# DengZhuangSouthRd/simple_tensorflow

Measured on AMD Instinct MI355X. Metric: images/sec, higher is better.
Workload: dtype bf16; 1 GPU; model=resnet50_v1, global_batch=256, parallelism=dp1

## Files before the change

simple_tensorflow_amd/csrc/framework/ops_defs.cc:

```cpp
#include "framework/op.h"

namespace stf {

#define NUMTYPES "{float, double, int32, int64, bfloat16, half, uint8, int8, complex64}"
#define REALTYPES "{float, double, int32, int64, bfloat16, half}"
#define FLOATTYPES "{float, double, bfloat16, half}"

REGISTER_OP("Const").Output("output: dtype").Attr("dtype: type").Attr("value: tensor");
REGISTER_OP("Placeholder").Output("output: dtype").Attr("dtype: type").Attr("shape: shape = []");
REGISTER_OP("DepthwiseConv2dNative").Input("input: T").Input("filter: T").Output("output: T").Attr("T: {float, bfloat16}").Attr("strides: list(int)").Attr("padding: string").Attr("data_format: string = 'NHWC'");
REGISTER_OP("DepthwiseConv2dNativeBackpropInput").Input("input_sizes: int32").Input("filter: T").Input("out_backprop: T").Output("output: T").Attr("T: {float, bfloat16}").Attr("strides: list(int)").Attr("padding: string").Attr("data_format: string = 'NHWC'");
REGISTER_OP("DepthwiseConv2dNativeBackpropFilter").Input("input: T").Input("filter_sizes: int32").Input("out_backprop: T").Output("output: T").Attr("T: {float, bfloat16}").Attr("strides: list(int)").Attr("padding: string").Attr("data_format: string = 'NHWC'");
REGISTER_OP("PlaceholderWithDefault").Input("input: dtype").Output("output: dtype").Attr("dtype: type").Attr("shape: shape");
REGISTER_OP("Identity").Input("input: T").Output("output: T").Attr("T: type");
REGISTER_OP("StopGradient").Input("input: T").Output("output: T").Attr("T: type");
REGISTER_OP("PreventGradient").Input("input: T").Output("output: T").Attr("T: type").Attr("message: string = ''");
REGISTER_OP("Shape").Input("input: T").Output("output: out_type").Attr("T: type").Attr("out_type: {int32, int64} = int32");
REGISTER_OP("ShapeN").Input("input: N * T").Output("output: N * out_type").Attr("N: int >= 1").Attr("T: type").Attr("out_type: {int32, int64} = int32");
REGISTER_OP("Rank").Input("input: T").Output("output: int32").Attr("T: type");
REGISTER_OP("Size").Input("input: T").Output("output: out_type").Attr("T: type").Attr("out_type: {int32, int64} = int32");
REGISTER_OP("Reshape").Input("tensor: T").Input("shape: Tshape").Output("output: T").Attr("T: type").Attr("Tshape: {int32, int64} = int32");
REGISTER_OP("ExpandDims").Input("input: T").Input("dim: Tdim").Output("output: T").Attr("T: type").Attr("Tdim: {int32, int64} = int32");
REGISTER_OP("Squeeze").Input("input: T").Output("output: T").Attr("T: type").Attr("squeeze_dims: list(int) = []");
REGISTER_OP("Fill").Input("dims: int32").Input("value: T").Output("output: T").Attr("T: type");
REGISTER_OP("ZerosLike").Input("x: T").Output("y: T").Attr("T: type");
REGISTER_OP("OnesLike").Input("x: T").Output("y: T").Attr("T: type");
REGISTER_OP("Cast").Input("x: SrcT").Output("y: DstT").Attr("SrcT: type").Attr("DstT: type");
REGISTER_OP("Pack").Input("values: N * T").Output("output: T").Attr("N: int >= 1").Attr("T: type").Attr("axis: int = 0");
REGISTER_OP("Unpack").Input("value: T").Output("output: num * T").Attr("num: int >= 0").Attr("T: type").Attr("axis: int = 0");
REGISTER_OP("ConcatV2").Input("values: N * T").Input("axis: Tidx").Output("output: T").Attr("N: int >= 2").Attr("T: type").Attr("Tidx: {int32, int64} = int32");
REGISTER_OP("Concat").Input("concat_dim: int32").Input("values: N * T").Output("output: T").Attr("N: int >= 2").Attr("T: type");
REGISTER_OP("ConcatOffset").Input("concat_dim: int32").Input("shape: N * int32").Output("offset: N * int32").Attr("N: int >= 2");
REGISTER_OP("Split").Input("split_dim: int32").Input("value: T").Output("output: num_split * T").Attr("num_split: int >= 1").Attr("T: type");
REGISTER_OP("SplitV").Input("value: T").Input("size_splits: Tlen").Input("split_dim: int32").Output("output: num_split * T").Attr("num_split: int >= 1").Attr("T: type").Attr("Tlen: {int32, int64} = int64");
REGISTER_OP("Slice").Input("input: T").Input("begin: Index").Input("size: Index").Output("output: T").Attr("T: type").Attr("Index: {int32, int64}");
REGISTER_OP("StridedSlice").Input("input: T").Input("begin: Index").Input("end: Index").Input("strides: Index").Output("output: T").Attr("T: type").Attr("Index: {int32, int64}").Attr("begin_mask: int = 0").Attr("end_mask: int = 0").Attr("ellipsis_mask: int = 0").Attr("new_axis_mask: int = 0").Attr("shrink_axis_mask: int = 0");
REGISTER_OP("StridedSliceGrad").Input("shape: Index").Input("begin: Index").Input("end: Index").Input("strides: Index").Input("dy: T").Output("output: T").Attr("T: type").Attr("Index: {int32, int64}").Attr("begin_mask: int = 0").Attr("end_mask: int = 0").Attr("ellipsis_mask: int = 0").Attr("new_axis_mask: int = 0").Attr("shrink_axis_mask: int = 0");
REGISTER_OP("Pad").Input("input: T").Input("paddings: Tpaddings").Output("output: T").Attr("T: type").Attr("Tpaddings: {int32, int64} = int32");
REGISTER_OP("Transpose").Input("x: T").Input("perm: Tperm").Output("y: T").Attr("T: type").Attr("Tperm: {int32, int64} = int32");
REGISTER_OP("Gather").Input("params: Tparams").Input("indices: Tindices").Output("output: Tparams").Attr("validate_indices: bool = true").Attr("Tparams: type").Attr("Tindices: {int32, int64}");
REGISTER_OP("GatherV2").Input("params: Tparams").Input("indices: Tindices").Input("axis: Taxis").Output("output: Tparams").Attr("Tparams: type").Attr("Tindices: {int32, int64}").Attr("Taxis: {int32, int64} = int32");
REGISTER_OP("Tile").Input("input: T").Input("multiples: Tmultiples").Output("output: T").Attr("T: type").Attr("Tmultiples: {int32, int64} = int32");
REGISTER_OP("InvertPermutation").Input("x: T").Output("y: T").Attr("T: {int32, int64} = int32");
REGISTER_OP("Reverse").Input("tensor: T").Input("dims: bool").Output("output: T").Attr("T: type");
REGISTER_OP("BroadcastGradientArgs").Input("s0: T").Input("s1: T").Output("r0: T").Output("r1: T").Attr("T: {int32, int64} = int32");
REGISTER_OP("OneHot").Input("indices: TI").Input("depth: int32").Input("on_value: T").Input("off_value: T").Output("output: T").Attr("axis: int = -1").Attr("T: type").Attr("TI: {uint8, int32, int64} = int64");
REGISTER_OP("Range").Input("start: Tidx").Input("limit: Tidx").Input("delta: Tidx").Output("output: Tidx").Attr("Tidx: {float, double, int32, int64} = int32");
REGISTER_OP("LinSpace").Input("start: T").Input("stop: T").Input("num: Tidx").Output("output: T").Attr("T: {float, double}").Attr("Tidx: {int32, int64} = int32");
REGISTER_OP("CheckNumerics").Input("tensor: T").Output("output: T").Attr("T: " FLOATTYPES).Attr("message: string");
REGISTER_OP("UnsortedSegmentSum").Input("data: T").Input("segment_ids: Tindices").Input("num_segments: int32").Output("output: T").Attr("T: " NUMTYPES).Attr("Tindices: {int32, int64}");
REGISTER_OP("DynamicStitch").Input("indices: N * int32").Input("data: N * T").Output("merged: T").Attr("N: int >= 1").Attr("T: type");

#define BINARY_OP(NAME) REGISTER_OP(NAME).Input("x: T").Input("y: T").Output("z: T")
BINARY_OP("Add").Attr("T: " NUMTYPES);
BINARY_OP("Sub").Attr("T: " NUMTYPES);
BINARY_OP("Mul").Attr("T: " NUMTYPES);
BINARY_OP("Div").Attr("T: " NUMTYPES);
BINARY_OP("RealDiv").Attr("T: " NUMTYPES);
BINARY_OP("FloorDiv").Attr("T: " NUMTYPES);
BINARY_OP("FloorMod").Attr("T: " NUMTYPES);
BINARY_OP("Pow").Attr("T: " NUMTYPES);
BINARY_OP("Maximum").Attr("T: " REALTYPES);
BINARY_OP("Minimum").Attr("T: " REALTYPES);
BINARY_OP("SquaredDifference").Attr("T: " NUMTYPES);
#undef BINARY_OP
#define CMP_OP(NAME) REGISTER_OP(NAME).Input("x: T").Input("y: T").Output("z: bool")
CMP_OP("Less").Attr("T: " REALTYPES);
CMP_OP("LessEqual").Attr("T: " REALTYPES);
CMP_OP("Greater").Attr("T: " REALTYPES);
CMP_OP("GreaterEqual").Attr("T: " REALTYPES);
CMP_OP("Equal").Attr("T: " NUMTYPES);
CMP_OP("NotEqual").Attr("T: " NUMTYPES);
#undef CMP_OP
REGISTER_OP("LogicalAnd").Input("x: bool").Input("y: bool").Output("z: bool");
REGISTER_OP("LogicalOr").Input("x: bool").Input("y: bool").Output("z: bool");
REGISTER_OP("LogicalNot").Input("x: bool").Output("y: bool");
#define UNARY_OP(NAME) REGISTER_OP(NAME).Input("x: T").Output("y: T")
UNARY_OP("Neg").Attr("T: " NUMTYPES);
UNARY_OP("Abs").Attr("T: " REALTYPES);
UNARY_OP("Sign").Attr("T: " REALTYPES);
UNARY_OP("Square").Attr("T: " NUMTYPES);
UNARY_OP("Sqrt").Attr("T: " FLOATTYPES);
UNARY_OP("Rsqrt").Attr("T: " FLOATTYPES);
UNARY_OP("Exp").Attr("T: " FLOATTYPES);
UNARY_OP("Log").Attr("T: " FLOATTYPES);
UNARY_OP("Log1p").Attr("T: " FLOATTYPES);
UNARY_OP("Tanh").Attr("T: " FLOATTYPES);
UNARY_OP("Sigmoid").Attr("T: " FLOATTYPES);
UNARY_OP("Sin").Attr("T: " FLOATTYPES);
UNARY_OP("Cos").Attr("T: " FLOATTYPES);
UNARY_OP("Floor").Attr("T: " FLOATTYPES);
UNARY_OP("Ceil").Attr("T: " FLOATTYPES);
UNARY_OP("Round").Attr("T: " FLOATTYPES);
UNARY_OP("Reciprocal").Attr("T: " NUMTYPES);
#undef UNARY_OP
REGISTER_OP("IsNan").Input("x: T").Output("y: bool").Attr("T: " FLOATTYPES);
REGISTER_OP("IsInf").Input("x: T").Output("y: bool").Attr("T: " FLOATTYPES);
REGISTER_OP("IsFinite").Input("x: T").Output("y: bool").Attr("T: " FLOATTYPES);
#define GRAD2_OP(NAME) REGISTER_OP(NAME).Input("y: T").Input("dy: T").Output("z: T").Attr("T: " FLOATTYPES)
GRAD2_OP("SigmoidGrad");
GRAD2_OP("TanhGrad");
GRAD2_OP("RsqrtGrad");
GRAD2_OP("SqrtGrad");
GRAD2_OP("ReciprocalGrad");
#undef GRAD2_OP
REGISTER_OP("AddN").Input("inputs: N * T").Output("sum: T").Attr("N: int >= 1").Attr("T: " NUMTYPES);
REGISTER_OP("MatMul").Input("a: T").Input("b: T").Output("product: T").Attr("transpose_a: bool = false").Attr("transpose_b: bool = false").Attr("T: " FLOATTYPES);
REGISTER_OP("BatchMatMul").Input("x: T").Input("y: T").Output("output: T").Attr("T: " FLOATTYPES).Attr("adj_x: bool = false").Attr("adj_y: bool = false");
#define REDUCE_OP(NAME) REGISTER_OP(NAME).Input("input: T").Input("reduction_indices: Tidx").Output("output: T").Attr("keep_dims: bool = false").Attr("T: " NUMTYPES).Attr("Tidx: {int32, int64} = int32")
REDUCE_OP("Sum");
REDUCE_OP("Mean");
REDUCE_OP("Prod");
REDUCE_OP("Max");
REDUCE_OP("Min");
#undef REDUCE_OP
REGISTER_OP("All").Input("input: bool").Input("reduction_indices: Tidx").Output("output: bool").Attr("keep_dims: bool = false").Attr("Tidx: {int32, int64} = int32");
REGISTER_OP("Any").Input("input: bool").Input("reduction_indices: Tidx").Output("output: bool").Attr("keep_dims: bool = false").Attr("Tidx: {int32, int64} = int32");
REGISTER_OP("ArgMax").Input("input: T").Input("dimension: Tidx").Output("output: output_type").Attr("T: " NUMTYPES).Attr("Tidx: {int32, int64} = int32").Attr("output_type: {int32, int64} = int64");
REGISTER_OP("ArgMin").Input("input: T").Input("dimension: Tidx").Output("output: output_type").Attr("T: " NUMTYPES).Attr("Tidx: {int32, int64} = int32").Attr("output_type: {int32, int64} = int64");
REGISTER_OP("Select").Input("condition: bool").Input("t: T").Input("e: T").Output("output: T").Attr("T: type");
REGISTER_OP("Cumsum").Input("x: T").Input("axis: Tidx").Output("out: T").Attr("exclusive: bool = false").Attr("reverse: bool = false").Attr("T: " NUMTYPES).Attr("Tidx: {int32, int64} = int32");

REGISTER_OP("Conv2D").Input("input: T").Input("filter: T").Output("output: T").Attr("T: " FLOATTYPES).Attr("strides: list(int)").Attr("use_cudnn_on_gpu: bool = true").Attr("padding: string").Attr("data_format: string = 'NHWC'");
REGISTER_OP("Conv2DBackpropInput").Input("input_sizes: int32").Input("filter: T").Input("out_backprop: T").Output("output: T").Attr("T: " FLOATTYPES).Attr("strides: list(int)").Attr("use_cudnn_on_gpu: bool = true").Attr("padding: string").Attr("data_format: string = 'NHWC'");
REGISTER_OP("Conv2DBackpropInputAdd").Input("input_sizes: int32").Input("filter: T").Input("out_backprop: T").Input("side: T").Output("output: T").Attr("T: " FLOATTYPES).Attr("strides: list(int)").Attr("padding: string").Attr("data_format: string = 'NHWC'");
REGISTER_OP("Conv2DBackpropFilter").Input("input: T").Input("filter_sizes: int32").Input("out_backprop: T").Output("output: T").Attr("T: " FLOATTYPES).Attr("strides: list(int)").Attr("use_cudnn_on_gpu: bool = true").Attr("padding: string").Attr("data_format: string = 'NHWC'");
REGISTER_OP("BiasAdd").Input("value: T").Input("bias: T").Output("output: T").Attr("T: " NUMTYPES).Attr("data_format: string = 'NHWC'");
REGISTER_OP("BiasAddGrad").Input("out_backprop: T").Output("output: T").Attr("T: " NUMTYPES).Attr("data_format: string = 'NHWC'");
REGISTER_OP("Relu").Input("features: T").Output("activations: T").Attr("T: " REALTYPES);
REGISTER_OP("ReluGrad").Input("gradients: T").Input("features: T").Output("backprops: T").Attr("T: " REALTYPES);
REGISTER_OP("Relu6").Input("features: T").Output("activations: T").Attr("T: " REALTYPES);
REGISTER_OP("Relu6Grad").Input("gradients: T").Input("features: T").Output("backprops: T").Attr("T: " REALTYPES);
REGISTER_OP("Elu").Input("features: T").Output("activations: T").Attr("T: " FLOATTYPES);
REGISTER_OP("EluGrad").Input("gradients: T").Input("outputs: T").Output("backprops: T").Attr("T: " FLOATTYPES);
REGISTER_OP("Softplus").Input("features: T").Output("activations: T").Attr("T: " FLOATTYPES);
REGISTER_OP("SoftplusGrad").Input("gradients: T").Input("features: T").Output("backprops: T").Attr("T: " FLOATTYPES);
REGISTER_OP("Softmax").Input("logits: T").Output("softmax: T").Attr("T: " FLOATTYPES);
REGISTER_OP("LogSoftmax").Input("logits: T").Output("logsoftmax: T").Attr("T: " FLOATTYPES);
REGISTER_OP("SoftmaxCrossEntropyWithLogits").Input("features: T").Input("labels: T").Output("loss: T").Output("backprop: T").Attr("T: " FLOATTYPES);
REGISTER_OP("SparseSoftmaxCrossEntropyWithLogits").Input("features: T").Input("labels: Tlabels").Output("loss: T").Output("backprop: T").Attr("T: " FLOATTYPES).Attr("Tlabels: {int32, int64} = int64");
REGISTER_OP("MaxPool").Input("input: T").Output("output: T").Attr("T: " FLOATTYPES).Attr("ksize: list(int)").Attr("strides: list(int)").Attr("padding: string").Attr("data_format: string = 'NHWC'");
REGISTER_OP("MaxPoolGrad").Input("orig_input: T").Input("orig_output: T").Input("grad: T").Output("output: T").Attr("T: " FLOATTYPES).Attr("ksize: list(int)").Attr("strides: list(int)").Attr("padding: string").Attr("data_format: string = 'NHWC'");
REGISTER_OP("AvgPool").Input("value: T").Output("output: T").Attr("T: " FLOATTYPES).Attr("ksize: list(int)").Attr("strides: list(int)").Attr("padding: string").Attr("data_format: string = 'NHWC'");
REGISTER_OP("AvgPoolGrad").Input("orig_input_shape: int32").Input("grad: T").Output("output: T").Attr("T: " FLOATTYPES).Attr("ksize: list(int)").Attr("strides: list(int)").Attr("padding: string").Attr("data_format: string = 'NHWC'");
REGISTER_OP("FusedBatchNorm").Input("x: T").Input("scale: T").Input("offset: T").Input("mean: T").Input("variance: T").Output("y: T").Output("batch_mean: T").Output("batch_variance: T").Output("reserve_space_1: T").Output("reserve_space_2: T").Attr("T: {float}").Attr("epsilon: float = 0.0001").Attr("data_format: string = 'NHWC'").Attr("is_training: bool = true");
REGISTER_OP("FusedBatchNormGrad").Input("y_backprop: T").Input("x: T").Input("scale: T").Input("reserve_space_1: T").Input("reserve_space_2: T").Output("x_backprop: T").Output("scale_backprop: T").Output("offset_backprop: T").Output("reserve_space_3: T").Output("reserve_space_4: T").Attr("T: {float}").Attr("epsilon: float = 0.0001").Attr("data_format: string = 'NHWC'").Attr("is_training: bool = true");
REGISTER_OP("BatchNormMi").Input("x: T").Input("scale: float").Input("offset: float").Output("y: T").Output("batch_mean: float").Output("batch_variance: float").Output("reserve_inv_std: float").Attr("T: {float, bfloat16}").Attr("epsilon: float = 0.0001").Attr("fuse_relu: bool = false");
REGISTER_OP("BatchNormAddReluMi").Input("x: T").Input("scale: float").Input("offset: float").Input("side: T").Output("y: T").Output("batch_mean: float").Output("batch_variance: float").Output("reserve_inv_std: float").Attr("T: {float, bfloat16}").Attr("epsilon: float = 0.0001");
REGISTER_OP("BatchNormAddReluMiGrad").Input("y_backprop: T").Input("x: T").Input("scale: float").Input("saved_mean: float").Input("saved_inv_std: float").Input("y_relu: T").Output("x_backprop: T").Output("scale_backprop: float").Output("offset_backprop: float").Output("side_backprop: T").Attr("T: {float, bfloat16}").Attr("epsilon: float = 0.0001");
REGISTER_OP("BatchNormMiGrad").Input("y_backprop: T").Input("x: T").Input("scale: float").Input("saved_mean: float").Input("saved_inv_std: float").Input("y_relu: T").Output("x_backprop: T").Output("scale_backprop: float").Output("offset_backprop: float").Attr("T: {float, bfloat16}").Attr("epsilon: float = 0.0001").Attr("fuse_relu: bool = false");
REGISTER_OP("_FusedElementwise").Input("inputs: N * T").Output("output: T").Attr("N: int >= 1").Attr("T: {float, bfloat16}").Attr("program: list(int)");
REGISTER_OP("L2Loss").Input("t: T").Output("output: T").Attr("T: " FLOATTYPES);
REGISTER_OP("LSTMGates").Input("gates: T").Input("c_prev: T").Output("i: T").Output("f: T").Output("o: T").Output("ci: T").Output("cs: T").Output("co: T").Output("h: T").Attr("T: {float, bfloat16}").Attr("forget_bias: float = 1.0");
REGISTER_OP("LSTMGatesGrad").Input("c_prev: T").Input("i: T").Input("f: T").Input("o: T").Input("ci: T").Input("co: T").Input("dh: T").Input("dcs: T").Output("dgates: T").Output("dc_prev: T").Attr("T: {float, bfloat16}");
REGISTER_OP("RGBToHSV").Input("images: T").Output("output: T").Attr("T: {float, double} = float");
REGISTER_OP("HSVToRGB").Input("images: T").Output("output: T").Attr("T: {float, double} = float");
REGISTER_OP("AdjustContrastv2").Input("images: T").Input("contrast_factor: float").Output("output: T").Attr("T: {float} = float");
REGISTER_OP("NonMaxSuppression").Input("boxes: float").Input("scores: float").Input("max_output_size: int32").Output("selected_indices: int32").Attr("iou_threshold: float = 0.5");
REGISTER_OP("NonMaxSuppressionV2").Input("boxes: float").Input("scores: float").Input("max_output_size: int32").Input("iou_threshold: float").Output("selected_indices: int32");
REGISTER_OP("SampleDistortedBoundingBox").Input("image_size: T").Input("bounding_boxes: float").Output("begin: T").Output("size: T").Output("bboxes: float").Attr("T: {int32, int64} = int32").Attr("seed: int = 0").Attr("seed2: int = 0").Attr("min_object_covered: float = 0.1").Attr("aspect_ratio_range: list(float) = [0.75, 1.33]").Attr("area_range: list(float) = [0.05, 1.0]").Attr("max_attempts: int = 100").Attr("use_image_if_no_bounding_boxes: bool = false").SetIsStateful();
REGISTER_OP("LRN").Input("input: T").Output("output: T").Attr("depth_radius: int = 5").Attr("bias: float = 1.0").Attr("alpha: float = 1.0").Attr("beta: float = 0.5").Attr("T: {float}");
REGISTER_OP("InTopK").Input("predictions: float").Input("targets: T").Output("precision: bool").Attr("k: int").Attr("T: {int32, int64} = int32");

#define SAMPLER_OP(NAME) REGISTER_OP(NAME).Input("true_classes: int64").Output("sampled_candidates: int64").Output("true_expected_count: float").Output("sampled_expected_count: float").Attr("num_true: int >= 1").Attr("num_sampled: int >= 1").Attr("unique: bool").Attr("range_max: int >= 1").Attr("seed: int = 0").Attr("seed2: int = 0").SetIsStateful()
SAMPLER_OP("UniformCandidateSampler");
SAMPLER_OP("LogUniformCandidateSampler");
SAMPLER_OP("LearnedUnigramCandidateSampler");
#undef SAMPLER_OP
REGISTER_OP("ComputeAccidentalHits").Input("true_classes: int64").Input("sampled_candidates: int64").Output("indices: int32").Output("ids: int64").Output("weights: float").Attr("num_true: int").Attr("seed: int = 0").Attr("seed2: int = 0");

REGISTER_OP("CTCLoss").Input("inputs: float").Input("labels_indices: int64").Input("labels_values: int32").Input("sequence_length: int32").Output("loss: float").Output("gradient: float").Attr("preprocess_collapse_repeated: bool = false").Attr("ctc_merge_repeated: bool = true");
REGISTER_OP("CTCGreedyDecoder").Input("inputs: float").Input("sequence_length: int32").Output("decoded_indices: int64").Output("decoded_values: int64").Output("decoded_shape: int64").Output("log_probability: float").Attr("merge_repeated: bool = false");

REGISTER_OP("FFT").Input("input: complex64").Output("output: complex64");
REGISTER_OP("IFFT").Input("input: complex64").Output("output: complex64");
REGISTER_OP("FFT2D").Input("input: complex64").Output("output: complex64");
REGISTER_OP("IFFT2D").Input("input: complex64").Output("output: complex64");
REGISTER_OP("FFT3D").Input("input: complex64").Output("output: complex64");
REGISTER_OP("IFFT3D").Input("input: complex64").Output("output: complex64");
REGISTER_OP("RFFT").Input("input: float").Input("fft_length: int32").Output("output: complex64");
REGISTER_OP("IRFFT").Input("input: complex64").Input("fft_length: int32").Output("output: float");
REGISTER_OP("RFFT2D").Input("input: float").Input("fft_length: int32").Output("output: complex64");
REGISTER_OP("IRFFT2D").Input("input: complex64").Input("fft_length: int32").Output("output: float");
REGISTER_OP("Complex").Input("real: T").Input("imag: T").Output("out: Tout").Attr("T: {float, double} = float").Attr("Tout: {complex64, complex128} = complex64");
REGISTER_OP("Real").Input("input: T").Output("output: Tout").Attr("T: {complex64, complex128} = complex64").Attr("Tout: {float, double} = float");
REGISTER_OP("Imag").Input("input: T").Output("output: Tout").Attr("T: {complex64, complex128} = complex64").Attr("Tout: {float, double} = float");
REGISTER_OP("Conj").Input("input: T").Output("output: T").Attr("T: {complex64, complex128} = complex64");
REGISTER_OP("ComplexAbs").Input("x: T").Output("y: Tout").Attr("T: {complex64, complex128} = complex64").Attr("Tout: {float, double} = float");

REGISTER_OP("DenseToDenseSetOperation").Input("set1: T").Input("set2: T").Output("result_indices: int64").Output("result_values: T").Output("result_shape: int64").Attr("set_operation: string").Attr("validate_indices: bool = true").Attr("T: {int32, int64}");
REGISTER_OP("SetSize").Input("set_indices: int64").Input("set_values: T").Input("set_shape: int64").Output("size: int32").Attr("validate_indices: bool = true").Attr("T: {int32, int64}");

REGISTER_OP("QuantizeV2").Input("input: float").Input("min_range: float").Input("max_range: float").Output("output: T").Output("output_min: float").Output("output_max: float").Attr("T: {uint8} = uint8").Attr("mode: string = 'MIN_COMBINED'");
REGISTER_OP("Dequantize").Input("input: T").Input("min_range: float").Input("max_range: float").Output("output: float").Attr("T: {uint8, int32} = uint8").Attr("mode: string = 'MIN_COMBINED'");
REGISTER_OP("QuantizedMatMul").Input("a: T1").Input("b: T2").Input("min_a: float").Input("max_a: float").Input("min_b: float").Input("max_b: float").Output("out: Toutput").Output("min_out: float").Output("max_out: float").Attr("T1: {uint8} = uint8").Attr("T2: {uint8} = uint8").Attr("Toutput: {int32} = int32").Attr("transpose_a: bool = false").Attr("transpose_b: bool = false");
REGISTER_OP("QuantizedRelu").Input("features: T").Input("min_features: float").Input("max_features: float").Output("activations: T").Output("min_activations: float").Output("max_activations: float").Attr("T: {uint8} = uint8");
REGISTER_OP("QuantizeDownAndShrinkRange").Input("input: Tinput").Input("input_min: float").Input("input_max: float").Output("output: out_type").Output("output_min: float").Output("output_max: float").Attr("Tinput: {int32} = int32").Attr("out_type: {uint8} = uint8");
REGISTER_OP("RequantizationRange").Input("input: Tinput").Input("input_min: float").Input("input_max: float").Output("output_min: float").Output("output_max: float").Attr("Tinput: {int32} = int32");

REGISTER_OP("Cholesky").Input("input: T").Output("output: T").Attr("T: {float, double}");
REGISTER_OP("CholeskyGrad").Input("l: T").Input("grad: T").Output("output: T").Attr("T: {float, double}");
REGISTER_OP("MatrixDeterminant").Input("input: T").Output("output: T").Attr("T: {float, double}");
REGISTER_OP("MatrixInverse").Input("input: T").Output("output: T").Attr("adjoint: bool = false").Attr("T: {float, double}");
REGISTER_OP("MatrixSolve").Input("matrix: T").Input("rhs: T").Output("output: T").Attr("adjoint: bool = false").Attr("T: {float, double}");
REGISTER_OP("MatrixTriangularSolve").Input("matrix: T").Input("rhs: T").Output("output: T").Attr("lower: bool = true").Attr("adjoint: bool = false").Attr("T: {float, double}");
REGISTER_OP("MatrixSolveLs").Input("matrix: T").Input("rhs: T").Input("l2_regularizer: double").Output("output: T").Attr("T: {float, double}").Attr("fast: bool = true");
REGISTER_OP("Qr").Input("input: T").Output("q: T").Output("r: T").Attr("full_matrices: bool = false").Attr("T: {float, double}");
REGISTER_OP("Svd").Input("input: T").Output("s: T").Output("u: T").Output("v: T").Attr("compute_uv: bool = true").Attr("full_matrices: bool = false").Attr("T: {float, double}");
REGISTER_OP("SelfAdjointEigV2").Input("input: T").Output("e: T").Output("v: T").Attr("compute_v: bool = true").Attr("T: {float, double}");

REGISTER_OP("VariableV2").Output("ref: Ref(dtype)").Attr("shape: shape").Attr("dtype: type").Attr("container: string = ''").Attr("shared_name: string = ''").SetIsStateful();
REGISTER_OP("Variable").Output("ref: Ref(dtype)").Attr("shape: shape").Attr("dtype: type").Attr("container: string = ''").Attr("shared_name: string = ''").SetIsStateful();
REGISTER_OP("IsVariableInitialized").Input("ref: Ref(dtype)").Output("is_initialized: bool").Attr("dtype: type").SetAllowsUninitializedInput();
REGISTER_OP("Assign").Input("ref: Ref(T)").Input("value: T").Output("output_ref: Ref(T)").Attr("T: type").Attr("validate_shape: bool = true").Attr("use_locking: bool = true").SetAllowsUninitializedInput();
REGISTER_OP("AssignAdd").Input("ref: Ref(T)").Input("value: T").Output("output_ref: Ref(T)").Attr("T: " NUMTYPES).Attr("use_locking: bool = false");
REGISTER_OP("AssignSub").Input("ref: Ref(T)").Input("value: T").Output("output_ref: Ref(T)").Attr("T: " NUMTYPES).Attr("use_locking: bool = false");
REGISTER_OP("ScatterSub").Input("ref: Ref(T)").Input("indices: Tindices").Input("updates: T").Output("output_ref: Ref(T)").Attr("T: " NUMTYPES).Attr("Tindices: {int32, int64}").Attr("use_locking: bool = false");
REGISTER_OP("ScatterAdd").Input("ref: Ref(T)").Input("indices: Tindices").Input("updates: T").Output("output_ref: Ref(T)").Attr("T: " NUMTYPES).Attr("Tindices: {int32, int64}").Attr("use_locking: bool = false");
REGISTER_OP("ApplyGradientDescent").Input("var: Ref(T)").Input("alpha: T").Input("delta: T").Output("out: Ref(T)").Attr("T: " FLOATTYPES).Attr("use_locking: bool = false");
REGISTER_OP("ApplyMomentum").Input("var: Ref(T)").Input("accum: Ref(T)").Input("lr: T").Input("grad: T").Input("momentum: T").Output("out: Ref(T)").Attr("T: " FLOATTYPES).Attr("use_locking: bool = false").Attr("use_nesterov: bool = false");
REGISTER_OP("ApplyAdam").Input("var: Ref(T)").Input("m: Ref(T)").Input("v: Ref(T)").Input("beta1_power: T").Input("beta2_power: T").Input("lr: T").Input("beta1: T").Input("beta2: T").Input("epsilon: T").Input("grad: T").Output("out: Ref(T)").Attr("T: " FLOATTYPES).Attr("use_locking: bool = false");
REGISTER_OP("ApplyRMSProp").Input("var: Ref(T)").Input("ms: Ref(T)").Input("mom: Ref(T)").Input("lr: T").Input("rho: T").Input("momentum: T").Input("epsilon: T").Input("grad: T").Output("out: Ref(T)").Attr("T: " FLOATTYPES).Attr("use_locking: bool = false");
REGISTER_OP("ApplyAdagrad").Input("var: Ref(T)").Input("accum: Ref(T)").Input("lr: T").Input("grad: T").Output("out: Ref(T)").Attr("T: " FLOATTYPES).Attr("use_locking: bool = false");
REGISTER_OP("ApplyAdadelta").Input("var: Ref(T)").Input("accum: Ref(T)").Input("accum_update: Ref(T)").Input("lr: T").Input("rho: T").Input("epsilon: T").Input("grad: T").Output("out: Ref(T)").Attr("T: " FLOATTYPES).Attr("use_locking: bool = false");
REGISTER_OP("ApplyFtrl").Input("var: Ref(T)").Input("accum: Ref(T)").Input("linear: Ref(T)").Input("grad: T").Input("lr: T").Input("l1: T").Input("l2: T").Input("lr_power: T").Output("out: Ref(T)").Attr("T: " FLOATTYPES).Attr("use_locking: bool = false");
REGISTER_OP("ApplyProximalGradientDescent").Input("var: Ref(T)").Input("alpha: T").Input("l1: T").Input("l2: T").Input("delta: T").Output("out: Ref(T)").Attr("T: " FLOATTYPES).Attr("use_locking: bool = false");
REGISTER_OP("CountUpTo").Input("ref: Ref(T)").Output("output: T").Attr("limit: int").Attr("T: {int32, int64}");
REGISTER_OP("DestroyTemporaryVariable").Input("ref: Ref(T)").Output("value: T").Attr("T: type").Attr("var_name: string");

REGISTER_OP("RandomUniform").Input("shape: T").Output("output: dtype").Attr("seed: int = 0").Attr("seed2: int = 0").Attr("dtype: " FLOATTYPES).Attr("T: {int32, int64}").SetIsStateful();
REGISTER_OP("RandomStandardNormal").Input("shape: T").Output("output: dtype").Attr("seed: int = 0").Attr("seed2: int = 0").Attr("dtype: " FLOATTYPES).Attr("T: {int32, int64}").SetIsStateful();
REGISTER_OP("TruncatedNormal").Input("shape: T").Output("output: dtype").Attr("seed: int = 0").Attr("seed2: int = 0").Attr("dtype: " FLOATTYPES).Attr("T: {int32, int64}").SetIsStateful();
REGISTER_OP("RandomUniformInt").Input("shape: T").Input("minval: Tout").Input("maxval: Tout").Output("output: Tout").Attr("seed: int = 0").Attr("seed2: int = 0").Attr("T: {int32, int64}").Attr("Tout: {int32, int64}").SetIsStateful();
REGISTER_OP("RandomShuffle").Input("value: T").Output("output: T").Attr("seed: int = 0").Attr("seed2: int = 0").Attr("T: type").SetIsStateful();
REGISTER_OP("Multinomial").Input("logits: T").Input("num_samples: int32").Output("output: int64").Attr("seed: int = 0").Attr("seed2: int = 0").Attr("T: " REALTYPES).SetIsStateful();

REGISTER_OP("Switch").Input("data: T").Input("pred: bool").Output("output_false: T").Output("output_true: T").Attr("T: type");
REGISTER_OP("RefSwitch").Input("data: Ref(T)").Input("pred: bool").Output("output_false: Ref(T)").Output("output_true: Ref(T)").Attr("T: type").SetAllowsUninitializedInput();
REGISTER_OP("Merge").Input("inputs: N * T").Output("output: T").Output("value_index: int32").Attr("N: int >= 1").Attr("T: type");
REGISTER_OP("RefMerge").Input("inputs: N * Ref(T)").Output("output: Ref(T)").Output("value_index: int32").Attr("N: int >= 1").Attr("T: type");
REGISTER_OP("Enter").Input("data: T").Output("output: T").Attr("T: type").Attr("frame_name: string").Attr("is_constant: bool = false").Attr("parallel_iterations: int = 10");
REGISTER_OP("RefEnter").Input("data: Ref(T)").Output("output: Ref(T)").Attr("T: type").Attr("frame_name: string").Attr("is_constant: bool = false").Attr("parallel_iterations: int = 10");
REGISTER_OP("Exit").Input("data: T").Output("output: T").Attr("T: type");
REGISTER_OP("RefExit").Input("data: Ref(T)").Output("output: Ref(T)").Attr("T: type");
REGISTER_OP("NextIteration").Input("data: T").Output("output: T").Attr("T: type");
REGISTER_OP("RefNextIteration").Input("data: Ref(T)").Output("output: Ref(T)").Attr("T: type");
REGISTER_OP("LoopCond").Input("input: bool").Output("output: bool");
REGISTER_OP("ControlTrigger");
REGISTER_OP("NoOp");

REGISTER_OP("_Send").Input("tensor: T").Attr("T: type").Attr("tensor_name: string").Attr("send_device: string").Attr("send_device_incarnation: int = 0").Attr("recv_device: string").Attr("client_terminated: bool = false").SetIsStateful();
REGISTER_OP("_Recv").Output("tensor: tensor_type").Attr("tensor_type: type").Attr("tensor_name: string").Attr("send_device: string").Attr("send_device_incarnation: int = 0").Attr("recv_device: string").Attr("client_terminated: bool = false").SetIsStateful();

REGISTER_OP("Assert").Input("condition: bool").Input("data: T").Attr("T: list(type)").Attr("summarize: int = 3").SetIsStateful();
REGISTER_OP("Print").Input("input: T").Input("data: U").Output("output: T").Attr("T: type").Attr("U: list(type)").Attr("message: string = ''").Attr("first_n: int = -1").Attr("summarize: int = 3").SetIsStateful();
REGISTER_OP("ScalarSummary").Input("tags: string").Input("values: T").Output("summary: string").Attr("T: " REALTYPES);
REGISTER_OP("HistogramSummary").Input("tag: string").Input("values: T").Output("summary: string").Attr("T: " REALTYPES);
REGISTER_OP("MergeSummary").Input("inputs: N * string").Output("summary: string").Attr("N: int >= 1");

REGISTER_OP("SaveV2").Input("prefix: string").Input("tensor_names: string").Input("shape_and_slices: string").Input("tensors: dtypes").Attr("dtypes: list(type)").SetIsStateful();
REGISTER_OP("RestoreV2").Input("prefix: string").Input("tensor_names: string").Input("shape_and_slices: string").Output("tensors: dtypes").Attr("dtypes: list(type)").SetIsStateful();
REGISTER_OP("MergeV2Checkpoints").Input("checkpoint_prefixes: string").Input("destination_prefix: string").Attr("delete_old_dirs: bool = true").SetIsStateful();

REGISTER_OP("PlaceholderWithDefault").Input("input: dtype").Output("output: dtype").Attr("dtype: type").Attr("shape: shape = []");
REGISTER_OP("SparseToDense").Input("sparse_indices: Tindices").Input("output_shape: Tindices").Input("sparse_values: T").Input("default_value: T").Output("dense: T").Attr("validate_indices: bool = true").Attr("T: type").Attr("Tindices: {int32, int64}");

REGISTER_OP("SparseAdd").Input("a_indices: int64").Input("a_values: T").Input("a_shape: int64").Input("b_indices: int64").Input("b_values: T").Input("b_shape: int64").Input("thresh: Treal").Output("sum_indices: int64").Output("sum_values: T").Output("sum_shape: int64").Attr("T: " NUMTYPES).Attr("Treal: {float, double, int32, int64}");
REGISTER_OP("SparseTensorDenseAdd").Input("a_indices: Tindices").Input("a_values: T").Input("a_shape: Tindices").Input("b: T").Output("output: T").Attr("T: " NUMTYPES).Attr("Tindices: {int32, int64}");
REGISTER_OP("SparseReorder").Input("input_indices: int64").Input("input_values: T").Input("input_shape: int64").Output("output_indices: int64").Output("output_values: T").Attr("T: type");
REGISTER_OP("SparseReduceSum").Input("input_indices: int64").Input("input_values: T").Input("input_shape: int64").Input("reduction_axes: int32").Output("output: T").Attr("keep_dims: bool = false").Attr("T: " NUMTYPES);
REGISTER_OP("SparseConcat").Input("indices: N * int64").Input("values: N * T").Input("shapes: N * int64").Output("output_indices: int64").Output("output_values: T").Output("output_shape: int64").Attr("concat_dim: int").Attr("N: int >= 2").Attr("T: type");REGISTER_OP("ResizeBilinear").Input("images: T").Input("size: int32").Output("resized_images: float").Attr("T: {float}").Attr("align_corners: bool = false");
REGISTER_OP("ResizeBilinearGrad").Input("grads: float").Input("original_image: T").Output("output: T").Attr("T: {float}").Attr("align_corners: bool = false");
REGISTER_OP("ResizeNearestNeighbor").Input("images: T").Input("size: int32").Output("resized_images: T").Attr("T: {float}").Attr("align_corners: bool = false");
REGISTER_OP("ConditionalAccumulator").Output("handle: Ref(string)").Attr("dtype: type").Attr("shape: shape").Attr("container: string = ''").Attr("shared_name: string = ''").SetIsStateful();
REGISTER_OP("AccumulatorApplyGradient").Input("handle: Ref(string)").Input("local_step: int64").Input("gradient: dtype").Attr("dtype: type").SetIsStateful();
REGISTER_OP("AccumulatorTakeGradient").Input("handle: Ref(string)").Input("num_required: int32").Output("average: dtype").Attr("dtype: type").SetIsStateful();
REGISTER_OP("AccumulatorSetGlobalStep").Input("handle: Ref(string)").Input("new_global_step: int64").SetIsStateful();
REGISTER_OP("AccumulatorNumAccumulated").Input("handle: Ref(string)").Output("num_accumulated: int32").SetIsStateful();
REGISTER_OP("PyFunc").Input("input: Tin").Output("output: Tout").Attr("token: string").Attr("Tin: list(type) >= 0").Attr("Tout: list(type) >= 0").SetIsStateful();
REGISTER_OP("PyFuncStateless").Input("input: Tin").Output("output: Tout").Attr("token: string").Attr("Tin: list(type) >= 0").Attr("Tout: list(type) >= 0");
REGISTER_OP("TensorArrayV3").Input("size: int32").Output("handle: string").Output("flow: float").Attr("dtype: type").Attr("dynamic_size: bool = false").Attr("clear_after_read: bool = true").Attr("tensor_array_name: string = ''").SetIsStateful();
REGISTER_OP("TensorArrayGradV3").Input("handle: string").Input("flow_in: float").Output("grad_handle: string").Output("flow_out: float").Attr("source: string").SetIsStateful();
REGISTER_OP("TensorArrayWriteV3").Input("handle: string").Input("index: int32").Input("value: T").Input("flow_in: float").Output("flow_out: float").Attr("T: type").SetIsStateful();
REGISTER_OP("TensorArrayReadV3").Input("handle: string").Input("index: int32").Input("flow_in: float").Output("value: dtype").Attr("dtype: type").SetIsStateful();
REGISTER_OP("TensorArraySizeV3").Input("handle: string").Input("flow_in: float").Output("size: int32").SetIsStateful();
REGISTER_OP("TensorArrayGatherV3").Input("handle: string").Input("indices: int32").Input("flow_in: float").Output("value: dtype").Attr("dtype: type").SetIsStateful();
REGISTER_OP("TensorArrayScatterV3").Input("handle: string").Input("indices: int32").Input("value: T").Input("flow_in: float").Output("flow_out: float").Attr("T: type").SetIsStateful();
REGISTER_OP("TensorArrayCloseV3").Input("handle: string").SetIsStateful();

REGISTER_OP("FIFOQueue").Output("handle: Ref(string)").Attr("component_types: list(type)").Attr("shapes: list(shape) = []").Attr("capacity: int = -1").Attr("container: string = ''").Attr("shared_name: string = ''").SetIsStateful();
REGISTER_OP("RandomShuffleQueue").Output("handle: Ref(string)").Attr("component_types: list(type)").Attr("shapes: list(shape) = []").Attr("capacity: int = -1").Attr("min_after_dequeue: int = 0").Attr("seed: int = 0").Attr("seed2: int = 0").Attr("container: string = ''").Attr("shared_name: string = ''").SetIsStateful();
REGISTER_OP("PaddingFIFOQueue").Output("handle: Ref(string)").Attr("component_types: list(type)").Attr("shapes: list(shape) = []").Attr("capacity: int = -1").Attr("container: string = ''").Attr("shared_name: string = ''").SetIsStateful();
REGISTER_OP("QueueEnqueue").Input("handle: Ref(string)").Input("components: Tcomponents").Attr("Tcomponents: list(type)").Attr("timeout_ms: int = -1").SetIsStateful().SetAllowsUninitializedInput();
REGISTER_OP("QueueEnqueueMany").Input("handle: Ref(string)").Input("components: Tcomponents").Attr("Tcomponents: list(type)").Attr("timeout_ms: int = -1").SetIsStateful().SetAllowsUninitializedInput();
REGISTER_OP("QueueDequeue").Input("handle: Ref(string)").Output("components: component_types").Attr("component_types: list(type)").Attr("timeout_ms: int = -1").SetIsStateful().SetAllowsUninitializedInput();
REGISTER_OP("QueueDequeueMany").Input("handle: Ref(string)").Input("n: int32").Output("components: component_types").Attr("component_types: list(type)").Attr("timeout_ms: int = -1").SetIsStateful().SetAllowsUninitializedInput();
REGISTER_OP("QueueClose").Input("handle: Ref(string)").Attr("cancel_pending_enqueues: bool = false").SetIsStateful().SetAllowsUninitializedInput();
REGISTER_OP("QueueSize").Input("handle: Ref(string)").Output("size: int32").SetIsStateful().SetAllowsUninitializedInput();

REGISTER_OP("RcclAllReduce").Input("input: T").Output("output: T").Attr("T: {float, bfloat16, half}").Attr("reduction: string = 'sum'").Attr("num_devices: int = 1").Attr("shared_name: string = ''").SetIsStateful();
REGISTER_OP("RcclBroadcast").Input("input: T").Output("output: T").Attr("T: {float, bfloat16, half}").Attr("root: int = 0").SetIsStateful();
REGISTER_OP("RcclBucketAllReduce").Input("inputs: N * T").Output("outputs: N * T").Attr("N: int >= 1").Attr("T: {float, bfloat16}").Attr("scale: float = 1").SetIsStateful();
REGISTER_OP("RcclCommSync").SetIsStateful();

REGISTER_OP("Where").Input("input: bool").Output("index: int64");
REGISTER_OP("Unique").Input("x: T").Output("y: T").Output("idx: out_idx").Attr("T: type").Attr("out_idx: {int32, int64} = int32");
REGISTER_OP("UniqueWithCounts").Input("x: T").Output("y: T").Output("idx: out_idx").Output("count: out_idx").Attr("T: type").Attr("out_idx: {int32, int64} = int32");
REGISTER_OP("TopKV2").Input("input: T").Input("k: int32").Output("values: T").Output("indices: int32").Attr("sorted: bool = true").Attr("T: " REALTYPES);
REGISTER_OP("TopK").Input("input: T").Output("values: T").Output("indices: int32").Attr("k: int >= 0").Attr("sorted: bool = true").Attr("T: " REALTYPES);
REGISTER_OP("Cumprod").Input("x: T").Input("axis: Tidx").Output("out: T").Attr("exclusive: bool = false").Attr("reverse: bool = false").Attr("T: " NUMTYPES).Attr("Tidx: {int32, int64} = int32");
#define SEGMENT_OP(NAME) REGISTER_OP(NAME).Input("data: T").Input("segment_ids: Tindices").Output("output: T").Attr("T: " NUMTYPES).Attr("Tindices: {int32, int64}")
SEGMENT_OP("SegmentSum");
SEGMENT_OP("SegmentMean");
SEGMENT_OP("SegmentMax");
SEGMENT_OP("SegmentMin");
SEGMENT_OP("SegmentProd");
#undef SEGMENT_OP
REGISTER_OP("ReverseV2").Input("tensor: T").Input("axis: Tidx").Output("output: T").Attr("T: type").Attr("Tidx: {int32, int64} = int32");
REGISTER_OP("ListDiff").Input("x: T").Input("y: T").Output("out: T").Output("idx: out_idx").Attr("T: type").Attr("out_idx: {int32, int64} = int32");
REGISTER_OP("DynamicPartition").Input("data: T").Input("partitions: int32").Output("outputs: num_partitions * T").Attr("num_partitions: int >= 1").Attr("T: type");
REGISTER_OP("GatherNd").Input("params: Tparams").Input("indices: Tindices").Output("output: Tparams").Attr("Tparams: type").Attr("Tindices: {int32, int64}");
REGISTER_OP("ScatterNd").Input("indices: Tindices").Input("updates: T").Input("shape: Tindices").Output("output: T").Attr("T: " NUMTYPES).Attr("Tindices: {int32, int64}");
REGISTER_OP("Diag").Input("diagonal: T").Output("output: T").Attr("T: " NUMTYPES);
REGISTER_OP("DiagPart").Input("input: T").Output("diagonal: T").Attr("T: " NUMTYPES);
REGISTER_OP("MatrixDiag").Input("diagonal: T").Output("output: T").Attr("T: type");
REGISTER_OP("BatchMatrixDiag").Input("diagonal: T").Output("output: T").Attr("T: type");
REGISTER_OP("MatrixDiagPart").Input("input: T").Output("diagonal: T").Attr("T: type");
REGISTER_OP("BatchMatrixDiagPart").Input("input: T").Output("diagonal: T").Attr("T: type");
REGISTER_OP("MatrixSetDiag").Input("input: T").Input("diagonal: T").Output("output: T").Attr("T: type");
REGISTER_OP("BatchMatrixSetDiag").Input("input: T").Input("diagonal: T").Output("output: T").Attr("T: type");
REGISTER_OP("MatrixBandPart").Input("input: T").Input("num_lower: int64").Input("num_upper: int64").Output("band: T").Attr("T: " NUMTYPES);
REGISTER_OP("BatchMatrixBandPart").Input("input: T").Input("num_lower: int64").Input("num_upper: int64").Output("band: T").Attr("T: " NUMTYPES);
REGISTER_OP("SpaceToDepth").Input("input: T").Output("output: T").Attr("T: type").Attr("block_size: int >= 2");
REGISTER_OP("DepthToSpace").Input("input: T").Output("output: T").Attr("T: type").Attr("block_size: int >= 2");
REGISTER_OP("MirrorPad").Input("input: T").Input("paddings: Tpaddings").Output("output: T").Attr("T: type").Attr("Tpaddings: {int32, int64} = int32").Attr("mode: string");
REGISTER_OP("ReverseSequence").Input("input: T").Input("seq_lengths: Tlen").Output("output: T").Attr("seq_dim: int").Attr("batch_dim: int = 0").Attr("T: " NUMTYPES).Attr("Tlen: {int32, int64} = int64");
REGISTER_OP("Bitcast").Input("input: T").Output("output: type").Attr("T: " NUMTYPES).Attr("type: " NUMTYPES);
#define UOP(NAME) REGISTER_OP(NAME).Input("x: T").Output("y: T").Attr("T: " FLOATTYPES)
UOP("Tan");
UOP("Asin");
UOP("Acos");
UOP("Atan");
UOP("Erf");
UOP("Erfc");
UOP("Expm1");
UOP("Lgamma");
UOP("Digamma");
UOP("Rint");
UOP("Softsign");
UOP("Inv");
#undef UOP
REGISTER_OP("SoftsignGrad").Input("gradients: T").Input("features: T").Output("backprops: T").Attr("T: " FLOATTYPES);
REGISTER_OP("InvGrad").Input("y: T").Input("dy: T").Output("z: T").Attr("T: " FLOATTYPES);
REGISTER_OP("Mod").Input("x: T").Input("y: T").Output("z: T").Attr("T: {float, double, int32, int64}");
REGISTER_OP("ApproximateEqual").Input("x: T").Input("y: T").Output("z: bool").Attr("T: " NUMTYPES).Attr("tolerance: float = 1e-05");
REGISTER_OP("AsString").Input("input: T").Output("output: string").Attr("T: {float, double, int32, int64, bool}").Attr("precision: int = -1").Attr("scientific: bool = false").Attr("shortest: bool = false").Attr("width: int = -1").Attr("fill: string = ''");
REGISTER_OP("DecodeRaw").Input("bytes: string").Output("output: out_type").Attr("out_type: {float, double, int32, uint8, int16, int8, int64}").Attr("little_endian: bool = true");
REGISTER_OP("StringJoin").Input("inputs: N * string").Output("output: string").Attr("N: int >= 1").Attr("separator: string = ''");
REGISTER_OP("StringSplit").Input("input: string").Input("delimiter: string").Output("indices: int64").Output("values: string").Output("shape: int64").Attr("skip_empty: bool = true");
REGISTER_OP("Substr").Input("input: string").Input("pos: T").Input("len: T").Output("output: string").Attr("T: {int32, int64}");
REGISTER_OP("StringToHashBucket").Input("string_tensor: string").Output("output: int64").Attr("num_buckets: int >= 1");
REGISTER_OP("StringToHashBucketFast").Input("input: string").Output("output: int64").Attr("num_buckets: int >= 1");
REGISTER_OP("StringToHashBucketStrong").Input("input: string").Output("output: int64").Attr("num_buckets: int >= 1").Attr("key: list(int)");
REGISTER_OP("StringToNumber").Input("string_tensor: string").Output("output: out_type").Attr("out_type: {float, double, int32, int64} = float");
REGISTER_OP("ReduceJoin").Input("inputs: string").Input("reduction_indices: int32").Output("output: string").Attr("keep_dims: bool = false").Attr("separator: string = ''");
REGISTER_OP("EncodeBase64").Input("input: string").Output("output: string").Attr("pad: bool = false");
REGISTER_OP("DecodeBase64").Input("input: string").Output("output: string");
REGISTER_OP("HashTable").Output("table_handle: Ref(string)").Attr("container: string = ''").Attr("shared_name: string = ''").Attr("key_dtype: type").Attr("value_dtype: type").SetIsStateful();
REGISTER_OP("MutableHashTable").Output("table_handle: Ref(string)").Attr("container: string = ''").Attr("shared_name: string = ''").Attr("key_dtype: type").Attr("value_dtype: type").SetIsStateful();
REGISTER_OP("InitializeTable").Input("table_handle: Ref(string)").Input("keys: Tkey").Input("values: Tval").Attr("Tkey: type").Attr("Tval: type").SetIsStateful().SetAllowsUninitializedInput();
REGISTER_OP("LookupTableInsert").Input("table_handle: Ref(string)").Input("keys: Tin").Input("values: Tout").Attr("Tin: type").Attr("Tout: type").SetIsStateful().SetAllowsUninitializedInput();
REGISTER_OP("LookupTableImport").Input("table_handle: Ref(string)").Input("keys: Tin").Input("values: Tout").Attr("Tin: type").Attr("Tout: type").SetIsStateful().SetAllowsUninitializedInput();
REGISTER_OP("LookupTableFind").Input("table_handle: Ref(string)").Input("keys: Tin").Input("default_value: Tout").Output("values: Tout").Attr("Tin: type").Attr("Tout: type").SetIsStateful().SetAllowsUninitializedInput();
REGISTER_OP("LookupTableSize").Input("table_handle: Ref(string)").Output("size: int64").SetIsStateful().SetAllowsUninitializedInput();
REGISTER_OP("LookupTableExport").Input("table_handle: Ref(string)").Output("keys: Tkeys").Output("values: Tvalues").Attr("Tkeys: type").Attr("Tvalues: type").SetIsStateful().SetAllowsUninitializedInput();
REGISTER_OP("Stack").Output("handle: Ref(string)").Attr("elem_type: type").Attr("stack_name: string = ''").SetIsStateful();
REGISTER_OP("StackPush").Input("handle: Ref(string)").Input("elem: T").Output("output: T").Attr("T: type").Attr("swap_memory: bool = false").SetIsStateful().SetAllowsUninitializedInput();
REGISTER_OP("StackPop").Input("handle: Ref(string)").Output("elem: elem_type").Attr("elem_type: type").SetIsStateful().SetAllowsUninitializedInput();
REGISTER_OP("StackClose").Input("handle: Ref(string)").SetIsStateful().SetAllowsUninitializedInput();
REGISTER_OP("Barrier").Output("handle: Ref(string)").Attr("component_types: list(type) >= 1").Attr("shapes: list(shape) = []").Attr("capacity: int = -1").Attr("container: string = ''").Attr("shared_name: string = ''").SetIsStateful();
REGISTER_OP("BarrierInsertMany").Input("handle: Ref(string)").Input("keys: string").Input("values: T").Attr("T: type").Attr("component_index: int").SetIsStateful().SetAllowsUninitializedInput();
REGISTER_OP("BarrierTakeMany").Input("handle: Ref(string)").Input("num_elements: int32").Output("indices: int64").Output("keys: string").Output("values: component_types").Attr("component_types: list(type) >= 1").Attr("allow_small_batch: bool = false").Attr("wait_for_incomplete: bool = false").Attr("timeout_ms: int = -1").SetIsStateful().SetAllowsUninitializedInput();
REGISTER_OP("BarrierClose").Input("handle: Ref(string)").Attr("cancel_pending_enqueues: bool = false").SetIsStateful().SetAllowsUninitializedInput();
REGISTER_OP("BarrierReadySize").Input("handle: Ref(string)").Output("size: int32").SetIsStateful().SetAllowsUninitializedInput();
REGISTER_OP("BarrierIncompleteSize").Input("handle: Ref(string)").Output("size: int32").SetIsStateful().SetAllowsUninitializedInput();
#define SCATTER_VAR_OP(NAME) REGISTER_OP(NAME).Input("ref: Ref(T)").Input("indices: Tindices").Input("updates: T").Output("output_ref: Ref(T)").Attr("T: " NUMTYPES).Attr("Tindices: {int32, int64}").Attr("use_locking: bool = true")
SCATTER_VAR_OP("ScatterUpdate");
SCATTER_VAR_OP("ScatterMul");
SCATTER_VAR_OP("ScatterDiv");
#undef SCATTER_VAR_OP

}
```

simple_tensorflow_amd/csrc/graph/graph.h:

```cpp
#pragma once

#include <map>
#include <memory>
#include <set>
#include <string>
#include <vector>

#include "core/base.h"
#include "core/protos.h"
#include "framework/op.h"

namespace stf {

class Node;

struct Edge {
  Node* src = nullptr;
  int src_output = 0;
  Node* dst = nullptr;
  int dst_input = 0;
  bool IsControl() const { return src_output < 0; }
};

class Node {
 public:
  int id = -1;
  NodeDef def;
  const OpDef* op_def = nullptr;
  std::vector<DataType> in_types;
  std::vector<DataType> out_types;
  std::vector<bool> out_is_ref;
  std::vector<Edge*> in_edges;
  std::vector<Edge*> out_edges;
  std::string assigned_device;

  const std::string& name() const { return def.name; }
  const std::string& op() const { return def.op; }
  int num_inputs() const { return (int)in_types.size(); }
  int num_outputs() const { return (int)out_types.size(); }

  bool IsSwitch() const { return def.op == "Switch" || def.op == "RefSwitch"; }
  bool IsMerge() const { return def.op == "Merge" || def.op == "RefMerge"; }
  bool IsEnter() const { return def.op == "Enter" || def.op == "RefEnter"; }
  bool IsExit() const { return def.op == "Exit" || def.op == "RefExit"; }
  bool IsNextIteration() const {
    return def.op == "NextIteration" || def.op == "RefNextIteration";
  }
  bool IsConstant() const { return def.op == "Const"; }
  bool IsSend() const { return def.op == "_Send" || def.op == "_HostSend"; }
  bool IsRecv() const { return def.op == "_Recv" || def.op == "_HostRecv"; }
  bool IsControlFlow() const {
    return IsSwitch() || IsMerge() || IsEnter() || IsExit() || IsNextIteration();
  }

  const Edge* input_edge(int i) const {
    for (auto* e : in_edges)
      if (!e->IsControl() && e->dst_input == i) return e;
    return nullptr;
  }
};

class Graph {
 public:
  Graph() {}

  Status AddNode(const NodeDef& def, Node** out);
  Edge* AddEdge(Node* src, int src_output, Node* dst, int dst_input);
  Edge* AddControlEdge(Node* src, Node* dst);
  void RemoveNode(Node* n);
  void RemoveEdge(Edge* e);

  Node* FindNode(const std::string& name) const {
    auto it = by_name_.find(name);
    return it == by_name_.end() ? nullptr : it->second;
  }

  const std::vector<Node*>& nodes() const { return alive_; }
  int num_node_ids() const { return (int)nodes_.size(); }
  Node* FindNodeId(int id) const { return nodes_[id].get(); }

  void ToGraphDef(GraphDef* out) const;

 private:
  std::vector<std::unique_ptr<Node>> nodes_;
  std::vector<std::unique_ptr<Edge>> edges_;
  std::vector<Node*> alive_;
  std::map<std::string, Node*> by_name_;
};

Status ConvertGraphDefToGraph(const GraphDef& gdef, Graph* g);

Status TopologicalOrder(const Graph& g, std::vector<Node*>* order);

class Device;

int OptimizeGraph(Graph* g, Device* cpu, const std::set<std::string>& preserve);

}
```

simple_tensorflow_amd/csrc/graph/optimizer.cc:

```cpp
#include <map>
#include <set>
#include <string>
#include <vector>

#include "framework/op_kernel.h"
#include "graph/graph.h"
#include "kernels/fused_ew.h"

namespace stf {

namespace {

bool Blacklisted(const Node* n) {
  const std::string& op = n->op();
  return n->IsControlFlow() || n->IsSend() || n->IsRecv() ||
         op == "Placeholder" ||
         op == "PlaceholderWithDefault" || op == "NoOp" ||
         StrStartsWith(op, "Rccl") || StrStartsWith(op, "Random") ||
         StrStartsWith(op, "TruncatedNormal") || op == "PyFunc";
}

bool IsPure(const Node* n) {
  if (Blacklisted(n)) return false;
  if (n->op_def && n->op_def->is_stateful) return false;
  for (bool r : n->out_is_ref)
    if (r) return false;
  for (DataType t : n->in_types)
    if (t == DT_STRING) return false;
  for (const Edge* e : n->in_edges)
    if (!e->IsControl() && e->src_output < (int)e->src->out_is_ref.size() &&
        e->src->out_is_ref[e->src_output])
      return false;
  return true;
}

std::string AttrFingerprint(const NodeDef& def) {
  pb::Writer w;
  for (const auto& kv : def.attr) {
    pb::Writer av;
    kv.second.Serialize(&av);
    w.PutString(1, kv.first);
    w.PutString(2, av.buf());
  }
  return w.buf();
}

int EliminateCommonSubexpressions(Graph* g,
                                  const std::set<std::string>& preserve) {
  std::vector<Node*> order;
  if (!TopologicalOrder(*g, &order).ok()) return 0;
  std::map<std::string, Node*> canonical;
  int merged = 0;
  for (Node* n : order) {
    if (!IsPure(n) || preserve.count(n->name())) continue;
    std::string sig = n->op() + '\0' + n->def.device + '\0' +
                      AttrFingerprint(n->def);
    std::vector<std::string> ctrl;
    std::map<int, std::string> data;
    bool ok = true;
    for (const Edge* e : n->in_edges) {
      if (e->IsControl()) {
        ctrl.push_back(e->src->name());
      } else {
        data[e->dst_input] = e->src->name() + ':' +
                             std::to_string(e->src_output);
      }
    }
    for (auto& kv : data) sig += '\1' + kv.second;
    std::sort(ctrl.begin(), ctrl.end());
    for (auto& c : ctrl) sig += '\2' + c;
    (void)ok;
    auto it = canonical.find(sig);
    if (it == canonical.end()) {
      canonical.emplace(std::move(sig), n);
      continue;
    }
    Node* rep = it->second;
    std::vector<Edge*> outs(n->out_edges.begin(), n->out_edges.end());
    for (Edge* e : outs) {
      Node* dst = e->dst;
      int di = e->dst_input;
      int so = e->src_output;
      g->RemoveEdge(e);
      if (so < 0)
        g->AddControlEdge(rep, dst);
      else
        g->AddEdge(rep, so, dst, di);
    }
    g->RemoveNode(n);
    ++merged;
  }
  return merged;
}

constexpr int64_t kMaxFoldElements = 1 << 20;

bool AllInputsConst(const Node* n) {
  bool any = false;
  for (const Edge* e : n->in_edges) {
    if (e->IsControl()) return false;
    if (!e->src->IsConstant()) return false;
    any = true;
  }
  return any;
}

int FoldConstants(Graph* g, Device* cpu,
                  const std::set<std::string>& preserve) {
  int folded_total = 0;
  bool changed = true;
  while (changed) {
    changed = false;
    std::vector<Node*> order;
    if (!TopologicalOrder(*g, &order).ok()) return folded_total;
    for (Node* n : order) {
      if (!IsPure(n) || n->num_outputs() != 1 || !AllInputsConst(n) ||
          preserve.count(n->name()))
        continue;
      if (!KernelRegistry::Global()->HasKernel(n->def, "CPU")) continue;
      std::vector<Tensor> inputs(n->num_inputs());
      bool ready = true;
      for (const Edge* e : n->in_edges) {
        auto it = e->src->def.attr.find("value");
        if (it == e->src->def.attr.end() || it->second.kind != 'e') {
          ready = false;
          break;
        }
        Tensor t;
        if (!Tensor::FromProto(it->second.tensor, &t).ok()) {
          ready = false;
          break;
        }
        inputs[e->dst_input] = t;
      }
      if (!ready) continue;
      std::unique_ptr<OpKernel> kernel;
      if (!CreateOpKernel("CPU", cpu, n->def, &kernel).ok()) continue;
      OpKernelContext ctx(kernel.get(), cpu, std::move(inputs));
      kernel->Compute(&ctx);
      if (!ctx.status().ok()) continue;
      const Tensor& result = ctx.output(0);
      if (!result.IsInitialized() ||
          result.NumElements() > kMaxFoldElements ||
          result.dtype() == DT_STRING)
        continue;
      NodeDef cdef;
      cdef.name = n->name() + "/_folded";
      cdef.op = "Const";
      cdef.device = n->def.device;
      AttrValue dt;
      dt.kind = 't';
      dt.type = result.dtype();
      cdef.attr["dtype"] = dt;
      AttrValue val;
      val.kind = 'e';
      result.AsProto(&val.tensor);
      cdef.attr["value"] = val;
      Node* cnode = nullptr;
      if (!g->AddNode(cdef, &cnode).ok()) continue;
      std::vector<Edge*> outs(n->out_edges.begin(), n->out_edges.end());
      for (Edge* e : outs) {
        Node* dst = e->dst;
        int di = e->dst_input;
        int so = e->src_output;
        g->RemoveEdge(e);
        if (so < 0)
          g->AddControlEdge(cnode, dst);
        else
          g->AddEdge(cnode, 0, dst, di);
      }
      g->RemoveNode(n);
      ++folded_total;
      changed = true;
    }
  }
  return folded_total;
}

}


namespace {

int FuseOpcode(const std::string& op) {
  using namespace fused_ew;
  if (op == "Relu") return kRelu;
  if (op == "Relu6") return kRelu6;
  if (op == "Sigmoid") return kSigmoid;
  if (op == "Tanh") return kTanh;
  if (op == "Exp") return kExp;
  if (op == "Log") return kLog;
  if (op == "Log1p") return kLog1p;
  if (op == "Neg") return kNeg;
  if (op == "Sqrt") return kSqrt;
  if (op == "Rsqrt") return kRsqrt;
  if (op == "Square") return kSquare;
  if (op == "Abs") return kAbs;
  if (op == "Softplus") return kSoftplus;
  if (op == "Sign") return kSign;
  if (op == "Floor") return kFloor;
  if (op == "Reciprocal") return kReciprocal;
  if (op == "Add") return kAdd;
  if (op == "Sub") return kSub;
  if (op == "Mul") return kMul;
  if (op == "Div" || op == "RealDiv") return kDiv;
  if (op == "Maximum") return kMaximum;
  if (op == "Minimum") return kMinimum;
  if (op == "SquaredDifference") return kSquaredDifference;
  if (op == "Pow") return kPow;
  return 0;
}

bool IsScalarConst(const Node* n) {
  if (!n->IsConstant()) return false;
  auto it = n->def.attr.find("value");
  if (it == n->def.attr.end() || it->second.kind != 'e') return false;
  const TensorShapeProto& sh = it->second.tensor.tensor_shape;
  int64_t elems = 1;
  for (auto& d : sh.dim) elems *= d.size;
  return elems == 1;
}

bool FusableDtype(const Node* n) {
  if (n->out_types.size() != 1) return false;
  DataType t = n->out_types[0];
  if (t != DT_FLOAT && t != DT_BFLOAT16) return false;
  for (DataType it : n->in_types)
    if (it != t) return false;
  return true;
}

int FuseElementwise(Graph* g, const std::set<std::string>& preserve) {
  std::vector<Node*> order;
  if (!TopologicalOrder(*g, &order).ok()) return 0;
  std::map<Node*, std::pair<Node*, int>> root;
  std::map<Node*, int> opcode;
  for (Node* n : order) {
    if (preserve.count(n->name())) continue;
    int oc = FuseOpcode(n->op());
    if (!oc || !FusableDtype(n)) continue;
    bool has_control = false;
    for (const Edge* e : n->in_edges)
      if (e->IsControl()) has_control = true;
    if (has_control) continue;
    Node* r = nullptr;
    int rp = 0;
    bool ok = true;
    for (const Edge* e : n->in_edges) {
      Node* src = e->src;
      if (IsScalarConst(src)) continue;
      Node* cand;
      int cand_p;
      auto it = root.find(src);
      if (it != root.end()) {
        cand = it->second.first;
        cand_p = it->second.second;
      } else {
        cand = src;
        cand_p = e->src_output;
      }
      if (!r) {
        r = cand;
        rp = cand_p;
      } else if (r != cand || rp != cand_p) {
        ok = false;
        break;
      }
    }
    if (ok && r) {
      root[n] = {r, rp};
      opcode[n] = oc;
    }
  }
  std::map<std::pair<Node*, int>, std::vector<Node*>> groups;
  for (Node* n : order) {
    auto it = root.find(n);
    if (it != root.end()) groups[it->second].push_back(n);
  }
  int fused_total = 0;
  for (auto& kv : groups) {
    const std::vector<Node*>& members = kv.second;
    std::set<Node*> mem(members.begin(), members.end());
    std::vector<Node*> exits;
    for (Node* n : members) {
      bool escapes = n->out_edges.empty();
      for (const Edge* e : n->out_edges)
        if (!mem.count(e->dst)) escapes = true;
      if (escapes) exits.push_back(n);
    }
    for (Node* exit_node : exits) {
    std::vector<Node*> chain;
    std::set<Node*> keep;
    std::vector<Node*> stack = {exit_node};
    while (!stack.empty()) {
      Node* n = stack.back();
      stack.pop_back();
      if (!keep.insert(n).second) continue;
      for (const Edge* e : n->in_edges)
        if (mem.count(e->src)) stack.push_back(e->src);
    }
    for (Node* n : members)
      if (keep.count(n)) chain.push_back(n);
    if ((int)chain.size() < 2 ||
        (int)chain.size() > fused_ew::kMaxInstr)
      continue;
    Node* rnode = kv.first.first;
    int rport = kv.first.second;
    std::vector<std::pair<Node*, int>> inputs = {{rnode, rport}};
    std::map<Node*, int> slot_of_input;
    std::map<Node*, int> slot_of;
    auto input_slot = [&](Node* src, int port) -> int {
      if (src == rnode) return 0;
      auto it = slot_of_input.find(src);
      if (it != slot_of_input.end()) return it->second;
      int s = (int)inputs.size();
      inputs.push_back({src, port});
      slot_of_input[src] = s;
      return s;
    };
    bool ok = true;
    for (Node* n : chain) {
      for (const Edge* e : n->in_edges) {
        if (mem.count(e->src) && keep.count(e->src)) continue;
        if (IsScalarConst(e->src)) {
          input_slot(e->src, e->src_output);
        } else if (!(e->src == rnode && e->src_output == rport)) {
          ok = false;
        }
      }
      if (!ok) break;
    }
    if (!ok || (int)inputs.size() > fused_ew::kMaxInputs) continue;
    int n_in = (int)inputs.size();
    std::vector<int64_t> prog;
    int next_slot = n_in;
    for (Node* n : chain) {
      int srcs[2] = {0, 0};
      int si = 0;
      for (const Edge* e : n->in_edges) {
        if (e->IsControl()) continue;
        int slot;
        if (keep.count(e->src))
          slot = slot_of[e->src];
        else if (e->src == rnode && e->src_output == rport)
          slot = 0;
        else
          slot = input_slot(e->src, e->src_output);
        if (si < 2) srcs[e->dst_input < 2 ? e->dst_input : si] = slot;
        ++si;
      }
      prog.push_back(fused_ew::Pack(opcode[n], srcs[0], srcs[1]));
      slot_of[n] = next_slot++;
    }
    NodeDef fdef;
    fdef.name = exit_node->name() + "/_fused";
    fdef.op = "_FusedElementwise";
    fdef.device = exit_node->def.device;
    AttrValue t;
    t.kind = 't';
    t.type = exit_node->out_types[0];
    fdef.attr["T"] = t;
    AttrValue nattr;
    nattr.kind = 'i';
    nattr.i = n_in;
    fdef.attr["N"] = nattr;
    AttrValue pattr;
    pattr.kind = 'l';
    pattr.list.i = prog;
    fdef.attr["program"] = pattr;
    Node* fnode = nullptr;
    if (!g->AddNode(fdef, &fnode).ok()) continue;
    for (int i = 0; i < n_in; ++i)
      g->AddEdge(inputs[i].first, inputs[i].second, fnode, i);
    std::vector<Edge*> outs(exit_node->out_edges.begin(),
                            exit_node->out_edges.end());
    for (Edge* e : outs) {
      if (mem.count(e->dst)) continue;
      Node* dst = e->dst;
      int di = e->dst_input;
      int so = e->src_output;
      g->RemoveEdge(e);
      if (so < 0)
        g->AddControlEdge(fnode, dst);
      else
        g->AddEdge(fnode, 0, dst, di);
    }
    fused_total += (int)chain.size();
    }
    for (auto it = members.rbegin(); it != members.rend(); ++it)
      if ((*it)->out_edges.empty()) g->RemoveNode(*it);
  }
  return fused_total;
}

}

int OptimizeGraph(Graph* g, Device* cpu,
                  const std::set<std::string>& preserve) {
  static const bool disabled = getenv("STF_NO_GRAPH_OPT") != nullptr;
  if (disabled) return 0;
  int total = 0;
  for (int pass = 0; pass < 3; ++pass) {
    int changed = EliminateCommonSubexpressions(g, preserve);
    changed += FoldConstants(g, cpu, preserve);
    total += changed;
    if (!changed) break;
  }
  static const bool no_fusion = getenv("STF_NO_FUSION") != nullptr;
  if (!no_fusion) total += FuseElementwise(g, preserve);
  return total;
}

}
```

simple_tensorflow_amd/csrc/kernels/gpu_conv.cc:

```cpp
#include "kernels/gpu_common.h"

namespace stf {
namespace {

struct GpuConvGeom {
  int64_t N, H, W, C, R, S, K, sh, sw, ph, pw, P, Q;
  int64_t M() const { return N * P * Q; }
  int64_t RSC() const { return R * S * C; }
  int64_t RSCp() const { return (RSC() + 63) & ~int64_t(63); }
  bool is_1x1_s1() const {
    return R == 1 && S == 1 && sh == 1 && sw == 1 && ph == 0 && pw == 0;
  }
  StfConvGeom abi() const {
    return StfConvGeom{(int)N,  (int)H,  (int)W,  (int)C,  (int)R, (int)S,
                       (int)sh, (int)sw, (int)ph, (int)pw, (int)P, (int)Q, K};
  }
};

static Status GetConvGeom(const TensorShape& x, const TensorShape& f,
                          const std::vector<int64_t>& strides,
                          const std::string& padding, GpuConvGeom* g) {
  g->N = x.dim_size(0);
  g->H = x.dim_size(1);
  g->W = x.dim_size(2);
  g->C = x.dim_size(3);
  g->R = f.dim_size(0);
  g->S = f.dim_size(1);
  g->K = f.dim_size(3);
  if (f.dim_size(2) != g->C)
    return errors::InvalidArgument("conv channel mismatch");
  g->sh = strides[1];
  g->sw = strides[2];
  if (padding == "SAME") {
    g->P = (g->H + g->sh - 1) / g->sh;
    g->Q = (g->W + g->sw - 1) / g->sw;
    g->ph = std::max<int64_t>(0, (g->P - 1) * g->sh + g->R - g->H) / 2;
    g->pw = std::max<int64_t>(0, (g->Q - 1) * g->sw + g->S - g->W) / 2;
  } else {
    g->P = (g->H - g->R) / g->sh + 1;
    g->Q = (g->W - g->S) / g->sw + 1;
    g->ph = g->pw = 0;
  }
  return Status::OK();
}

static bool ImplicitConvEnabled() {
  static const bool enabled = getenv("STF_NO_IMPLICIT_CONV") == nullptr;
  return enabled;
}

static hipError_t PadChannels(OpKernelContext* ctx, const Tensor& x,
                              GpuConvGeom* g, Tensor* xp, hipStream_t s) {
  int64_t c8 = (g->C + 7) & ~7ll;
  *xp = ctx->allocate_temp(DT_BFLOAT16, TensorShape({g->N, g->H, g->W, c8}));
  hipError_t e = stf_block_pad(1, x.raw_data(), xp->raw_data(),
                               g->N * g->H * g->W, g->C, c8, s);
  g->C = c8;
  return e;
}

static hipError_t Im2Col(OpKernelContext* ctx, const Tensor& x,
                         const GpuConvGeom& g, int64_t ld, Tensor* col,
                         hipStream_t s) {
  *col = ctx->allocate_temp(DT_BFLOAT16, TensorShape({g.M(), ld}));
  if (ld != g.RSC()) {
    hipError_t e = hipMemsetAsync(col->raw_data(), 0, g.M() * ld * 2, s);
    if (e != hipSuccess) return e;
  }
  StfConvGeom sg = g.abi();
  return stf_im2col_bf16(x.raw_data(), col->raw_data(), &sg, ld, s);
}

static hipError_t TransposeBf16(OpKernelContext* ctx, const void* src,
                                int64_t rows, int64_t cols, Tensor* dst,
                                hipStream_t s) {
  *dst = ctx->allocate_temp(DT_BFLOAT16, TensorShape({cols, rows}));
  return stf_transpose2d(2, src, dst->raw_data(), rows, cols, s);
}

class GpuConv2DOp : public OpKernel {
 public:
  explicit GpuConv2DOp(OpKernelConstruction* c) : OpKernel(c) {
    c->GetAttr("strides", &strides_);
    c->GetAttr("padding", &padding_);
  }
  void Compute(OpKernelContext* ctx) override {
    hipStream_t s = GPU_STREAM(ctx);
    Tensor x = ctx->input(0);
    Tensor w = ctx->input(1);
    GpuConvGeom g;
    OP_REQUIRES_OK(ctx, GetConvGeom(x.shape(), w.shape(), strides_, padding_,
                                    &g));
    Tensor* y = ctx->allocate_output(0, TensorShape({g.N, g.P, g.Q, g.K}));
    if (!g.is_1x1_s1() && (g.C % 8) != 0 && x.dtype() == DT_BFLOAT16) {
      int64_t c = g.C;
      Tensor xp, wp;
      OP_HIP_OK(ctx, PadChannels(ctx, x, &g, &xp, s));
      wp = ctx->allocate_temp(DT_BFLOAT16, TensorShape({g.RSC(), g.K}));
      OP_HIP_OK(ctx, stf_block_pad(1, w.raw_data(), wp.raw_data(), g.R * g.S,
                                   c * g.K, g.C * g.K, s));
      x = xp;
      w = wp;
    }
    int64_t rsc = g.RSC();
    int64_t rscp = g.is_1x1_s1() ? rsc : g.RSCp();
    if (rscp != rsc) {
      Tensor wz = ctx->allocate_temp(DT_BFLOAT16, TensorShape({rscp, g.K}));
      OP_HIP_OK(ctx, hipMemsetAsync(wz.raw_data(), 0, rscp * g.K * 2, s));
      OP_HIP_OK(ctx, hipMemcpyAsync(wz.raw_data(), w.raw_data(),
                                    rsc * g.K * 2, hipMemcpyDeviceToDevice,
                                    s));
      w = wz;
    }
    StfConvGeom sg = g.abi();

    bool fits_8ph = stf_gemm_bf16_8ph_ok(g.M(), g.K, rscp);
    bool implicit = ImplicitConvEnabled() && !g.is_1x1_s1() && (g.C % 8) == 0;
    enum { kImplicit8Ph, kImplicitNT, kIm2ColGemm } path =
        implicit && fits_8ph && ZeroPage()         ? kImplicit8Ph
        : implicit && (g.K & 7) == 0 && ZeroPage() ? kImplicitNT
                                                   : kIm2ColGemm;

    Tensor wt;
    if (path == kImplicit8Ph) {
      OP_HIP_OK(ctx, TransposeBf16(ctx, w.raw_data(), rscp, g.K, &wt, s));
      OP_HIP_OK(ctx, stf_conv2d_fwd_8ph(x.raw_data(), wt.raw_data(),
                                        y->raw_data(), ZeroPage(), &sg, rscp,
                                        s));
      return;
    }
    if (path == kImplicitNT) {
      OP_HIP_OK(ctx, stf_conv2d_fwd_nt(x.raw_data(), w.raw_data(),
                                       y->raw_data(), ZeroPage(), &sg, rscp,
                                       s));
      return;
    }
    Tensor col = x;
    if (!g.is_1x1_s1()) OP_HIP_OK(ctx, Im2Col(ctx, x, g, rscp, &col, s));
    if (!fits_8ph && (g.K & 7) == 0) {
      OP_HIP_OK(ctx, stf_gemm_bf16(col.raw_data(), w.raw_data(), y->raw_data(),
                                   g.M(), g.K, rscp, rscp, g.K, 0, 1, s));
    } else {
      OP_HIP_OK(ctx, TransposeBf16(ctx, w.raw_data(), rscp, g.K, &wt, s));
      OP_HIP_OK(ctx, stf_gemm_bf16_nt(col.raw_data(), wt.raw_data(),
                                      y->raw_data(), g.M(), g.K, rscp, s));
    }
  }

 private:
  std::vector<int64_t> strides_;
  std::string padding_;
};
REGISTER_KERNEL_BUILDER(Name("Conv2D").Device(DEVICE_GPU).TypeConstraint<bfloat16>("T"), GpuConv2DOp);

class GpuConv2DBackpropInputOp : public OpKernel {
 public:
  explicit GpuConv2DBackpropInputOp(OpKernelConstruction* c, bool side = false)
      : OpKernel(c), side_(side) {
    c->GetAttr("strides", &strides_);
    c->GetAttr("padding", &padding_);
    implicit_dx_ = getenv("STF_NO_IMPLICIT_DX") == nullptr;
  }
  void Compute(OpKernelContext* ctx) override {
    auto in_sizes = IntVector(ctx->input(0));
    const Tensor& w = ctx->input(1);
    const Tensor& dy = ctx->input(2);
    hipStream_t s = GPU_STREAM(ctx);
    TensorShape x_shape(in_sizes);
    GpuConvGeom g;
    OP_REQUIRES_OK(ctx, GetConvGeom(x_shape, w.shape(), strides_, padding_,
                                    &g));
    Tensor* dx = ctx->allocate_output(0, x_shape);
    const void* side = nullptr;
    if (side_) {
      const Tensor& sd = ctx->input(3);
      OP_REQUIRES(ctx, sd.NumElements() == dx->NumElements(),
                  errors::InvalidArgument(
                      "Conv2DBackpropInputAdd: side shape mismatch"));
      side = sd.raw_data();
    }
    if (g.is_1x1_s1() && side && stf_gemm_bf16_8ph_ok(g.M(), g.RSC(), g.K)) {
      OP_HIP_OK(ctx, stf_gemm_bf16_8ph_side(dy.raw_data(), w.raw_data(),
                                            dx->raw_data(), side, g.M(),
                                            g.RSC(), g.K, g.K, g.K, s));
      return;
    }
    StfConvGeom sg = g.abi();
    int64_t nhw = g.N * g.H * g.W;
    int64_t rskp = (g.R * g.S * g.K + 63) & ~int64_t(63);
    bool implicit = implicit_dx_ && g.sh == 1 && g.sw == 1 &&
                    !g.is_1x1_s1() && (g.K % 8) == 0 && ZeroPage();
    if (implicit && stf_gemm_bf16_8ph_ok(nhw, g.C, rskp)) {
      Tensor wt = ctx->allocate_temp(DT_BFLOAT16, TensorShape({g.C, rskp}));
      OP_HIP_OK(ctx, stf_conv_dx_filter(w.raw_data(), wt.raw_data(), (int)g.R,
                                        (int)g.S, (int)g.C, g.K, rskp, s));
      OP_HIP_OK(ctx, stf_conv2d_dx_8ph(dy.raw_data(), wt.raw_data(),
                                       dx->raw_data(), side, ZeroPage(), &sg,
                                       rskp, s));
      return;
    }
    if (g.is_1x1_s1()) {
      OP_HIP_OK(ctx, stf_gemm_bf16_nt(dy.raw_data(), w.raw_data(),
                                      dx->raw_data(), g.M(), g.RSC(), g.K, s));
    } else {
      Tensor dcol = ctx->allocate_temp(DT_BFLOAT16,
                                       TensorShape({g.M(), g.RSC()}));
      OP_HIP_OK(ctx, stf_gemm_bf16_nt(dy.raw_data(), w.raw_data(),
                                      dcol.raw_data(), g.M(), g.RSC(), g.K,
                                      s));
      OP_HIP_OK(ctx, stf_col2im_bf16(dcol.raw_data(), side, dx->raw_data(),
                                     &sg, s));
      return;
    }
    if (side)
      OP_HIP_OK(ctx, stf_binary(B_ADD, DtypeCode(DT_BFLOAT16), dx->raw_data(),
                                side, dx->raw_data(), dx->NumElements(), s));
  }

 private:
  std::vector<int64_t> strides_;
  std::string padding_;
  bool side_;
  bool implicit_dx_;
};
REGISTER_KERNEL_BUILDER(Name("Conv2DBackpropInput").Device(DEVICE_GPU).TypeConstraint<bfloat16>("T").HostMemory("input_sizes"), GpuConv2DBackpropInputOp);

class GpuConv2DBackpropInputAddOp : public GpuConv2DBackpropInputOp {
 public:
  explicit GpuConv2DBackpropInputAddOp(OpKernelConstruction* c)
      : GpuConv2DBackpropInputOp(c, true) {}
};
REGISTER_KERNEL_BUILDER(Name("Conv2DBackpropInputAdd").Device(DEVICE_GPU).TypeConstraint<bfloat16>("T").HostMemory("input_sizes"), GpuConv2DBackpropInputAddOp);

class GpuConv2DBackpropFilterOp : public OpKernel {
 public:
  explicit GpuConv2DBackpropFilterOp(OpKernelConstruction* c) : OpKernel(c) {
    c->GetAttr("strides", &strides_);
    c->GetAttr("padding", &padding_);
  }
  void Compute(OpKernelContext* ctx) override {
    hipStream_t s = GPU_STREAM(ctx);
    const Tensor& x = ctx->input(0);
    auto f_sizes = IntVector(ctx->input(1));
    const Tensor& dy = ctx->input(2);
    TensorShape f_shape(f_sizes);
    GpuConvGeom g;
    OP_REQUIRES_OK(ctx, GetConvGeom(x.shape(), f_shape, strides_, padding_,
                                    &g));
    Tensor* dw = ctx->allocate_output(0, f_shape);
    int64_t rsc = g.RSC();

    bool pad_c = (g.C % 8) != 0 && x.dtype() == DT_BFLOAT16;
    enum { kImplicit, kKMajorGemm, kTransposeGemm } path =
        ImplicitConvEnabled() && !g.is_1x1_s1() &&
                ((g.C % 8) == 0 || pad_c) && (g.K & 7) == 0 &&
                (g.M() & 63) == 0 && ZeroPage()
            ? kImplicit
        : (g.K & 7) == 0 && (!g.is_1x1_s1() || (g.C & 7) == 0)
            ? kKMajorGemm
            : kTransposeGemm;

    if (path == kImplicit) {
      GpuConvGeom gi = g;
      Tensor xp, dwp;
      const void* xdata = x.raw_data();
      void* out = dw->raw_data();
      if (pad_c) {
        OP_HIP_OK(ctx, PadChannels(ctx, x, &gi, &xp, s));
        dwp = ctx->allocate_temp(DT_BFLOAT16, TensorShape({gi.RSC(), g.K}));
        xdata = xp.raw_data();
        out = dwp.raw_data();
      }
      StfConvGeom sg = gi.abi();
      int sk = PickSplitK(gi.RSC(), g.K, g.M());
      OP_HIP_OK(ctx, SplitKInto(ctx, gi.RSC() * g.K, [&](float* acc) {
        return stf_conv2d_dw_splitk(xdata, dy.raw_data(), acc, ZeroPage(),
                                    &sg, sk, s);
      }, out));
      if (pad_c)
        OP_HIP_OK(ctx, stf_block_pad(1, dwp.raw_data(), dw->raw_data(),
                                     g.R * g.S, gi.C * g.K, g.C * g.K, s));
      return;
    }
    if (path == kKMajorGemm) {
      Tensor col = x;
      int64_t lda = g.C;
      if (!g.is_1x1_s1()) {
        lda = g.RSCp();
        OP_HIP_OK(ctx, Im2Col(ctx, x, g, lda, &col, s));
      }
      OP_HIP_OK(ctx, GemmBf16AutoEx(ctx, col.raw_data(), dy.raw_data(),
                                    dw->raw_data(), rsc, g.K, g.M(), lda,
                                    g.K, 1, 1, s));
      return;
    }
    Tensor col = x, colT, dyT;
    if (!g.is_1x1_s1()) OP_HIP_OK(ctx, Im2Col(ctx, x, g, rsc, &col, s));
    OP_HIP_OK(ctx, TransposeBf16(ctx, col.raw_data(), g.M(), rsc, &colT, s));
    OP_HIP_OK(ctx, TransposeBf16(ctx, dy.raw_data(), g.M(), g.K, &dyT, s));
    OP_HIP_OK(ctx, GemmBf16AutoEx(ctx, colT.raw_data(), dyT.raw_data(),
                                  dw->raw_data(), rsc, g.K, g.M(), g.M(),
                                  g.M(), 0, 0, s));
  }

 private:
  std::vector<int64_t> strides_;
  std::string padding_;
};
REGISTER_KERNEL_BUILDER(Name("Conv2DBackpropFilter").Device(DEVICE_GPU).TypeConstraint<bfloat16>("T").HostMemory("filter_sizes"), GpuConv2DBackpropFilterOp);

class GpuDepthwiseConvOp : public OpKernel {
 public:
  explicit GpuDepthwiseConvOp(OpKernelConstruction* c) : OpKernel(c) {
    c->GetAttr("strides", &strides_);
    c->GetAttr("padding", &padding_);
  }
  void Compute(OpKernelContext* ctx) override {
    const Tensor& x = ctx->input(0);
    const Tensor& w = ctx->input(1);
    GpuConvGeom g;
    OP_REQUIRES_OK(ctx, GetConvGeom(x.shape(), w.shape(), strides_, padding_,
                                    &g));
    int mult = (int)w.dim_size(3);
    Tensor* y = ctx->allocate_output(
        0, TensorShape({g.N, g.P, g.Q, g.C * mult}));
    StfConvGeom sg = g.abi();
    OP_HIP_OK(ctx, stf_depthwise_fwd(x.raw_data(), w.raw_data(), y->raw_data(),
                                     &sg, mult, GPU_STREAM(ctx)));
  }

 private:
  std::vector<int64_t> strides_;
  std::string padding_;
};
REGISTER_KERNEL_BUILDER(Name("DepthwiseConv2dNative").Device(DEVICE_GPU).TypeConstraint<bfloat16>("T"), GpuDepthwiseConvOp);

class GpuDepthwiseConvBackpropInputOp : public OpKernel {
 public:
  explicit GpuDepthwiseConvBackpropInputOp(OpKernelConstruction* c)
      : OpKernel(c) {
    c->GetAttr("strides", &strides_);
    c->GetAttr("padding", &padding_);
  }
  void Compute(OpKernelContext* ctx) override {
    auto in_sizes = IntVector(ctx->input(0));
    const Tensor& w = ctx->input(1);
    const Tensor& dy = ctx->input(2);
    TensorShape x_shape(in_sizes);
    GpuConvGeom g;
    OP_REQUIRES_OK(ctx, GetConvGeom(x_shape, w.shape(), strides_, padding_,
                                    &g));
    int mult = (int)w.dim_size(3);
    Tensor* dx = ctx->allocate_output(0, x_shape);
    StfConvGeom sg = g.abi();
    OP_HIP_OK(ctx, stf_depthwise_bwd_input(dy.raw_data(), w.raw_data(),
                                           dx->raw_data(), &sg, mult,
                                           GPU_STREAM(ctx)));
  }

 private:
  std::vector<int64_t> strides_;
  std::string padding_;
};
REGISTER_KERNEL_BUILDER(Name("DepthwiseConv2dNativeBackpropInput").Device(DEVICE_GPU).TypeConstraint<bfloat16>("T").HostMemory("input_sizes"), GpuDepthwiseConvBackpropInputOp);

class GpuDepthwiseConvBackpropFilterOp : public OpKernel {
 public:
  explicit GpuDepthwiseConvBackpropFilterOp(OpKernelConstruction* c)
      : OpKernel(c) {
    c->GetAttr("strides", &strides_);
    c->GetAttr("padding", &padding_);
  }
  void Compute(OpKernelContext* ctx) override {
    const Tensor& x = ctx->input(0);
    auto f_sizes = IntVector(ctx->input(1));
    const Tensor& dy = ctx->input(2);
    TensorShape f_shape(f_sizes);
    GpuConvGeom g;
    OP_REQUIRES_OK(ctx, GetConvGeom(x.shape(), f_shape, strides_, padding_,
                                    &g));
    int mult = (int)f_shape.dim_size(3);
    hipStream_t s = GPU_STREAM(ctx);
    Tensor* dw = ctx->allocate_output(0, f_shape);
    Tensor scratch = ctx->allocate_temp(
        DT_FLOAT, TensorShape({f_shape.num_elements()}));
    OP_HIP_OK(ctx, ZeroF32(scratch.raw_data(), f_shape.num_elements(), s));
    StfConvGeom sg = g.abi();
    OP_HIP_OK(ctx, stf_depthwise_bwd_filter(x.raw_data(), dy.raw_data(),
                                            scratch.flat<float>(), &sg, mult,
                                            s));
    OP_HIP_OK(ctx, stf_cast(0, CastCode(dw->dtype()), scratch.raw_data(),
                            dw->raw_data(), f_shape.num_elements(), s));
  }

 private:
  std::vector<int64_t> strides_;
  std::string padding_;
};
REGISTER_KERNEL_BUILDER(Name("DepthwiseConv2dNativeBackpropFilter").Device(DEVICE_GPU).TypeConstraint<bfloat16>("T").HostMemory("filter_sizes"), GpuDepthwiseConvBackpropFilterOp);

}
}
```

simple_tensorflow_amd/csrc/kernels/gpu_nn.cc:

```cpp
#include "kernels/gpu_common.h"

namespace stf {
namespace {

class GpuBiasAddOp : public OpKernel {
 public:
  using OpKernel::OpKernel;
  void Compute(OpKernelContext* ctx) override {
    const Tensor& x = ctx->input(0);
    const Tensor& b = ctx->input(1);
    Tensor* y = ctx->allocate_output(0, x.shape());
    OP_HIP_OK(ctx, stf_bias_add(DtypeCode(x.dtype()), x.raw_data(),
                                b.raw_data(), y->raw_data(), x.NumElements(),
                                (int)b.NumElements(), GPU_STREAM(ctx)));
  }
};
REGISTER_KERNEL_BUILDER(Name("BiasAdd").Device(DEVICE_GPU).TypeConstraint<float>("T"), GpuBiasAddOp);
REGISTER_KERNEL_BUILDER(Name("BiasAdd").Device(DEVICE_GPU).TypeConstraint<bfloat16>("T"), GpuBiasAddOp);

class GpuBiasAddGradOp : public OpKernel {
 public:
  using OpKernel::OpKernel;
  void Compute(OpKernelContext* ctx) override {
    const Tensor& dy = ctx->input(0);
    int c = (int)dy.dim_size(dy.dims() - 1);
    int64_t rows = dy.NumElements() / c;
    Tensor* db = ctx->allocate_output(0, TensorShape({c}));
    hipStream_t s = GPU_STREAM(ctx);
    Tensor scratch = ctx->allocate_temp(DT_FLOAT, TensorShape({c}));
    OP_HIP_OK(ctx, ZeroF32(scratch.raw_data(), c, s));
    OP_HIP_OK(ctx, stf_bias_grad(DtypeCode(dy.dtype()), dy.raw_data(),
                                 scratch.raw_data(), rows, c, s));
    OP_HIP_OK(ctx, stf_cast(0, CastCode(db->dtype()), scratch.raw_data(),
                            db->raw_data(), c, s));
  }
};
REGISTER_KERNEL_BUILDER(Name("BiasAddGrad").Device(DEVICE_GPU).TypeConstraint<float>("T"), GpuBiasAddGradOp);
REGISTER_KERNEL_BUILDER(Name("BiasAddGrad").Device(DEVICE_GPU).TypeConstraint<bfloat16>("T"), GpuBiasAddGradOp);

class GpuSoftmaxOp : public OpKernel {
 public:
  GpuSoftmaxOp(OpKernelConstruction* c, bool log_sm)
      : OpKernel(c), log_(log_sm) {}
  void Compute(OpKernelContext* ctx) override {
    const Tensor& x = ctx->input(0);
    Tensor* y = ctx->allocate_output(0, x.shape());
    int cols = (int)x.dim_size(x.dims() - 1);
    int64_t rows = x.NumElements() / cols;
    OP_HIP_OK(ctx, stf_softmax(DtypeCode(x.dtype()), log_, x.raw_data(),
                               y->raw_data(), rows, cols, GPU_STREAM(ctx)));
  }

 private:
  bool log_;
};
class SoftmaxGpu : public GpuSoftmaxOp {
 public:
  explicit SoftmaxGpu(OpKernelConstruction* c) : GpuSoftmaxOp(c, false) {}
};
class LogSoftmaxGpu : public GpuSoftmaxOp {
 public:
  explicit LogSoftmaxGpu(OpKernelConstruction* c) : GpuSoftmaxOp(c, true) {}
};
REGISTER_KERNEL_BUILDER(Name("Softmax").Device(DEVICE_GPU).TypeConstraint<float>("T"), SoftmaxGpu);
REGISTER_KERNEL_BUILDER(Name("Softmax").Device(DEVICE_GPU).TypeConstraint<bfloat16>("T"), SoftmaxGpu);
REGISTER_KERNEL_BUILDER(Name("LogSoftmax").Device(DEVICE_GPU).TypeConstraint<float>("T"), LogSoftmaxGpu);

class GpuSparseXentOp : public OpKernel {
 public:
  using OpKernel::OpKernel;
  void Compute(OpKernelContext* ctx) override {
    const Tensor& logits = ctx->input(0);
    const Tensor& labels = ctx->input(1);
    int64_t rows = logits.dim_size(0);
    int cols = (int)logits.dim_size(1);
    Tensor* loss = ctx->allocate_output(0, TensorShape({rows}));
    Tensor* bp = ctx->allocate_output(1, logits.shape());
    hipStream_t s = GPU_STREAM(ctx);
    Tensor loss_f32 = ctx->allocate_temp(DT_FLOAT, TensorShape({rows}));
    OP_HIP_OK(ctx,
              stf_sparse_xent(DtypeCode(logits.dtype()), logits.raw_data(),
                              labels.raw_data(), labels.dtype() == DT_INT32,
                              loss_f32.raw_data(), bp->raw_data(), rows, cols,
                              s));
    OP_HIP_OK(ctx, stf_cast(0, CastCode(loss->dtype()), loss_f32.raw_data(),
                            loss->raw_data(), rows, s));
  }
};
REGISTER_KERNEL_BUILDER(Name("SparseSoftmaxCrossEntropyWithLogits").Device(DEVICE_GPU).TypeConstraint<float>("T"), GpuSparseXentOp);
REGISTER_KERNEL_BUILDER(Name("SparseSoftmaxCrossEntropyWithLogits").Device(DEVICE_GPU).TypeConstraint<bfloat16>("T"), GpuSparseXentOp);

class GpuXentOp : public OpKernel {
 public:
  using OpKernel::OpKernel;
  void Compute(OpKernelContext* ctx) override {
    const Tensor& logits = ctx->input(0);
    const Tensor& labels = ctx->input(1);
    int64_t rows = logits.dim_size(0);
    int cols = (int)logits.dim_size(1);
    Tensor* loss = ctx->allocate_output(0, TensorShape({rows}));
    Tensor* bp = ctx->allocate_output(1, logits.shape());
    hipStream_t s = GPU_STREAM(ctx);
    Tensor loss_f32 = ctx->allocate_temp(DT_FLOAT, TensorShape({rows}));
    OP_HIP_OK(ctx, stf_xent(DtypeCode(logits.dtype()), logits.raw_data(),
                            labels.raw_data(), loss_f32.raw_data(),
                            bp->raw_data(), rows, cols, s));
    OP_HIP_OK(ctx, stf_cast(0, CastCode(loss->dtype()), loss_f32.raw_data(),
                            loss->raw_data(), rows, s));
  }
};
REGISTER_KERNEL_BUILDER(Name("SoftmaxCrossEntropyWithLogits").Device(DEVICE_GPU).TypeConstraint<float>("T"), GpuXentOp);
REGISTER_KERNEL_BUILDER(Name("SoftmaxCrossEntropyWithLogits").Device(DEVICE_GPU).TypeConstraint<bfloat16>("T"), GpuXentOp);

class GpuBatchNormMiOp : public OpKernel {
 public:
  explicit GpuBatchNormMiOp(OpKernelConstruction* c) : OpKernel(c) {
    c->GetAttr("epsilon", &eps_);
    c->GetAttr("fuse_relu", &fuse_relu_);
  }
  void Compute(OpKernelContext* ctx) override {
    const Tensor& x = ctx->input(0);
    const Tensor& scale = ctx->input(1);
    const Tensor& offset = ctx->input(2);
    int c = (int)x.dim_size(x.dims() - 1);
    int64_t rows = x.NumElements() / c;
    Tensor* y = ctx->allocate_output(0, x.shape());
    Tensor* mean = ctx->allocate_output(1, TensorShape({c}));
    Tensor* var = ctx->allocate_output(2, TensorShape({c}));
    Tensor* inv_std = ctx->allocate_output(3, TensorShape({c}));
    hipStream_t s = GPU_STREAM(ctx);
    Tensor acc = ctx->allocate_temp(DT_FLOAT, TensorShape({2 * c}));
    OP_HIP_OK(ctx, ZeroF32(acc.raw_data(), 2 * c, s));
    OP_HIP_OK(ctx, stf_bn_fwd(DtypeCode(x.dtype()), x.raw_data(),
                              scale.raw_data(), offset.raw_data(),
                              acc.flat<float>(), mean->flat<float>(),
                              var->flat<float>(), inv_std->flat<float>(),
                              y->raw_data(), rows, c, eps_,
                              fuse_relu_ ? 1 : 0, s));
  }

 private:
  float eps_ = 1e-4f;
  bool fuse_relu_ = false;
};
REGISTER_KERNEL_BUILDER(Name("BatchNormMi").Device(DEVICE_GPU).TypeConstraint<float>("T"), GpuBatchNormMiOp);
REGISTER_KERNEL_BUILDER(Name("BatchNormMi").Device(DEVICE_GPU).TypeConstraint<bfloat16>("T"), GpuBatchNormMiOp);

class GpuBatchNormAddReluMiOp : public OpKernel {
 public:
  explicit GpuBatchNormAddReluMiOp(OpKernelConstruction* c) : OpKernel(c) {
    c->GetAttr("epsilon", &eps_);
  }
  void Compute(OpKernelContext* ctx) override {
    const Tensor& x = ctx->input(0);
    const Tensor& scale = ctx->input(1);
    const Tensor& offset = ctx->input(2);
    const Tensor& side = ctx->input(3);
    int c = (int)x.dim_size(x.dims() - 1);
    int64_t rows = x.NumElements() / c;
    Tensor* y = ctx->allocate_output(0, x.shape());
    Tensor* mean = ctx->allocate_output(1, TensorShape({c}));
    Tensor* var = ctx->allocate_output(2, TensorShape({c}));
    Tensor* inv_std = ctx->allocate_output(3, TensorShape({c}));
    hipStream_t s = GPU_STREAM(ctx);
    Tensor acc = ctx->allocate_temp(DT_FLOAT, TensorShape({2 * c}));
    OP_HIP_OK(ctx, ZeroF32(acc.raw_data(), 2 * c, s));
    OP_HIP_OK(ctx, stf_bn_stats_only(DtypeCode(x.dtype()), x.raw_data(),
                                     acc.flat<float>(), mean->flat<float>(),
                                     var->flat<float>(),
                                     inv_std->flat<float>(), rows, c, eps_,
                                     s));
    OP_HIP_OK(ctx, stf_bn_add_relu(x.raw_data(), side.raw_data(),
                                   mean->flat<float>(),
                                   inv_std->flat<float>(), scale.raw_data(),
                                   offset.raw_data(), y->raw_data(), rows, c,
                                   s));
  }

 private:
  float eps_ = 1e-4f;
};
REGISTER_KERNEL_BUILDER(Name("BatchNormAddReluMi").Device(DEVICE_GPU).TypeConstraint<bfloat16>("T"), GpuBatchNormAddReluMiOp);

class GpuBatchNormMiGradOp : public OpKernel {
 public:
  explicit GpuBatchNormMiGradOp(OpKernelConstruction* c) : OpKernel(c) {
    c->GetAttr("fuse_relu", &fuse_relu_);
  }
  void Compute(OpKernelContext* ctx) override {
    const Tensor& dy = ctx->input(0);
    const Tensor& x = ctx->input(1);
    const Tensor& scale = ctx->input(2);
    const Tensor& mean = ctx->input(3);
    const Tensor& inv_std = ctx->input(4);
    const Tensor& y_relu = ctx->input(5);
    int c = (int)x.dim_size(x.dims() - 1);
    int64_t rows = x.NumElements() / c;
    Tensor* dx = ctx->allocate_output(0, x.shape());
    Tensor* dscale = ctx->allocate_output(1, TensorShape({c}));
    Tensor* doffset = ctx->allocate_output(2, TensorShape({c}));
    hipStream_t s = GPU_STREAM(ctx);
    OP_HIP_OK(ctx, ZeroF32(doffset->raw_data(), c, s));
    OP_HIP_OK(ctx, ZeroF32(dscale->raw_data(), c, s));
    OP_HIP_OK(ctx, stf_bn_bwd(DtypeCode(x.dtype()), dy.raw_data(),
                              x.raw_data(), y_relu.raw_data(),
                              mean.flat<float>(), inv_std.flat<float>(),
                              scale.raw_data(), doffset->flat<float>(),
                              dscale->flat<float>(), dx->raw_data(), nullptr,
                              rows, c, fuse_relu_ ? 1 : 0, s));
  }

 private:
  bool fuse_relu_ = false;
};
class GpuBatchNormAddReluMiGradOp : public OpKernel {
 public:
  using OpKernel::OpKernel;
  void Compute(OpKernelContext* ctx) override {
    const Tensor& dy = ctx->input(0);
    const Tensor& x = ctx->input(1);
    const Tensor& scale = ctx->input(2);
    const Tensor& mean = ctx->input(3);
    const Tensor& inv_std = ctx->input(4);
    const Tensor& y_relu = ctx->input(5);
    int c = (int)x.dim_size(x.dims() - 1);
    int64_t rows = x.NumElements() / c;
    Tensor* dx = ctx->allocate_output(0, x.shape());
    Tensor* dscale = ctx->allocate_output(1, TensorShape({c}));
    Tensor* doffset = ctx->allocate_output(2, TensorShape({c}));
    Tensor* dside = ctx->allocate_output(3, x.shape());
    hipStream_t s = GPU_STREAM(ctx);
    OP_HIP_OK(ctx, ZeroF32(doffset->raw_data(), c, s));
    OP_HIP_OK(ctx, ZeroF32(dscale->raw_data(), c, s));
    OP_HIP_OK(ctx, stf_bn_bwd(DtypeCode(x.dtype()), dy.raw_data(),
                              x.raw_data(), y_relu.raw_data(),
                              mean.flat<float>(), inv_std.flat<float>(),
                              scale.raw_data(), doffset->flat<float>(),
                              dscale->flat<float>(), dx->raw_data(),
                              dside->raw_data(), rows, c, 1, s));
  }
};
REGISTER_KERNEL_BUILDER(Name("BatchNormAddReluMiGrad").Device(DEVICE_GPU).TypeConstraint<bfloat16>("T"), GpuBatchNormAddReluMiGradOp);

REGISTER_KERNEL_BUILDER(Name("BatchNormMiGrad").Device(DEVICE_GPU).TypeConstraint<float>("T"), GpuBatchNormMiGradOp);
REGISTER_KERNEL_BUILDER(Name("BatchNormMiGrad").Device(DEVICE_GPU).TypeConstraint<bfloat16>("T"), GpuBatchNormMiGradOp);

struct PoolAttrs {
  std::vector<int64_t> ksize, strides;
  std::string padding;
};
static void GetPool(OpKernelConstruction* c, PoolAttrs* p) {
  c->GetAttr("ksize", &p->ksize);
  c->GetAttr("strides", &p->strides);
  c->GetAttr("padding", &p->padding);
}
static StfPoolGeom PoolGeomFor(const TensorShape& x, const PoolAttrs& p) {
  StfPoolGeom g;
  g.N = (int)x.dim_size(0);
  g.H = (int)x.dim_size(1);
  g.W = (int)x.dim_size(2);
  g.C = (int)x.dim_size(3);
  g.kh = (int)p.ksize[1];
  g.kw = (int)p.ksize[2];
  g.sh = (int)p.strides[1];
  g.sw = (int)p.strides[2];
  if (p.padding == "SAME") {
    g.P = (g.H + g.sh - 1) / g.sh;
    g.Q = (g.W + g.sw - 1) / g.sw;
    g.ph = std::max(0, (g.P - 1) * g.sh + g.kh - g.H) / 2;
    g.pw = std::max(0, (g.Q - 1) * g.sw + g.kw - g.W) / 2;
  } else {
    g.P = (g.H - g.kh) / g.sh + 1;
    g.Q = (g.W - g.kw) / g.sw + 1;
    g.ph = g.pw = 0;
  }
  return g;
}

class GpuPoolOp : public OpKernel {
 public:
  GpuPoolOp(OpKernelConstruction* c, bool is_max)
      : OpKernel(c), is_max_(is_max) {
    GetPool(c, &p_);
  }
  void Compute(OpKernelContext* ctx) override {
    const Tensor& x = ctx->input(0);
    StfPoolGeom g = PoolGeomFor(x.shape(), p_);
    Tensor* y = ctx->allocate_output(0, TensorShape({g.N, g.P, g.Q, g.C}));
    OP_HIP_OK(ctx, stf_pool_fwd(DtypeCode(x.dtype()), is_max_, x.raw_data(),
                                y->raw_data(), &g, GPU_STREAM(ctx)));
  }

 private:
  bool is_max_;
  PoolAttrs p_;
};
class MaxPoolGpu : public GpuPoolOp {
 public:
  explicit MaxPoolGpu(OpKernelConstruction* c) : GpuPoolOp(c, true) {}
};
class AvgPoolGpu : public GpuPoolOp {
 public:
  explicit AvgPoolGpu(OpKernelConstruction* c) : GpuPoolOp(c, false) {}
};
REGISTER_KERNEL_BUILDER(Name("MaxPool").Device(DEVICE_GPU).TypeConstraint<float>("T"), MaxPoolGpu);
REGISTER_KERNEL_BUILDER(Name("MaxPool").Device(DEVICE_GPU).TypeConstraint<bfloat16>("T"), MaxPoolGpu);
REGISTER_KERNEL_BUILDER(Name("AvgPool").Device(DEVICE_GPU).TypeConstraint<float>("T"), AvgPoolGpu);
REGISTER_KERNEL_BUILDER(Name("AvgPool").Device(DEVICE_GPU).TypeConstraint<bfloat16>("T"), AvgPoolGpu);

class GpuMaxPoolGradOp : public OpKernel {
 public:
  explicit GpuMaxPoolGradOp(OpKernelConstruction* c) : OpKernel(c) {
    GetPool(c, &p_);
  }
  void Compute(OpKernelContext* ctx) override {
    const Tensor& x = ctx->input(0);
    const Tensor& dy = ctx->input(2);
    StfPoolGeom g = PoolGeomFor(x.shape(), p_);
    Tensor* dx = ctx->allocate_output(0, x.shape());
    hipStream_t s = GPU_STREAM(ctx);
    if (x.dtype() == DT_BFLOAT16 && g.C % 8 == 0) {
      OP_HIP_OK(ctx, stf_max_pool_bwd_v8(x.raw_data(), dy.raw_data(),
                                         dx->raw_data(), &g, s));
      return;
    }
    Tensor scratch = ctx->allocate_temp(DT_FLOAT, x.shape());
    OP_HIP_OK(ctx, ZeroF32(scratch.raw_data(), x.NumElements(), s));
    OP_HIP_OK(ctx, stf_max_pool_bwd(DtypeCode(x.dtype()), x.raw_data(),
                                    dy.raw_data(), scratch.flat<float>(), &g,
                                    s));
    OP_HIP_OK(ctx, stf_cast(0, CastCode(dx->dtype()), scratch.raw_data(),
                            dx->raw_data(), x.NumElements(), s));
  }

 private:
  PoolAttrs p_;
};
REGISTER_KERNEL_BUILDER(Name("MaxPoolGrad").Device(DEVICE_GPU).TypeConstraint<float>("T"), GpuMaxPoolGradOp);
REGISTER_KERNEL_BUILDER(Name("MaxPoolGrad").Device(DEVICE_GPU).TypeConstraint<bfloat16>("T"), GpuMaxPoolGradOp);

class GpuAvgPoolGradOp : public OpKernel {
 public:
  explicit GpuAvgPoolGradOp(OpKernelConstruction* c) : OpKernel(c) {
    GetPool(c, &p_);
  }
  void Compute(OpKernelContext* ctx) override {
    auto in_sizes = IntVector(ctx->input(0));
    const Tensor& dy = ctx->input(1);
    TensorShape x_shape(in_sizes);
    StfPoolGeom g = PoolGeomFor(x_shape, p_);
    Tensor* dx = ctx->allocate_output(0, x_shape);
    OP_HIP_OK(ctx, stf_avg_pool_bwd(DtypeCode(dy.dtype()), dy.raw_data(),
                                    dx->raw_data(), &g, GPU_STREAM(ctx)));
  }

 private:
  PoolAttrs p_;
};
REGISTER_KERNEL_BUILDER(Name("AvgPoolGrad").Device(DEVICE_GPU).TypeConstraint<float>("T").HostMemory("orig_input_shape"), GpuAvgPoolGradOp);
REGISTER_KERNEL_BUILDER(Name("AvgPoolGrad").Device(DEVICE_GPU).TypeConstraint<bfloat16>("T").HostMemory("orig_input_shape"), GpuAvgPoolGradOp);

class GpuLRNOp : public OpKernel {
 public:
  explicit GpuLRNOp(OpKernelConstruction* c) : OpKernel(c) {
    c->GetAttr("depth_radius", &radius_);
    c->GetAttr("bias", &bias_);
    c->GetAttr("alpha", &alpha_);
    c->GetAttr("beta", &beta_);
  }
  void Compute(OpKernelContext* ctx) override {
    const Tensor& x = ctx->input(0);
    Tensor* y = ctx->allocate_output(0, x.shape());
    int64_t c = x.dim_size(x.dims() - 1);
    OP_HIP_OK(ctx, stf_lrn_fwd(x.raw_data(), y->raw_data(),
                               x.NumElements() / c, (int)c, (int)radius_,
                               bias_, alpha_, beta_, GPU_STREAM(ctx)));
  }

 private:
  int64_t radius_ = 5;
  float bias_ = 1.f, alpha_ = 1.f, beta_ = 0.5f;
};
REGISTER_KERNEL_BUILDER(Name("LRN").Device(DEVICE_GPU).TypeConstraint<float>("T"), GpuLRNOp);

class GpuL2LossOp : public OpKernel {
 public:
  using OpKernel::OpKernel;
  void Compute(OpKernelContext* ctx) override {
    const Tensor& x = ctx->input(0);
    hipStream_t s = GPU_STREAM(ctx);
    int dt = DtypeCode(x.dtype());
    int64_t n = x.NumElements();
    Tensor* out = ctx->allocate_output(0, TensorShape({}));
    if (x.dtype() == DT_FLOAT) {
      OP_HIP_OK(ctx, ZeroF32(out->raw_data(), 1, s));
      OP_HIP_OK(ctx, stf_l2loss(dt, x.raw_data(), out->flat<float>(), n, s));
    } else {
      Tensor acc = ctx->allocate_temp(DT_FLOAT, TensorShape({}));
      OP_HIP_OK(ctx, ZeroF32(acc.raw_data(), 1, s));
      OP_HIP_OK(ctx, stf_l2loss(dt, x.raw_data(), acc.flat<float>(), n, s));
      OP_HIP_OK(ctx, stf_cast(0, CastCode(x.dtype()), acc.raw_data(),
                              out->raw_data(), 1, s));
    }
  }
};
REGISTER_KERNEL_BUILDER(Name("L2Loss").Device(DEVICE_GPU).TypeConstraint<float>("T"), GpuL2LossOp);
REGISTER_KERNEL_BUILDER(Name("L2Loss").Device(DEVICE_GPU).TypeConstraint<bfloat16>("T"), GpuL2LossOp);

class GpuLSTMGatesOp : public OpKernel {
 public:
  explicit GpuLSTMGatesOp(OpKernelConstruction* c) : OpKernel(c) {
    c->GetAttr("forget_bias", &forget_bias_);
  }
  void Compute(OpKernelContext* ctx) override {
    const Tensor& gates = ctx->input(0);
    const Tensor& c_prev = ctx->input(1);
    int64_t B = c_prev.shape().dim_size(0);
    int64_t H = c_prev.shape().dim_size(1);
    void* outs[7];
    for (int k = 0; k < 7; ++k)
      outs[k] = ctx->allocate_output(k, c_prev.shape())->raw_data();
    OP_HIP_OK(ctx, stf_lstm_gates(DtypeCode(gates.dtype()), gates.raw_data(),
                                  c_prev.raw_data(), forget_bias_, outs[0],
                                  outs[1], outs[2], outs[3], outs[4], outs[5],
                                  outs[6], B, (int)H, GPU_STREAM(ctx)));
  }

 private:
  float forget_bias_ = 1.f;
};
REGISTER_KERNEL_BUILDER(Name("LSTMGates").Device(DEVICE_GPU).TypeConstraint<float>("T"), GpuLSTMGatesOp);
REGISTER_KERNEL_BUILDER(Name("LSTMGates").Device(DEVICE_GPU).TypeConstraint<bfloat16>("T"), GpuLSTMGatesOp);

class GpuLSTMGatesGradOp : public OpKernel {
 public:
  using OpKernel::OpKernel;
  void Compute(OpKernelContext* ctx) override {
    const Tensor& c_prev = ctx->input(0);
    int64_t B = c_prev.shape().dim_size(0);
    int64_t H = c_prev.shape().dim_size(1);
    Tensor* dgates = ctx->allocate_output(0, TensorShape({B, 4 * H}));
    Tensor* dc_prev = ctx->allocate_output(1, c_prev.shape());
    OP_HIP_OK(ctx, stf_lstm_gates_grad(
                       DtypeCode(c_prev.dtype()), c_prev.raw_data(),
                       ctx->input(1).raw_data(), ctx->input(2).raw_data(),
                       ctx->input(3).raw_data(), ctx->input(4).raw_data(),
                       ctx->input(5).raw_data(), ctx->input(6).raw_data(),
                       ctx->input(7).raw_data(), dgates->raw_data(),
                       dc_prev->raw_data(), B, (int)H, GPU_STREAM(ctx)));
  }
};
REGISTER_KERNEL_BUILDER(Name("LSTMGatesGrad").Device(DEVICE_GPU).TypeConstraint<float>("T"), GpuLSTMGatesGradOp);
REGISTER_KERNEL_BUILDER(Name("LSTMGatesGrad").Device(DEVICE_GPU).TypeConstraint<bfloat16>("T"), GpuLSTMGatesGradOp);

}
}
```

simple_tensorflow_amd/csrc/kernels/hip/bn.hip:

```cpp
#include "hip_common.h"
#include "stf_kernels.h"

namespace {

template <typename T>
__global__ void BnStatsKernel(const T* __restrict__ x, float* __restrict__ acc,
                              int64_t rows, int c) {
  extern __shared__ __attribute__((aligned(16))) char smem[];
  float* s1 = (float*)smem;
  float* s2 = s1 + c;
  for (int i = threadIdx.x; i < c; i += blockDim.x) {
    s1[i] = 0.f;
    s2[i] = 0.f;
  }
  __syncthreads();
  int64_t n = rows * c;
  int64_t gstride = (int64_t)gridDim.x * blockDim.x;
  for (int64_t i = (int64_t)blockIdx.x * blockDim.x + threadIdx.x; i < n;
       i += gstride) {
    float f = (float)x[i];
    int ch = (int)(i % c);
    atomicAdd(&s1[ch], f);
    atomicAdd(&s2[ch], f * f);
  }
  __syncthreads();
  for (int i = threadIdx.x; i < c; i += blockDim.x) {
    atomicAdd(&acc[i], s1[i]);
    atomicAdd(&acc[c + i], s2[i]);
  }
}

__global__ void BnFinalizeKernel(const float* __restrict__ acc,
                                 float* __restrict__ mean,
                                 float* __restrict__ var,
                                 float* __restrict__ inv_std, int64_t rows,
                                 int c, float eps) {
  int i = blockIdx.x * blockDim.x + threadIdx.x;
  if (i >= c) return;
  float m = acc[i] / rows;
  float v = acc[c + i] / rows - m * m;
  v = v > 0.f ? v : 0.f;
  mean[i] = m;
  var[i] = v;
  inv_std[i] = rsqrtf(v + eps);
}

template <typename T, bool RELU>
__global__ void BnNormKernel(const T* __restrict__ x,
                             const float* __restrict__ mean,
                             const float* __restrict__ inv_std,
                             const float* __restrict__ scale,
                             const float* __restrict__ offset,
                             T* __restrict__ y, int64_t n, int c) {
  int64_t stride = (int64_t)gridDim.x * blockDim.x;
  for (int64_t i = blockIdx.x * blockDim.x + threadIdx.x; i < n; i += stride) {
    int ch = (int)(i % c);
    float v = ((float)x[i] - mean[ch]) * inv_std[ch] * scale[ch] + offset[ch];
    if (RELU) v = v > 0.f ? v : 0.f;
    y[i] = (T)v;
  }
}

template <typename T, bool RELU>
__global__ void BnGradStatsKernel(const T* __restrict__ dy,
                                  const T* __restrict__ x,
                                  const T* __restrict__ yr,
                                  const float* __restrict__ mean,
                                  const float* __restrict__ inv_std,
                                  float* __restrict__ sum_dy,
                                  float* __restrict__ sum_dy_xhat,
                                  int64_t rows, int c) {
  extern __shared__ __attribute__((aligned(16))) char smem[];
  float* s1 = (float*)smem;
  float* s2 = s1 + c;
  for (int i = threadIdx.x; i < c; i += blockDim.x) {
    s1[i] = 0.f;
    s2[i] = 0.f;
  }
  __syncthreads();
  int64_t n = rows * c;
  int64_t gstride = (int64_t)gridDim.x * blockDim.x;
  for (int64_t i = (int64_t)blockIdx.x * blockDim.x + threadIdx.x; i < n;
       i += gstride) {
    int ch = (int)(i % c);
    float gf = (float)dy[i];
    if (RELU && (float)yr[i] <= 0.f) gf = 0.f;
    float xhat = ((float)x[i] - mean[ch]) * inv_std[ch];
    atomicAdd(&s1[ch], gf);
    atomicAdd(&s2[ch], gf * xhat);
  }
  __syncthreads();
  for (int i = threadIdx.x; i < c; i += blockDim.x) {
    atomicAdd(&sum_dy[i], s1[i]);
    atomicAdd(&sum_dy_xhat[i], s2[i]);
  }
}

template <typename T, bool RELU, bool DSIDE>
__global__ void BnGradKernel(const T* __restrict__ dy, const T* __restrict__ x,
                             const T* __restrict__ yr,
                             const float* __restrict__ mean,
                             const float* __restrict__ inv_std,
                             const float* __restrict__ scale,
                             const float* __restrict__ sum_dy,
                             const float* __restrict__ sum_dy_xhat,
                             T* __restrict__ dx, T* __restrict__ dside,
                             int64_t n, int64_t rows, int c) {
  int64_t stride = (int64_t)gridDim.x * blockDim.x;
  float inv_rows = 1.f / (float)rows;
  for (int64_t i = blockIdx.x * blockDim.x + threadIdx.x; i < n; i += stride) {
    int ch = (int)(i % c);
    float xhat = ((float)x[i] - mean[ch]) * inv_std[ch];
    float g = (float)dy[i];
    if (RELU && (float)yr[i] <= 0.f) g = 0.f;
    dx[i] = (T)(scale[ch] * inv_std[ch] *
                (g - sum_dy[ch] * inv_rows -
                 xhat * sum_dy_xhat[ch] * inv_rows));
    if (DSIDE) dside[i] = (T)((float)yr[i] > 0.f ? (float)dy[i] : 0.f);
  }
}

struct BnIdx {
  int nw;
  int w;
  int64_t chunk;
  int64_t chunks;
  bool active;
};

__device__ __forceinline__ BnIdx BnThreadIndex(int c, int64_t rows) {
  BnIdx ix;
  ix.nw = c >> 3;
  int64_t tid = (int64_t)blockIdx.x * blockDim.x + threadIdx.x;
  int64_t nthreads = (int64_t)gridDim.x * blockDim.x;
  ix.chunks = nthreads / ix.nw;
  if (ix.chunks > rows) ix.chunks = rows;
  if (ix.chunks < 1) ix.chunks = 1;
  ix.w = (int)(tid % ix.nw);
  ix.chunk = tid / ix.nw;
  ix.active = ix.chunk < ix.chunks;
  return ix;
}

inline int BnGridV9(int c, int64_t rows) {
  int nw = c >> 3;
  int64_t chunks = (131072 + nw - 1) / nw;
  if (chunks > rows) chunks = rows;
  if (chunks < 1) chunks = 1;
  return (int)((nw * chunks + 255) / 256) + 1;
}

__device__ __forceinline__ void Load8(__bf16 (&v)[8], const __bf16* p) {
  *(ulong2*)v = *(const ulong2*)p;
}
__device__ __forceinline__ void Store8(__bf16* p, __bf16 (&v)[8]) {
  *(ulong2*)p = *(ulong2*)v;
}

__global__ void BnStatsKernelV9(const __bf16* __restrict__ x,
                                float* __restrict__ acc, int64_t rows,
                                int c) {
  extern __shared__ __attribute__((aligned(16))) char smem[];
  float* s1 = (float*)smem;
  float* s2 = s1 + c;
  for (int i = threadIdx.x; i < c; i += blockDim.x) {
    s1[i] = 0.f;
    s2[i] = 0.f;
  }
  __syncthreads();
  BnIdx ix = BnThreadIndex(c, rows);
  float p1[8] = {0, 0, 0, 0, 0, 0, 0, 0};
  float p2[8] = {0, 0, 0, 0, 0, 0, 0, 0};
  if (ix.active) {
    const __bf16* base = x + (int64_t)ix.w * 8;
    for (int64_t r = ix.chunk; r < rows; r += ix.chunks) {
      __bf16 v[8];
      Load8(v, base + r * c);
#pragma unroll
      for (int e = 0; e < 8; ++e) {
        float f = (float)v[e];
        p1[e] += f;
        p2[e] += f * f;
      }
    }
#pragma unroll
    for (int e = 0; e < 8; ++e) {
      atomicAdd(&s1[ix.w * 8 + e], p1[e]);
      atomicAdd(&s2[ix.w * 8 + e], p2[e]);
    }
  }
  __syncthreads();
  for (int i = threadIdx.x; i < c; i += blockDim.x)
    if (s1[i] != 0.f || s2[i] != 0.f) {
      atomicAdd(&acc[i], s1[i]);
      atomicAdd(&acc[c + i], s2[i]);
    }
}

template <bool RELU>
__global__ void BnNormKernelV9(const __bf16* __restrict__ x,
                               const float* __restrict__ mean,
                               const float* __restrict__ inv_std,
                               const float* __restrict__ scale,
                               const float* __restrict__ offset,
                               __bf16* __restrict__ y, int64_t rows, int c) {
  BnIdx ix = BnThreadIndex(c, rows);
  if (!ix.active) return;
  int cb = ix.w * 8;
  float m[8], is[8], sc[8], of[8];
#pragma unroll
  for (int e = 0; e < 8; ++e) {
    m[e] = mean[cb + e];
    is[e] = inv_std[cb + e] * scale[cb + e];
    sc[e] = is[e];
    of[e] = offset[cb + e] - m[e] * is[e];
  }
  for (int64_t r = ix.chunk; r < rows; r += ix.chunks) {
    __bf16 v[8], o[8];
    Load8(v, x + r * c + cb);
#pragma unroll
    for (int e = 0; e < 8; ++e) {
      float f = (float)v[e] * sc[e] + of[e];
      if (RELU) f = f > 0.f ? f : 0.f;
      o[e] = (__bf16)f;
    }
    Store8(y + r * c + cb, o);
  }
}

__global__ void BnNormAddReluKernelV9(const __bf16* __restrict__ x,
                                      const __bf16* __restrict__ side,
                                      const float* __restrict__ mean,
                                      const float* __restrict__ inv_std,
                                      const float* __restrict__ scale,
                                      const float* __restrict__ offset,
                                      __bf16* __restrict__ y, int64_t rows,
                                      int c) {
  BnIdx ix = BnThreadIndex(c, rows);
  if (!ix.active) return;
  int cb = ix.w * 8;
  float sc[8], of[8];
#pragma unroll
  for (int e = 0; e < 8; ++e) {
    sc[e] = inv_std[cb + e] * scale[cb + e];
    of[e] = offset[cb + e] - mean[cb + e] * sc[e];
  }
  for (int64_t r = ix.chunk; r < rows; r += ix.chunks) {
    __bf16 v[8], sd[8], o[8];
    Load8(v, x + r * c + cb);
    Load8(sd, side + r * c + cb);
#pragma unroll
    for (int e = 0; e < 8; ++e) {
      float f = (float)v[e] * sc[e] + of[e] + (float)sd[e];
      o[e] = (__bf16)(f > 0.f ? f : 0.f);
    }
    Store8(y + r * c + cb, o);
  }
}

template <bool RELU>
__global__ void BnGradStatsKernelV9(const __bf16* __restrict__ dy,
                                    const __bf16* __restrict__ x,
                                    const __bf16* __restrict__ yr,
                                    const float* __restrict__ mean,
                                    const float* __restrict__ inv_std,
                                    float* __restrict__ sum_dy,
                                    float* __restrict__ sum_dy_xhat,
                                    int64_t rows, int c) {
  extern __shared__ __attribute__((aligned(16))) char smem[];
  float* s1 = (float*)smem;
  float* s2 = s1 + c;
  for (int i = threadIdx.x; i < c; i += blockDim.x) {
    s1[i] = 0.f;
    s2[i] = 0.f;
  }
  __syncthreads();
  BnIdx ix = BnThreadIndex(c, rows);
  float p1[8] = {0, 0, 0, 0, 0, 0, 0, 0};
  float p2[8] = {0, 0, 0, 0, 0, 0, 0, 0};
  if (ix.active) {
    int cb = ix.w * 8;
    float mloc[8], iloc[8];
#pragma unroll
    for (int e = 0; e < 8; ++e) {
      mloc[e] = mean[cb + e];
      iloc[e] = inv_std[cb + e];
    }
    int64_t off = (int64_t)cb;
    for (int64_t r = ix.chunk; r < rows; r += ix.chunks) {
      __bf16 g[8], xv[8], yv[8];
      Load8(g, dy + r * c + off);
      Load8(xv, x + r * c + off);
      if (RELU) Load8(yv, yr + r * c + off);
#pragma unroll
      for (int e = 0; e < 8; ++e) {
        float gf = (float)g[e];
        if (RELU && (float)yv[e] <= 0.f) gf = 0.f;
        float xhat = ((float)xv[e] - mloc[e]) * iloc[e];
        p1[e] += gf;
        p2[e] += gf * xhat;
      }
    }
#pragma unroll
    for (int e = 0; e < 8; ++e) {
      atomicAdd(&s1[cb + e], p1[e]);
      atomicAdd(&s2[cb + e], p2[e]);
    }
  }
  __syncthreads();
  for (int i = threadIdx.x; i < c; i += blockDim.x)
    if (s1[i] != 0.f || s2[i] != 0.f) {
      atomicAdd(&sum_dy[i], s1[i]);
      atomicAdd(&sum_dy_xhat[i], s2[i]);
    }
}

template <bool RELU, bool DSIDE>
__global__ void BnGradKernelV9(const __bf16* __restrict__ dy,
                               const __bf16* __restrict__ x,
                               const __bf16* __restrict__ yr,
                               const float* __restrict__ mean,
                               const float* __restrict__ inv_std,
                               const float* __restrict__ scale,
                               const float* __restrict__ sum_dy,
                               const float* __restrict__ sum_dy_xhat,
                               __bf16* __restrict__ dx,
                               __bf16* __restrict__ dside, int64_t rows,
                               int c) {
  BnIdx ix = BnThreadIndex(c, rows);
  if (!ix.active) return;
  int cb = ix.w * 8;
  float inv_rows = 1.f / (float)rows;
  float m[8], is[8], k[8], a[8], b[8];
#pragma unroll
  for (int e = 0; e < 8; ++e) {
    m[e] = mean[cb + e];
    is[e] = inv_std[cb + e];
    k[e] = scale[cb + e] * is[e];
    a[e] = sum_dy[cb + e] * inv_rows;
    b[e] = sum_dy_xhat[cb + e] * inv_rows;
  }
  for (int64_t r = ix.chunk; r < rows; r += ix.chunks) {
    __bf16 g8[8], x8[8], y8[8], o[8], ds[8];
    Load8(g8, dy + r * c + cb);
    Load8(x8, x + r * c + cb);
    if (RELU) Load8(y8, yr + r * c + cb);
#pragma unroll
    for (int e = 0; e < 8; ++e) {
      float xhat = ((float)x8[e] - m[e]) * is[e];
      float g = (float)g8[e];
      if (RELU && (float)y8[e] <= 0.f) g = 0.f;
      o[e] = (__bf16)(k[e] * (g - a[e] - xhat * b[e]));
      if (DSIDE) ds[e] = (__bf16)((float)y8[e] > 0.f ? (float)g8[e] : 0.f);
    }
    Store8(dx + r * c + cb, o);
    if (DSIDE) Store8(dside + r * c + cb, ds);
  }
}

inline bool UseV9(int dtype, int c) { return dtype != 0 && c % 8 == 0; }

inline size_t BnLdsBytes(int c) { return (size_t)c * 2 * sizeof(float); }

void LaunchBnStats(int dtype, const void* x, float* acc, float* mean,
                   float* var, float* inv_std, int64_t rows, int c, float eps,
                   hipStream_t stream) {
  if (UseV9(dtype, c)) {
    hipLaunchKernelGGL(BnStatsKernelV9, dim3(BnGridV9(c, rows)), dim3(256),
                       BnLdsBytes(c), stream, (const __bf16*)x, acc, rows, c);
  } else {
    DispatchDtype(dtype, [&](auto t) {
      using T = typename decltype(t)::type;
      hipLaunchKernelGGL((BnStatsKernel<T>), dim3(512), dim3(256),
                         BnLdsBytes(c), stream, (const T*)x, acc, rows, c);
    });
  }
  hipLaunchKernelGGL(BnFinalizeKernel, dim3((c + 255) / 256), dim3(256), 0,
                     stream, acc, mean, var, inv_std, rows, c, eps);
}

}

extern "C" {

hipError_t stf_bn_stats_only(int dtype, const void* x, float* acc, float* mean,
                             float* var, float* inv_std, int64_t rows, int c,
                             float eps, hipStream_t stream) {
  LaunchBnStats(dtype, x, acc, mean, var, inv_std, rows, c, eps, stream);
  return hipGetLastError();
}

hipError_t stf_bn_fwd(int dtype, const void* x, const void* scale,
                      const void* offset, float* acc, float* mean, float* var,
                      float* inv_std, void* y, int64_t rows, int c, float eps,
                      int fuse_relu, hipStream_t stream) {
  LaunchBnStats(dtype, x, acc, mean, var, inv_std, rows, c, eps, stream);
  DispatchBool(fuse_relu, [&](auto relu) {
    constexpr bool RELU = decltype(relu)::value;
    if (UseV9(dtype, c)) {
      hipLaunchKernelGGL((BnNormKernelV9<RELU>), dim3(BnGridV9(c, rows)),
                         dim3(256), 0, stream, (const __bf16*)x, mean,
                         inv_std, (const float*)scale, (const float*)offset,
                         (__bf16*)y, rows, c);
      return;
    }
    DispatchDtype(dtype, [&](auto t) {
      using T = typename decltype(t)::type;
      int64_t n = rows * c;
      hipLaunchKernelGGL((BnNormKernel<T, RELU>), ElemwiseGrid(n, 256, 4),
                         dim3(256), 0, stream, (const T*)x, mean, inv_std,
                         (const float*)scale, (const float*)offset, (T*)y, n,
                         c);
    });
  });
  return hipGetLastError();
}

hipError_t stf_bn_add_relu(const void* x, const void* side, const float* mean,
                           const float* inv_std, const void* scale,
                           const void* offset, void* y, int64_t rows, int c,
                           hipStream_t stream) {
  if (c % 8 != 0) return hipErrorInvalidValue;
  hipLaunchKernelGGL(BnNormAddReluKernelV9, dim3(BnGridV9(c, rows)),
                     dim3(256), 0, stream, (const __bf16*)x,
                     (const __bf16*)side, mean, inv_std, (const float*)scale,
                     (const float*)offset, (__bf16*)y, rows, c);
  return hipGetLastError();
}

hipError_t stf_bn_bwd(int dtype, const void* dy, const void* x,
                      const void* y_relu, const float* mean,
                      const float* inv_std, const void* scale,
                      float* sum_dy, float* sum_dy_xhat, void* dx,
                      void* dside, int64_t rows, int c, int fuse_relu,
                      hipStream_t stream) {
  if (dside && !fuse_relu) return hipErrorInvalidValue;
  DispatchBool(fuse_relu, [&](auto relu) {
    constexpr bool RELU = decltype(relu)::value;
    if (UseV9(dtype, c)) {
      dim3 g9(BnGridV9(c, rows));
      hipLaunchKernelGGL((BnGradStatsKernelV9<RELU>), g9, dim3(256),
                         BnLdsBytes(c), stream, (const __bf16*)dy,
                         (const __bf16*)x, (const __bf16*)y_relu, mean,
                         inv_std, sum_dy, sum_dy_xhat, rows, c);
      DispatchBool(RELU && dside, [&](auto ds) {
        constexpr bool DSIDE = RELU && decltype(ds)::value;
        hipLaunchKernelGGL((BnGradKernelV9<RELU, DSIDE>), g9, dim3(256), 0,
                           stream, (const __bf16*)dy, (const __bf16*)x,
                           (const __bf16*)y_relu, mean, inv_std,
                           (const float*)scale, sum_dy, sum_dy_xhat,
                           (__bf16*)dx, (__bf16*)dside, rows, c);
      });
      return;
    }
    DispatchDtype(dtype, [&](auto t) {
      using T = typename decltype(t)::type;
      int64_t n = rows * c;
      hipLaunchKernelGGL((BnGradStatsKernel<T, RELU>), dim3(512), dim3(256),
                         BnLdsBytes(c), stream, (const T*)dy, (const T*)x,
                         (const T*)y_relu, mean, inv_std, sum_dy, sum_dy_xhat,
                         rows, c);
      DispatchBool(RELU && dside, [&](auto ds) {
        constexpr bool DSIDE = RELU && decltype(ds)::value;
        hipLaunchKernelGGL((BnGradKernel<T, RELU, DSIDE>),
                           ElemwiseGrid(n, 256, 4), dim3(256), 0, stream,
                           (const T*)dy, (const T*)x, (const T*)y_relu, mean,
                           inv_std, (const float*)scale, sum_dy, sum_dy_xhat,
                           (T*)dx, (T*)dside, n, rows, c);
      });
    });
  });
  return hipGetLastError();
}

}
```

simple_tensorflow_amd/csrc/kernels/hip/gemm_bf16_8ph.hip:

```cpp
#include "hip_common.h"
#include "stf_kernels.h"

#include <type_traits>

namespace {

__device__ __forceinline__ f32x4 mfma_bf16_8(bf16x8 a, bf16x8 b, f32x4 c) {
  return __builtin_amdgcn_mfma_f32_16x16x32_bf16(a, b, c, 0, 0, 0);
}

__device__ __forceinline__ int Swz8(int r) { return (r ^ (r >> 3)) & 7; }

constexpr int kBM = 256, kBK = 64;
constexpr int kThreads = 512;

template <int ROWS, class AG>
__device__ __forceinline__ void Stage8(const AG& ag, int64_t row0, int64_t k0,
                                       uint16_t* lds_base, int tid) {
#pragma unroll
  for (int p = 0; p < ROWS / 64; ++p) {
    int s = p * kThreads + tid;
    int r = s >> 3;
    int c8 = (s & 7) ^ Swz8(r);
    const uint16_t* g = ag.at(row0 + r, k0 + c8 * 8);
    __builtin_amdgcn_global_load_lds(
        (const __attribute__((address_space(1))) uint32_t*)g,
        (__attribute__((address_space(3))) uint32_t*)(lds_base + s * 8), 16,
        0, 0);
  }
}

template <int NR, bool OUT_BF16, bool FUSE_RELU, class AG>
__launch_bounds__(512) __global__ void Gemm256x8Ph(
    AG ag, const uint16_t* __restrict__ B, void* __restrict__ C,
    const float* __restrict__ bias, const uint16_t* __restrict__ side,
    int64_t M, int64_t N, int64_t K, int64_t ldb) {
  constexpr int kBN = 64 * NR;
  constexpr int kABytes = kBM * kBK * 2;
  constexpr int kBBytes = kBN * kBK * 2;
  extern __shared__ __attribute__((aligned(16))) uint16_t lds[];
  auto a_slot = [&](int slot) { return lds + (size_t)slot * (kABytes / 2); };
  auto b_slot = [&](int slot) {
    return lds + kABytes + (size_t)slot * (kBBytes / 2);
  };

  int nbm = (int)(M / kBM), nbn = (int)(N / kBN);
  int bid = XcdSwizzle(blockIdx.x, nbm * nbn);
  int64_t m0 = (int64_t)(bid / nbn) * kBM;
  int64_t n0 = (int64_t)(bid % nbn) * kBN;

  int tid = threadIdx.x;
  int lane = tid & 63;
  int wid = tid >> 6;
  int wr = wid >> 2;
  int wc = wid & 3;

  int nkt = (int)(K / kBK);

  Stage8<128>(ag, m0, 0, a_slot(0), tid);
  Stage8<128>(ag, m0 + 128, 0, a_slot(0) + 128 * kBK, tid);
  Stage8<kBN>(LinearAG{B, ldb}, n0, 0, b_slot(0), tid);
  if (nkt > 1) {
    Stage8<kBN>(LinearAG{B, ldb}, n0, kBK, b_slot(1), tid);
    if (NR == 4) asm volatile("s_waitcnt vmcnt(4)" ::: "memory");
    else if (NR == 2) asm volatile("s_waitcnt vmcnt(2)" ::: "memory");
    else asm volatile("s_waitcnt vmcnt(1)" ::: "memory");
  } else {
    asm volatile("s_waitcnt vmcnt(0)" ::: "memory");
  }
  __builtin_amdgcn_s_barrier();

  f32x4 acc[8][NR];
#pragma unroll
  for (int i = 0; i < 8; ++i)
#pragma unroll
    for (int j = 0; j < NR; ++j) acc[i][j] = {0.f, 0.f, 0.f, 0.f};

  int a_row_base = wr * 128 + (lane & 15);
  int b_row_base = wc * 16 * NR + (lane & 15);
  int kq = lane >> 4;

  for (int u = 0; u < nkt; ++u) {
    int slot = u & 1;
    const uint16_t* at = a_slot(slot);
    const uint16_t* bt = b_slot(slot);

    bf16x8 bfr[NR][2];
    bf16x8 afr[2][2];

#pragma unroll
    for (int j = 0; j < NR; ++j) {
      int r = b_row_base + j * 16;
#pragma unroll
      for (int kk = 0; kk < 2; ++kk)
        bfr[j][kk] =
            *(const bf16x8*)(bt + (r * 8 + ((kk * 4 + kq) ^ Swz8(r))) * 8);
    }
#pragma unroll
    for (int i = 0; i < 2; ++i) {
      int r = a_row_base + i * 16;
#pragma unroll
      for (int kk = 0; kk < 2; ++kk)
        afr[i][kk] =
            *(const bf16x8*)(at + (r * 8 + ((kk * 4 + kq) ^ Swz8(r))) * 8);
    }
    if (u + 1 < nkt)
      Stage8<128>(ag, m0, (int64_t)(u + 1) * kBK, a_slot(slot ^ 1), tid);
    __builtin_amdgcn_s_barrier();
    asm volatile("s_waitcnt lgkmcnt(0)" ::: "memory");
    __builtin_amdgcn_s_setprio(1);
#pragma unroll
    for (int i = 0; i < 2; ++i)
#pragma unroll
      for (int j = 0; j < NR; ++j)
#pragma unroll
        for (int kk = 0; kk < 2; ++kk)
          acc[i][j] = mfma_bf16_8(afr[i][kk], bfr[j][kk], acc[i][j]);
    __builtin_amdgcn_s_setprio(0);
    __builtin_amdgcn_s_barrier();

#pragma unroll
    for (int q = 1; q < 4; ++q) {
#pragma unroll
      for (int i = 0; i < 2; ++i) {
        int r = a_row_base + (q * 2 + i) * 16;
#pragma unroll
        for (int kk = 0; kk < 2; ++kk)
          afr[i][kk] =
              *(const bf16x8*)(at + (r * 8 + ((kk * 4 + kq) ^ Swz8(r))) * 8);
      }
      if (q == 1) {
        if (u + 1 < nkt)
          Stage8<128>(ag, m0 + 128, (int64_t)(u + 1) * kBK,
                      a_slot(slot ^ 1) + 128 * kBK, tid);
      } else if (q == 2) {
        if (NR == 4) {
          if (u + 2 < nkt)
            Stage8<128>(LinearAG{B, ldb}, n0, (int64_t)(u + 2) * kBK,
                        b_slot(slot), tid);
        }
      } else {
        if (u + 2 < nkt) {
          if (NR == 4) {
            Stage8<128>(LinearAG{B, ldb}, n0 + 128, (int64_t)(u + 2) * kBK,
                        b_slot(slot) + 128 * kBK, tid);
            asm volatile("s_waitcnt vmcnt(4)" ::: "memory");
          } else if (NR == 2) {
            Stage8<kBN>(LinearAG{B, ldb}, n0, (int64_t)(u + 2) * kBK,
                        b_slot(slot), tid);
            asm volatile("s_waitcnt vmcnt(2)" ::: "memory");
          } else {
            Stage8<kBN>(LinearAG{B, ldb}, n0, (int64_t)(u + 2) * kBK,
                        b_slot(slot), tid);
            asm volatile("s_waitcnt vmcnt(1)" ::: "memory");
          }
        } else {
          asm volatile("s_waitcnt vmcnt(0)" ::: "memory");
        }
      }
      __builtin_amdgcn_s_barrier();
      asm volatile("s_waitcnt lgkmcnt(0)" ::: "memory");
      __builtin_amdgcn_s_setprio(1);
#pragma unroll
      for (int i = 0; i < 2; ++i)
#pragma unroll
        for (int j = 0; j < NR; ++j)
#pragma unroll
          for (int kk = 0; kk < 2; ++kk)
            acc[q * 2 + i][j] =
                mfma_bf16_8(afr[i][kk], bfr[j][kk], acc[q * 2 + i][j]);
      __builtin_amdgcn_s_setprio(0);
      __builtin_amdgcn_s_barrier();
    }
  }

  if (OUT_BF16) {
    uint16_t* cbuf = lds;
#pragma unroll
    for (int i = 0; i < 8; ++i) {
#pragma unroll
      for (int j = 0; j < NR; ++j) {
        int col = wc * 16 * NR + j * 16 + (lane & 15);
        float bv = bias ? bias[n0 + col] : 0.f;
#pragma unroll
        for (int rgi = 0; rgi < 4; ++rgi) {
          int row = wr * 128 + i * 16 + (lane >> 4) * 4 + rgi;
          float v = acc[i][j][rgi] + bv;
          if (FUSE_RELU) v = v > 0.f ? v : 0.f;
          cbuf[row * kBN + col] = f32_to_bf16(v);
        }
      }
    }
    __builtin_amdgcn_s_barrier();
    asm volatile("s_waitcnt lgkmcnt(0)" ::: "memory");
#pragma unroll
    for (int p = 0; p < kBM * kBN / 8 / kThreads; ++p) {
      int sidx = (p * kThreads + tid) * 8;
      int r = sidx / kBN;
      int c = sidx % kBN;
      int64_t off = (m0 + r) * N + n0 + c;
      if (side) {
        __bf16 v[8], sv[8];
        *(ulong2*)v = *(ulong2*)(cbuf + sidx);
        *(ulong2*)sv = *(const ulong2*)(side + off);
#pragma unroll
        for (int e = 0; e < 8; ++e) v[e] = (__bf16)((float)v[e] + (float)sv[e]);
        *(ulong2*)((uint16_t*)C + off) = *(ulong2*)v;
      } else {
        *(ulong2*)((uint16_t*)C + off) = *(ulong2*)(cbuf + sidx);
      }
    }
    return;
  }
#pragma unroll
  for (int i = 0; i < 8; ++i) {
#pragma unroll
    for (int j = 0; j < NR; ++j) {
      int64_t col = n0 + wc * 16 * NR + j * 16 + (lane & 15);
      float bv = bias ? bias[col] : 0.f;
#pragma unroll
      for (int rgi = 0; rgi < 4; ++rgi) {
        int64_t row = m0 + wr * 128 + i * 16 + (lane >> 4) * 4 + rgi;
        float v = acc[i][j][rgi] + bv;
        if (side) v += (float)((const __bf16*)side)[row * N + col];
        if (FUSE_RELU) v = v > 0.f ? v : 0.f;
        ((float*)C)[row * N + col] = v;
      }
    }
  }
}

template <class AG>
hipError_t Launch8Ph(const AG& ag, const void* B, void* C, const void* side,
                     int64_t M, int64_t N, int64_t K, int64_t ldb,
                     hipStream_t stream) {
  auto launch = [&](auto nr_c) {
    constexpr int NR = decltype(nr_c)::value;
    int64_t blocks = (M / kBM) * (N / (64 * NR));
    size_t shmem = 64 * 1024 + 2 * (size_t)(64 * NR) * kBK * 2;
    hipLaunchKernelGGL((Gemm256x8Ph<NR, true, false, AG>),
                       dim3((uint32_t)blocks), dim3(kThreads), shmem, stream,
                       ag, (const uint16_t*)B, C, (const float*)nullptr,
                       (const uint16_t*)side, M, N, K, ldb);
  };
  if (N % 256 == 0) launch(std::integral_constant<int, 4>{});
  else if (N % 128 == 0) launch(std::integral_constant<int, 2>{});
  else launch(std::integral_constant<int, 1>{});
  return hipGetLastError();
}

}

extern "C" {

int stf_gemm_bf16_8ph_ok(int64_t M, int64_t N, int64_t K) {
  return (M % 256 == 0) && (N % 64 == 0) && (K % 64 == 0) && K > 0;
}

hipError_t stf_gemm_bf16_8ph_side(const void* A, const void* B, void* C,
                                  const void* side_bf16, int64_t M, int64_t N,
                                  int64_t K, int64_t lda, int64_t ldb,
                                  hipStream_t stream) {
  if (!stf_gemm_bf16_8ph_ok(M, N, K)) return hipErrorInvalidValue;
  LinearAG ag{(const uint16_t*)A, lda};
  return Launch8Ph(ag, B, C, side_bf16, M, N, K, ldb, stream);
}

hipError_t stf_conv2d_fwd_8ph(const void* x, const void* wt, void* y,
                              const void* zero16, const StfConvGeom* g,
                              int64_t rscp, hipStream_t stream) {
  int64_t M = (int64_t)g->n * g->p * g->q;
  if (!stf_gemm_bf16_8ph_ok(M, g->cout, rscp) || (g->c % 8) != 0)
    return hipErrorInvalidValue;
  return Launch8Ph(MakeConvAG(*g, x, zero16), wt, y, nullptr, M, g->cout,
                   rscp, rscp, stream);
}

hipError_t stf_conv2d_dx_8ph(const void* dy, const void* wt, void* dx,
                             const void* side, const void* zero16,
                             const StfConvGeom* g, int64_t rscp,
                             hipStream_t stream) {
  int64_t M = (int64_t)g->n * g->h * g->w;
  if (g->sh != 1 || g->sw != 1 || (g->cout % 8) != 0 ||
      !stf_gemm_bf16_8ph_ok(M, g->c, rscp) ||
      rscp < (int64_t)g->r * g->s * g->cout)
    return hipErrorInvalidValue;
  return Launch8Ph(MakeConvAG(ConvDxGeom(*g), dy, zero16), wt, dx, side, M,
                   g->c, rscp, rscp, stream);
}

}
```

simple_tensorflow_amd/csrc/kernels/hip/stf_kernels.h:

```cpp
#pragma once

#include <hip/hip_runtime_api.h>

#include <cstdint>

struct StfConvGeom {
  int n, h, w, c;
  int r, s;
  int sh, sw, ph, pw;
  int p, q;
  int64_t cout;
};

struct StfPoolGeom {
  int N, H, W, C, kh, kw, sh, sw, ph, pw, P, Q;
};

constexpr int kStfMaxPermuteRank = 6;

enum StfReduce { STF_REDUCE_SUM = 0, STF_REDUCE_MAX = 1, STF_REDUCE_MIN = 2 };
constexpr float StfReduceIdentity(StfReduce kind) {
  return kind == STF_REDUCE_SUM ? 0.f
         : kind == STF_REDUCE_MAX ? -3.4e38f : 3.4e38f;
}

extern "C" {

hipError_t stf_gemm_bf16(const void* A, const void* B, void* C, int64_t M,
                         int64_t N, int64_t K, int64_t lda, int64_t ldb,
                         int a_km, int b_km, hipStream_t stream);
hipError_t stf_gemm_bf16_nt(const void* A, const void* B, void* C, int64_t M,
                            int64_t N, int64_t K, hipStream_t stream);
hipError_t stf_gemm_bf16_splitk(const void* A, const void* B, void* C_f32,
                                int64_t M, int64_t N, int64_t K, int64_t lda,
                                int64_t ldb, int a_km, int b_km, int splitk,
                                hipStream_t stream);
int stf_gemm_bf16_8ph_ok(int64_t M, int64_t N, int64_t K);
hipError_t stf_gemm_bf16_8ph_side(const void* A, const void* B, void* C,
                                  const void* side_bf16, int64_t M, int64_t N,
                                  int64_t K, int64_t lda, int64_t ldb,
                                  hipStream_t stream);
hipError_t stf_gemm_f32_nt(const void* A, const void* B, void* C, int64_t M,
                           int64_t N, int64_t K, hipStream_t stream);

hipError_t stf_conv2d_fwd_8ph(const void* x, const void* wt, void* y,
                              const void* zero16, const StfConvGeom* g,
                              int64_t rscp, hipStream_t stream);
hipError_t stf_conv2d_fwd_nt(const void* x, const void* w, void* y,
                             const void* zero16, const StfConvGeom* g,
                             int64_t rscp, hipStream_t stream);
hipError_t stf_conv2d_dw_splitk(const void* x, const void* dy, void* dw_f32,
                                const void* zero16, const StfConvGeom* g,
                                int splitk, hipStream_t stream);
hipError_t stf_im2col_bf16(const void* x, void* col, const StfConvGeom* g,
                           int64_t ld, hipStream_t stream);
hipError_t stf_col2im_bf16(const void* dcol, const void* side, void* dx,
                           const StfConvGeom* g, hipStream_t stream);
hipError_t stf_conv_dx_filter(const void* w, void* wt, int r, int s, int c,
                              int64_t k, int64_t rscp, hipStream_t stream);
hipError_t stf_conv2d_dx_8ph(const void* dy, const void* wt, void* dx,
                             const void* side, const void* zero16,
                             const StfConvGeom* g, int64_t rscp,
                             hipStream_t stream);

hipError_t stf_depthwise_fwd(const void* x, const void* w, void* y,
                             const StfConvGeom* g, int mult,
                             hipStream_t stream);
hipError_t stf_depthwise_bwd_input(const void* dy, const void* w, void* dx,
                                   const StfConvGeom* g, int mult,
                                   hipStream_t stream);
hipError_t stf_depthwise_bwd_filter(const void* x, const void* dy,
                                    float* dw_f32, const StfConvGeom* g,
                                    int mult, hipStream_t stream);

hipError_t stf_unary(int op, int dtype, const void* x, void* y, int64_t n,
                     hipStream_t stream);
hipError_t stf_binary(int op, int dtype, const void* a, const void* b,
                      void* y, int64_t n, hipStream_t stream);
hipError_t stf_binary_scalar(int op, int dtype, const void* a,
                             const void* scalar, void* y, int64_t n,
                             int scalar_left, hipStream_t stream);
hipError_t stf_binary_bcast(int op, int dtype, const void* a, const void* b,
                            void* y, int64_t n, int rank,
                            const int64_t* out_dims, const int64_t* sa,
                            const int64_t* sb, hipStream_t stream);
hipError_t stf_cast(int sdt, int ddt, const void* x, void* y, int64_t n,
                    hipStream_t stream);
hipError_t stf_cast_f32_bf16_zero(void* src_f32, void* dst_bf16, int64_t n,
                                  hipStream_t stream);
hipError_t stf_fill_f32(void* y, float v, int64_t n, int as_bf16,
                        hipStream_t stream);
hipError_t stf_scale(int dtype, const void* x, void* y, int64_t n,
                     float factor, hipStream_t stream);
hipError_t stf_fused_elementwise(int dtype, const void** inputs,
                                 const uint8_t* scalar_flags, int n_in,
                                 const int64_t* prog, int n_prog, void* out,
                                 int64_t n, hipStream_t stream);

hipError_t stf_lrn_fwd(const void* x, void* y, int64_t rows, int c,
                       int radius, float bias, float alpha, float beta,
                       hipStream_t stream);

hipError_t stf_bias_add(int dtype, const void* x, const void* bias, void* y,
                        int64_t n, int c, hipStream_t stream);
hipError_t stf_bias_grad(int dtype, const void* dy, void* db_f32,
                         int64_t rows, int c, hipStream_t stream);
hipError_t stf_softmax(int dtype, int log_sm, const void* x, void* y,
                       int64_t rows, int cols, hipStream_t stream);
hipError_t stf_sparse_xent(int dtype, const void* logits, const void* labels,
                           int labels_i32, void* loss_f32, void* backprop,
                           int64_t rows, int cols, hipStream_t stream);
hipError_t stf_xent(int dtype, const void* logits, const void* labels,
                    void* loss_f32, void* backprop, int64_t rows, int cols,
                    hipStream_t stream);

hipError_t stf_bn_fwd(int dtype, const void* x, const void* scale,
                      const void* offset, float* acc, float* mean, float* var,
                      float* inv_std, void* y, int64_t rows, int c, float eps,
                      int fuse_relu, hipStream_t stream);
hipError_t stf_bn_stats_only(int dtype, const void* x, float* acc,
                             float* mean, float* var, float* inv_std,
                             int64_t rows, int c, float eps,
                             hipStream_t stream);
hipError_t stf_bn_add_relu(const void* x, const void* side, const float* mean,
                           const float* inv_std, const void* scale,
                           const void* offset, void* y, int64_t rows, int c,
                           hipStream_t stream);
hipError_t stf_bn_bwd(int dtype, const void* dy, const void* x,
                      const void* y_relu, const float* mean,
                      const float* inv_std, const void* scale, float* sum_dy,
                      float* sum_dy_xhat, void* dx, void* dside, int64_t rows,
                      int c, int fuse_relu, hipStream_t stream);

hipError_t stf_pool_fwd(int dtype, int is_max, const void* x, void* y,
                        const StfPoolGeom* g, hipStream_t stream);
hipError_t stf_max_pool_bwd(int dtype, const void* x, const void* dy,
                            float* dx_f32, const StfPoolGeom* g,
                            hipStream_t stream);
hipError_t stf_max_pool_bwd_v8(const void* x, const void* dy, void* dx_bf16,
                               const StfPoolGeom* g, hipStream_t stream);
hipError_t stf_avg_pool_bwd(int dtype, const void* dy, void* dx,
                            const StfPoolGeom* g, hipStream_t stream);

hipError_t stf_lstm_gates(int dtype, const void* gates, const void* c_prev,
                          float forget_bias, void* i_out, void* f_out,
                          void* o_out, void* ci_out, void* cs_out,
                          void* co_out, void* h_out, int64_t batch, int H,
                          hipStream_t stream);
hipError_t stf_lstm_gates_grad(int dtype, const void* c_prev, const void* i_,
                               const void* f_, const void* o_,
                               const void* ci_, const void* co_,
                               const void* dh, const void* dcs_next,
                               void* dgates, void* dc_prev, int64_t batch,
                               int H, hipStream_t stream);

hipError_t stf_transpose2d(int elem_size, const void* in, void* out,
                           int64_t rows, int64_t cols, hipStream_t stream);
hipError_t stf_permute(int elem_size, const void* in, void* out, int64_t n,
                       int rank, const int64_t* out_dims,
                       const int64_t* src_strides, hipStream_t stream);
hipError_t stf_block_pad(int dtype, const void* src, void* dst,
                         int64_t nblocks, int64_t in_block, int64_t out_block,
                         hipStream_t stream);
hipError_t stf_strided_copy(int elem_size, int scatter, const void* src,
                            void* dst, int64_t outer, int64_t rows,
                            int64_t inner, int64_t big_stride,
                            int64_t row_off, hipStream_t stream);

hipError_t stf_l2loss(int dtype, const void* x, float* out_f32, int64_t n,
                      hipStream_t stream);
hipError_t stf_full_reduce(int dtype, StfReduce red, const void* x,
                           float* out_f32, int64_t n, hipStream_t stream);
hipError_t stf_row_reduce(int dtype, StfReduce red, const void* x, float* y,
                          int64_t rows, int64_t inner, hipStream_t stream);
hipError_t stf_col_reduce(int dtype, StfReduce red, const void* x, float* y,
                          int64_t outer, int64_t inner, hipStream_t stream);

hipError_t stf_apply_sgd(int grad_bf16, void* var, const void* lr,
                         const void* grad, int64_t n, hipStream_t stream);
hipError_t stf_apply_momentum(int grad_bf16, void* var, void* accum,
                              const void* lr, const void* grad,
                              const void* momentum, int nesterov, int64_t n,
                              hipStream_t stream);
hipError_t stf_apply_adam(int grad_bf16, void* var, void* m, void* v,
                          const void* b1p, const void* b2p, const void* lr,
                          const void* b1, const void* b2, const void* eps,
                          const void* grad, int64_t n, hipStream_t stream);

hipError_t stf_random_uniform(uint64_t seed, void* ctr_dev, void* out,
                              int64_t n, int as_bf16, hipStream_t stream);
hipError_t stf_random_normal(uint64_t seed, void* ctr_dev, void* out,
                             int64_t n, int as_bf16, int truncated,
                             hipStream_t stream);

hipError_t stf_gather_rows(int dtype, int idx_i32, const void* params,
                           const void* indices, void* out, int64_t nidx,
                           int64_t row, int64_t nrows, hipStream_t stream);
hipError_t stf_segment_sum(int dtype, int idx_i32, const void* data,
                           const void* ids, float* out_f32, int64_t nidx,
                           int64_t row, int64_t nseg, hipStream_t stream);

int stf_comm_max_segments();
hipError_t stf_comm_pack(int nseg, const void* const* ptrs,
                         const int64_t* ends, const unsigned char* is_bf16,
                         float* dst, int64_t total, hipStream_t stream);
hipError_t stf_comm_unpack(int nseg, void* const* ptrs, const int64_t* ends,
                           const unsigned char* is_bf16, const float* src,
                           float scale, int64_t total, hipStream_t stream);

}
```

simple_tensorflow_amd/csrc/runtime/session.cc:

```cpp
#include "runtime/session.h"

#include "gpu/gpu_tracer.h"

#include <algorithm>
#include <atomic>
#include <chrono>
#include <condition_variable>
#include <set>
#include <thread>

#include "graph/graph.h"

namespace stf {

void AddGpuDevices(DeviceMgr* mgr);
void* NewResourceMgr();
void DeleteResourceMgr(void*);

namespace {

std::pair<std::string, int> ParseTensorName(const std::string& s) {
  auto colon = s.rfind(':');
  if (colon != std::string::npos &&
      s.find_first_not_of("0123456789", colon + 1) == std::string::npos &&
      colon + 1 < s.size())
    return {s.substr(0, colon), atoi(s.c_str() + colon + 1)};
  return {s, 0};
}

NodeDef MakeSendRecv(const std::string& op, const std::string& name,
                     DataType dtype, const std::string& tensor_name,
                     const std::string& send_dev, const std::string& recv_dev) {
  NodeDef d;
  d.name = name;
  d.op = op;
  d.attr[op == "_Recv" ? "tensor_type" : "T"] = AttrValue::Type(dtype);
  d.attr["tensor_name"] = AttrValue::S(tensor_name);
  d.attr["send_device"] = AttrValue::S(send_dev);
  d.attr["recv_device"] = AttrValue::S(recv_dev);
  return d;
}

}

DirectSession::DirectSession(bool force_cpu_only, int num_threads) {
  devices_.AddDevice(std::make_unique<ThreadPoolDevice>("/cpu:0"));
  if (!force_cpu_only) AddGpuDevices(&devices_);
  int n = num_threads > 0 ? num_threads
                          : std::max(4u, std::thread::hardware_concurrency());
  pool_ = std::make_unique<ThreadPool>(n);
  resource_mgr_ = NewResourceMgr();
}

Status DirectSession::Create(const GraphDef& def) {
  std::lock_guard<std::mutex> l(mu_);
  graph_def_ = def;
  executors_.clear();
  return Status::OK();
}

Status DirectSession::Extend(const GraphDef& def) {
  std::lock_guard<std::mutex> l(mu_);
  for (auto& n : def.node) graph_def_.node.push_back(n);
  executors_.clear();
  return Status::OK();
}

Status DirectSession::GetOrCreateExecutors(
    const std::vector<std::string>& feeds,
    const std::vector<std::string>& fetches,
    const std::vector<std::string>& targets, ExecutorsAndKeys** out) {
  std::string key;
  for (auto& f : feeds) key += f + ",";
  key += "|";
  for (auto& f : fetches) key += f + ",";
  key += "|";
  for (auto& t : targets) key += t + ",";
  {
    std::lock_guard<std::mutex> l(mu_);
    auto it = executors_.find(key);
    if (it != executors_.end()) {
      *out = it->second.get();
      return Status::OK();
    }
  }
  std::unique_ptr<ExecutorsAndKeys> ek;
  STF_RETURN_IF_ERROR(BuildExecutors(feeds, fetches, targets, &ek));
  std::lock_guard<std::mutex> l(mu_);
  auto& slot = executors_[key];
  if (!slot) slot = std::move(ek);
  *out = slot.get();
  return Status::OK();
}

Status DirectSession::BuildExecutors(const std::vector<std::string>& feeds,
                                     const std::vector<std::string>& fetches,
                                     const std::vector<std::string>& targets,
                                     std::unique_ptr<ExecutorsAndKeys>* out) {
  GraphDef gdef_copy;
  {
    std::lock_guard<std::mutex> l(mu_);
    gdef_copy = graph_def_;
  }
  auto graph = std::make_unique<Graph>();
  STF_RETURN_IF_ERROR(ConvertGraphDefToGraph(gdef_copy, graph.get()));
  auto ek = std::make_unique<ExecutorsAndKeys>();

  {
    std::set<std::string> preserve;
    for (auto& f : feeds) preserve.insert(ParseTensorName(f).first);
    for (auto& f : fetches) preserve.insert(ParseTensorName(f).first);
    for (auto& t : targets) preserve.insert(ParseTensorName(t).first);
    OptimizeGraph(graph.get(), devices_.LookUp("/cpu:0"), preserve);
  }

  std::vector<Node*> order;
  STF_RETURN_IF_ERROR(TopologicalOrder(*graph, &order));
  Device* cpu = devices_.LookUp("/cpu:0");
  Device* gpu0 = nullptr;
  for (auto& d : devices_.devices())
    if (d->is_gpu() && !gpu0) gpu0 = d.get();

  auto kernel_available = [&](Node* n, Device* d) {
    if (n->IsControlFlow() || n->IsSend() || n->IsRecv() || n->op() == "NoOp")
      return true;
    return KernelRegistry::Global()->HasKernel(n->def, d->device_type());
  };
  for (Node* n : order) {
    std::string req = CanonicalDevice(n->def.device);
    Device* dev = nullptr;
    if (req.empty() && n->op() == "Const") {
      DataType dt;
      if (GetAttrType(n->def, "dtype", &dt) && dt == DT_INT32) {
        n->assigned_device = CanonicalDevice(cpu->name());
        continue;
      }
    }
    {
      bool touches_string = false;
      for (auto t : n->out_types)
        if (t == DT_STRING) touches_string = true;
      for (auto t : n->in_types)
        if (t == DT_STRING) touches_string = true;
      if (touches_string && !n->IsControlFlow()) {
        bool gpu_ok = false;
        const KernelDef* kd =
            gpu0 ? KernelRegistry::Global()->Find(n->def, "GPU") : nullptr;
        const OpDef* od = OpRegistry::Global()->LookUp(n->op());
        if (kd && od) {
          gpu_ok = od->output_arg.size() == n->out_types.size() &&
                   od->input_arg.size() == n->in_types.size();
          if (gpu_ok)
            for (size_t i = 0; i < n->out_types.size(); ++i)
              if (n->out_types[i] == DT_STRING &&
                  !kd->host_memory.count(od->output_arg[i].name))
                gpu_ok = false;
          if (gpu_ok)
            for (size_t i = 0; i < n->in_types.size(); ++i)
              if (n->in_types[i] == DT_STRING &&
                  !kd->host_memory.count(od->input_arg[i].name))
                gpu_ok = false;
        }
        if (!gpu_ok) {
          n->assigned_device = CanonicalDevice(cpu->name());
          continue;
        }
      }
    }
    if (!req.empty()) {
      dev = devices_.LookUp(req);
      if (!dev && StrStartsWith(req, "GPU") && gpu0) dev = gpu0;
      if (!dev) dev = cpu;
      if (!kernel_available(n, dev)) dev = cpu;
    } else {
      for (auto* e : n->in_edges) {
        if (e->IsControl()) continue;
        if (e->src_output < (int)e->src->out_is_ref.size() &&
            e->src->out_is_ref[e->src_output] &&
            !e->src->assigned_device.empty()) {
          Device* cand = devices_.LookUp(e->src->assigned_device);
          if (cand && kernel_available(n, cand)) {
            dev = cand;
            break;
          }
        }
      }
      if (!dev) {
        if (gpu0 && kernel_available(n, gpu0)) dev = gpu0;
        else dev = cpu;
      }
    }
    n->assigned_device = CanonicalDevice(dev->name());
  }

  std::map<std::string, Node*> feed_nodes;
  for (auto& f : feeds) {
    auto [name, port] = ParseTensorName(f);
    Node* n = graph->FindNode(name);
    if (!n) return errors::NotFound("Feed node not found: ", name);
    std::string fkey = name + ":" + std::to_string(port);
    if (feed_nodes.count(fkey)) continue;
    std::string dev = n->assigned_device;
    std::string node_name = "_feed_" + name + "_" + std::to_string(port);
    NodeDef rd = MakeSendRecv("_Recv", node_name, n->out_types[port],
                              "feed:" + fkey, "client", dev);
    Node* recv;
    STF_RETURN_IF_ERROR(graph->AddNode(rd, &recv));
    recv->assigned_device = dev;
    ek->feed_devices["feed:" + fkey] = dev;
    std::vector<Edge*> to_rewire;
    for (auto* e : n->out_edges)
      if (!e->IsControl() && e->src_output == port) to_rewire.push_back(e);
    for (auto* e : to_rewire) {
      Node* dst = e->dst;
      int slot = e->dst_input;
      graph->RemoveEdge(e);
      graph->AddEdge(recv, 0, dst, slot);
    }
    feed_nodes[fkey] = recv;
  }

  std::vector<Node*> keep;
  for (auto& f : fetches) {
    auto [name, port] = ParseTensorName(f);
    std::string fkey = name + ":" + std::to_string(port);
    Node* src;
    int src_port;
    if (feed_nodes.count(fkey)) {
      src = feed_nodes[fkey];
      src_port = 0;
    } else {
      src = graph->FindNode(name);
      if (!src) return errors::NotFound("Fetch node not found: ", name);
      src_port = port;
      if (src_port >= src->num_outputs())
        return errors::InvalidArgument("Fetch ", f, ": port out of range");
    }
    std::string dev = src->assigned_device;
    NodeDef sd = MakeSendRecv("_Send",
                              "_fetch_" + name + "_" + std::to_string(port) +
                                  "_" + std::to_string(keep.size()),
                              src->out_types[src_port], "fetch:" + fkey, dev,
                              "client");
    Node* send;
    STF_RETURN_IF_ERROR(graph->AddNode(sd, &send));
    send->assigned_device = dev;
    graph->AddEdge(src, src_port, send, 0);
    ek->fetch_devices["fetch:" + fkey] = dev;
    keep.push_back(send);
  }
  for (auto& t : targets) {
    Node* n = graph->FindNode(ParseTensorName(t).first);
    if (!n) return errors::NotFound("Target node not found: ", t);
    keep.push_back(n);
  }

  std::set<Node*> reachable;
  std::vector<Node*> stack(keep);
  while (!stack.empty()) {
    Node* n = stack.back();
    stack.pop_back();
    if (!reachable.insert(n).second) continue;
    for (auto* e : n->in_edges) stack.push_back(e->src);
  }
  std::vector<Node*> to_remove;
  for (Node* n : graph->nodes())
    if (!reachable.count(n)) to_remove.push_back(n);
  for (Node* n : to_remove) graph->RemoveNode(n);

  std::set<std::string> part_devices;
  for (Node* n : graph->nodes()) part_devices.insert(n->assigned_device);

  std::map<std::string, GraphDef> parts;
  std::map<std::string, std::string> send_dedup;
  int edge_id = 0;
  for (auto& dev : part_devices) parts[dev];

  for (Node* n : graph->nodes()) {
    NodeDef d = n->def;
    d.device = n->assigned_device;
    d.input.clear();
    parts[n->assigned_device].node.push_back(d);
  }
  std::map<std::string, size_t> defs;
  for (auto& kv : parts)
    for (size_t i = 0; i < kv.second.node.size(); ++i)
      defs[kv.first + "|" + kv.second.node[i].name] = i;

  auto add_input = [&](const std::string& dev, const std::string& node,
                       const std::string& input) {
    parts[dev].node[defs[dev + "|" + node]].input.push_back(input);
  };

  for (Node* n : graph->nodes()) {
    std::vector<const Edge*> data(n->num_inputs(), nullptr);
    std::vector<const Edge*> ctrl;
    for (auto* e : n->in_edges) {
      if (e->IsControl()) ctrl.push_back(e);
      else data[e->dst_input] = e;
    }
    const std::string& ddev = n->assigned_device;
    for (auto* e : data) {
      if (!e) return errors::Internal("missing input edge on ", n->name());
      Node* s = e->src;
      if (s->assigned_device == ddev) {
        add_input(ddev, n->name(),
                  e->src_output == 0
                      ? s->name()
                      : s->name() + ":" + std::to_string(e->src_output));
      } else {
        std::string dkey = s->name() + ":" + std::to_string(e->src_output) +
                           "|" + ddev;
        auto it = send_dedup.find(dkey);
        std::string recv_name;
        if (it != send_dedup.end()) {
          recv_name = it->second;
        } else {
          std::string tname = "e" + std::to_string(edge_id++) + "_" + s->name();
          DataType dt = s->out_types[e->src_output];
          NodeDef sd = MakeSendRecv("_Send", "_s_" + tname, dt, tname,
                                    s->assigned_device, ddev);
          sd.device = s->assigned_device;
          sd.input.push_back(e->src_output == 0
                                 ? s->name()
                                 : s->name() + ":" +
                                       std::to_string(e->src_output));
          parts[s->assigned_device].node.push_back(sd);
          NodeDef rd = MakeSendRecv("_Recv", "_r_" + tname, dt, tname,
                                    s->assigned_device, ddev);
          rd.device = ddev;
          parts[ddev].node.push_back(rd);
          recv_name = rd.name;
          send_dedup[dkey] = recv_name;
        }
        add_input(ddev, n->name(), recv_name);
      }
    }
    for (auto* e : ctrl) {
      Node* s = e->src;
      if (s->assigned_device == ddev) {
        add_input(ddev, n->name(), "^" + s->name());
      } else {
        std::string dkey = s->name() + ":ctrl|" + ddev;
        auto it = send_dedup.find(dkey);
        std::string recv_name;
        if (it != send_dedup.end()) {
          recv_name = it->second;
        } else {
          std::string tname = "c" + std::to_string(edge_id++) + "_" + s->name();
          NodeDef cd;
          cd.name = "_c_" + tname;
          cd.op = "Const";
          cd.attr["dtype"] = AttrValue::Type(DT_BOOL);
          TensorProto tp;
          tp.dtype = DT_BOOL;
          tp.has_shape = true;
          tp.bool_val.push_back(0);
          AttrValue av;
          av.kind = 'e';
          av.tensor = tp;
          cd.attr["value"] = av;
          cd.device = s->assigned_device;
          cd.input.push_back("^" + s->name());
          parts[s->assigned_device].node.push_back(cd);
          NodeDef sd = MakeSendRecv("_Send", "_s_" + tname, DT_BOOL, tname,
                                    s->assigned_device, ddev);
          sd.device = s->assigned_device;
          sd.input.push_back(cd.name);
          parts[s->assigned_device].node.push_back(sd);
          NodeDef rd = MakeSendRecv("_Recv", "_r_" + tname, DT_BOOL, tname,
                                    s->assigned_device, ddev);
          rd.device = ddev;
          parts[ddev].node.push_back(rd);
          recv_name = rd.name;
          send_dedup[dkey] = recv_name;
        }
        add_input(ddev, n->name(), "^" + recv_name);
      }
    }
  }

  {
    int gpu_parts = 0;
    bool host_trivial = true;
    for (auto& kv : parts) {
      Device* dev = devices_.LookUp(kv.first);
      if (dev && dev->is_gpu()) {
        ++gpu_parts;
        continue;
      }
      for (auto& nd : kv.second.node) {
        if (nd.op != "Const" && nd.op != "_Send" && nd.op != "_Recv" &&
            nd.op != "NoOp" && nd.op != "Shape")
          host_trivial = false;
      }
    }
    ek->capture_eligible = gpu_parts == 1 && host_trivial &&
                           getenv("STF_NO_HIPGRAPH") == nullptr;
  }

  for (auto& kv : parts) {
    Device* dev = devices_.LookUp(kv.first);
    if (!dev) return errors::Internal("Unknown partition device ", kv.first);
    auto pg = std::make_unique<Graph>();
    STF_RETURN_IF_ERROR(ConvertGraphDefToGraph(kv.second, pg.get()));
    for (Node* n : pg->nodes()) n->assigned_device = kv.first;
    ExecutorsAndKeys::Item item;
    item.device = dev;
    STF_RETURN_IF_ERROR(
        Executor::Create(std::move(pg), dev, &opseg_, &item.executor));
    ek->items.push_back(std::move(item));
  }
  *out = std::move(ek);
  return Status::OK();
}

void DirectSession::Reset() {
  std::lock_guard<std::mutex> l(mu_);
  executors_.clear();
  opseg_.Clear();
  DeleteResourceMgr(resource_mgr_);
  resource_mgr_ = NewResourceMgr();
}


struct DirectSession::PartialRunState {
  std::shared_ptr<Rendezvous> rendez;
  ExecutorsAndKeys* ek = nullptr;
  std::mutex mu;
  std::condition_variable cv;
  int remaining = 0;
  Status agg;
  std::set<std::string> pending_fetches;
  std::set<std::string> pending_feeds;
};

Status DirectSession::PartialRunSetup(const std::vector<std::string>& feeds,
                                      const std::vector<std::string>& fetches,
                                      const std::vector<std::string>& targets,
                                      std::string* handle) {
  ExecutorsAndKeys* ek = nullptr;
  STF_RETURN_IF_ERROR(GetOrCreateExecutors(feeds, fetches, targets, &ek));
  auto prs = std::make_shared<PartialRunState>();
  prs->rendez = std::make_shared<Rendezvous>();
  prs->ek = ek;
  prs->remaining = (int)ek->items.size();
  for (auto& f : feeds) {
    auto [name, port] = ParseTensorName(f);
    prs->pending_feeds.insert(name + ":" + std::to_string(port));
  }
  for (auto& f : fetches) {
    auto [name, port] = ParseTensorName(f);
    prs->pending_fetches.insert(name + ":" + std::to_string(port));
  }
  int64_t step_id;
  {
    std::lock_guard<std::mutex> l(mu_);
    step_id = ++step_counter_;
    *handle = "prun_" + std::to_string(++partial_run_counter_);
    partial_runs_[*handle] = prs;
  }
  ThreadPool* pool = pool_.get();
  for (auto& item : ek->items) {
    ExecutorArgs args;
    args.step_id = step_id;
    args.rendezvous = prs->rendez.get();
    args.schedule = [pool](std::function<void()> fn) {
      pool->Schedule(std::move(fn));
    };
    args.resource_mgr = resource_mgr_;
    item.executor->RunAsync(args, [prs](Status s) {
      std::lock_guard<std::mutex> l(prs->mu);
      if (!s.ok() && prs->agg.ok()) prs->agg = s;
      if (--prs->remaining == 0) prs->cv.notify_all();
    });
  }
  return Status::OK();
}

Status DirectSession::PartialRun(
    const std::string& handle,
    const std::vector<std::pair<std::string, Tensor>>& feeds,
    const std::vector<std::string>& fetches, std::vector<Tensor>* outputs) {
  std::shared_ptr<PartialRunState> prs;
  {
    std::lock_guard<std::mutex> l(mu_);
    auto it = partial_runs_.find(handle);
    if (it == partial_runs_.end())
      return errors::InvalidArgument("Unknown partial-run handle ", handle);
    prs = it->second;
  }
  for (auto& f : feeds) {
    auto [name, port] = ParseTensorName(f.first);
    std::string fkey = name + ":" + std::to_string(port);
    {
      std::lock_guard<std::mutex> l(prs->mu);
      if (!prs->pending_feeds.erase(fkey))
        return errors::InvalidArgument(
            "Feed ", f.first,
            " was not declared in partial_run_setup (or already fed)");
    }
    auto it = prs->ek->feed_devices.find("feed:" + fkey);
    if (it == prs->ek->feed_devices.end())
      return errors::Internal("feed not wired: ", f.first);
    STF_RETURN_IF_ERROR(prs->rendez->Send(
        RendezvousKey("client", it->second, "feed:" + fkey, "", 0), f.second,
        false));
  }
  outputs->clear();
  Status fetch_status;
  for (auto& f : fetches) {
    auto [name, port] = ParseTensorName(f);
    std::string fkey = name + ":" + std::to_string(port);
    {
      std::lock_guard<std::mutex> l(prs->mu);
      if (!prs->pending_fetches.count(fkey))
        return errors::InvalidArgument(
            "Fetch ", f, " was not declared in partial_run_setup (or was "
            "already fetched)");
    }
    auto it = prs->ek->fetch_devices.find("fetch:" + fkey);
    if (it == prs->ek->fetch_devices.end()) {
      fetch_status = errors::Internal("fetch not wired: ", f);
      break;
    }
    Tensor val;
    bool is_dead = false;
    Status s = prs->rendez->Recv(
        RendezvousKey(it->second, "client", "fetch:" + fkey, "", 0), &val,
        &is_dead);
    if (!s.ok()) {
      fetch_status = s;
      break;
    }
    if (val.IsInitialized() && val.mem_space() == MemSpace::DEVICE) {
      Device* dev = devices_.LookUp(it->second);
      Tensor host;
      Status cs = dev->CopyDeviceTensorToHost(val, &host);
      if (!cs.ok()) {
        fetch_status = cs;
        break;
      }
      val = host;
    }
    outputs->push_back(val);
    std::lock_guard<std::mutex> l(prs->mu);
    prs->pending_fetches.erase(fkey);
  }
  bool finished;
  {
    std::lock_guard<std::mutex> l(prs->mu);
    finished = prs->pending_fetches.empty();
  }
  if (!fetch_status.ok() || finished) {
    prs->rendez->StartAbort(errors::Cancelled("partial run finished"));
    {
      std::unique_lock<std::mutex> l(prs->mu);
      prs->cv.wait_for(l, std::chrono::seconds(2),
                       [&]() { return prs->remaining == 0; });
    }
    std::lock_guard<std::mutex> l(mu_);
    partial_runs_.erase(handle);
  }
  return fetch_status;
}

DirectSession::~DirectSession() {
  std::map<std::string, std::shared_ptr<PartialRunState>> pending;
  {
    std::lock_guard<std::mutex> l(mu_);
    pending.swap(partial_runs_);
  }
  for (auto& kv : pending) {
    PartialRunState& prs = *kv.second;
    prs.rendez->StartAbort(errors::Cancelled("session closed"));
    std::unique_lock<std::mutex> l(prs.mu);
    prs.cv.wait_for(l, std::chrono::seconds(10),
                    [&]() { return prs.remaining == 0; });
  }
  DeleteResourceMgr(resource_mgr_);
}

Status DirectSession::Run(
    const std::vector<std::pair<std::string, Tensor>>& feeds,
    const std::vector<std::string>& fetches,
    const std::vector<std::string>& targets, std::vector<Tensor>* outputs,
    StatsCollector* stats, int64_t timeout_ms) {
  std::vector<std::string> feed_names;
  for (auto& f : feeds) feed_names.push_back(f.first);
  ExecutorsAndKeys* ek = nullptr;
  STF_RETURN_IF_ERROR(GetOrCreateExecutors(feed_names, fetches, targets, &ek));

  auto rendez_sp = std::make_shared<Rendezvous>();
  Rendezvous& rendez = *rendez_sp;
  for (auto& f : feeds) {
    auto [name, port] = ParseTensorName(f.first);
    std::string fkey = "feed:" + name + ":" + std::to_string(port);
    auto it = ek->feed_devices.find(fkey);
    if (it == ek->feed_devices.end())
      return errors::Internal("feed not wired: ", f.first);
    STF_RETURN_IF_ERROR(rendez.Send(
        RendezvousKey("client", it->second, fkey, "", 0), f.second, false));
  }

  bool no_io = feeds.empty() && fetches.empty() && stats == nullptr;
  if (no_io && ek->capture_eligible && ek->graph_exec) {
    outputs->clear();
    return ek->capture_device->LaunchCapturedGraph(ek->graph_exec);
  }
  bool do_capture = false;
  Device* capture_dev = nullptr;
  if (no_io && ek->capture_eligible && !ek->capture_broken &&
      ek->graph_exec == nullptr) {
    std::lock_guard<std::mutex> l(mu_);
    if (++ek->plain_runs > 2) {
      do_capture = true;
      for (auto& item : ek->items)
        if (item.device->is_gpu()) capture_dev = item.device;
    }
  }
  if (do_capture && capture_dev) {
    Status s = capture_dev->BeginGraphCapture();
    if (!s.ok()) {
      ek->capture_broken = true;
      do_capture = false;
    }
  }

  GpuTracer tracer;
  if (stats) {
    std::vector<Device*> gpus;
    for (auto& item : ek->items)
      if (item.device->is_gpu()) gpus.push_back(item.device);
    if (!gpus.empty() && tracer.Start(gpus).ok()) {
      stats->gpu_pre = [&tracer](Device* d) { return tracer.Pre(d); };
      stats->gpu_post = [&tracer](Device* d, void* t, const std::string& n,
                                  const std::string& o) {
        tracer.Post(d, t, n, o);
      };
    }
  }

  int64_t step_id;
  {
    std::lock_guard<std::mutex> l(mu_);
    step_id = ++step_counter_;
  }
  struct RunState {
    std::mutex mu;
    std::condition_variable cv;
    int remaining = 0;
    Status agg;
    std::atomic<bool> done{false};
    std::atomic<bool> cancelled{false};
  };
  auto rs = std::make_shared<RunState>();
  rs->remaining = (int)ek->items.size();
  std::mutex& mu = rs->mu;
  std::condition_variable& cv = rs->cv;
  int& remaining = rs->remaining;
  Status& agg = rs->agg;
  std::shared_ptr<std::thread> watchdog;
  if (timeout_ms > 0) {
    watchdog = std::make_shared<std::thread>([rs, rendez_sp, timeout_ms]() {
      std::unique_lock<std::mutex> l(rs->mu);
      if (!rs->cv.wait_for(l, std::chrono::milliseconds(timeout_ms),
                           [&]() { return rs->done.load(); })) {
        rs->cancelled = true;
        l.unlock();
        rendez_sp->StartAbort(
            errors::DeadlineExceeded("Session::Run timed out after ",
                                     timeout_ms, " ms"));
      }
    });
  }
  auto finish_watchdog = [&]() {
    if (watchdog) {
      {
        std::lock_guard<std::mutex> l(rs->mu);
        rs->done = true;
      }
      rs->cv.notify_all();
      watchdog->join();
      watchdog.reset();
    }
  };
  std::deque<std::function<void()>> inline_q;
  std::mutex inline_mu;
  ThreadPool* pool = pool_.get();
  std::function<void(std::function<void()>)> scheduler;
  if (do_capture) {
    scheduler = [&](std::function<void()> fn) {
      std::lock_guard<std::mutex> l(inline_mu);
      inline_q.push_back(std::move(fn));
    };
  } else {
    scheduler = [pool](std::function<void()> fn) {
      pool->Schedule(std::move(fn));
    };
  }
  for (auto& item : ek->items) {
    ExecutorArgs args;
    args.step_id = step_id;
    args.rendezvous = rendez_sp.get();
    args.is_cancelled = [rs]() { return rs->cancelled.load(); };
    args.schedule = scheduler;
    args.resource_mgr = resource_mgr_;
    args.stats = stats;
    item.executor->RunAsync(args, [rs, rendez_sp](Status s) {
      std::lock_guard<std::mutex> l(rs->mu);
      if (!s.ok() && rs->agg.ok()) rs->agg = s;
      if (--rs->remaining == 0) rs->cv.notify_all();
    });
  }
  if (do_capture) {
    for (;;) {
      std::function<void()> fn;
      {
        std::lock_guard<std::mutex> l(inline_mu);
        if (!inline_q.empty()) {
          fn = std::move(inline_q.front());
          inline_q.pop_front();
        }
      }
      if (fn) {
        fn();
        continue;
      }
      std::lock_guard<std::mutex> l(mu);
      if (remaining == 0) break;
      std::this_thread::yield();
    }
  }

  outputs->clear();
  Status fetch_status;
  for (auto& f : fetches) {
    auto [name, port] = ParseTensorName(f);
    std::string fkey = "fetch:" + name + ":" + std::to_string(port);
    auto it = ek->fetch_devices.find(fkey);
    if (it == ek->fetch_devices.end()) {
      fetch_status = errors::Internal("fetch not wired: ", f);
      break;
    }
    Tensor val;
    bool is_dead = false;
    Status s =
        rendez.Recv(RendezvousKey(it->second, "client", fkey, "", 0), &val,
                    &is_dead);
    if (!s.ok()) {
      fetch_status = s;
      break;
    }
    if (val.IsInitialized() && val.mem_space() == MemSpace::DEVICE) {
      Device* dev = devices_.LookUp(it->second);
      Tensor host;
      Status cs = dev->CopyDeviceTensorToHost(val, &host);
      if (!cs.ok()) {
        fetch_status = cs;
        break;
      }
      val = host;
    }
    outputs->push_back(val);
  }

  {
    std::unique_lock<std::mutex> l(mu);
    if (timeout_ms > 0) {
      if (!cv.wait_for(l, std::chrono::milliseconds(500),
                       [&]() { return remaining == 0; })) {
        l.unlock();
        finish_watchdog();
        return errors::DeadlineExceeded(
            "Session::Run timed out after ", timeout_ms,
            " ms (executors still pending)");
      }
    } else {
      cv.wait(l, [&]() { return remaining == 0; });
    }
  }
  finish_watchdog();
  if (do_capture && capture_dev) {
    if (agg.ok()) {
      void* exec = nullptr;
      Status cs = capture_dev->EndGraphCapture(&exec);
      if (cs.ok()) {
        ek->graph_exec = exec;
        ek->capture_device = capture_dev;
        Status ls = capture_dev->LaunchCapturedGraph(exec);
        if (!ls.ok()) return ls;
      } else {
        LOG(WARN) << "hipGraph capture failed; falling back to eager: "
                  << cs.ToString();
        ek->capture_broken = true;
      }
    } else {
      void* exec = nullptr;
      capture_dev->EndGraphCapture(&exec);
      ek->capture_broken = true;
    }
  }
  if (stats) {
    stats->gpu_pre = nullptr;
    stats->gpu_post = nullptr;
    (void)tracer.Collect(stats);
  }
  if (!agg.ok()) {
    if (do_capture) {
      return Run(feeds, fetches, targets, outputs);
    }
    return agg;
  }
  return fetch_status;
}

}
```

Measured before the change: 6717 images/sec.

## Fuse BatchNorm statistics into the preceding bf16 Conv2D GEMM epilogue

Adds a graph pass that rewrites Conv2D→BatchNormMi/BatchNormAddReluMi pairs into stats-producing variants. The conv GEMM epilogue accumulates per-channel sum and sum-of-squares into per-tile partials, which a small kernel then reduces. The BN op then only finalizes and normalizes, so it no longer re-reads the conv output just to compute statistics. The costs are an extra reduction kernel, LDS reduction work in the GEMM epilogue, and a fallback separate sums pass on non-8ph paths.

```diff
diff --git a/simple_tensorflow_amd/csrc/framework/ops_defs.cc b/simple_tensorflow_amd/csrc/framework/ops_defs.cc
--- a/simple_tensorflow_amd/csrc/framework/ops_defs.cc
+++ b/simple_tensorflow_amd/csrc/framework/ops_defs.cc
@@ -147,6 +147,9 @@
 REGISTER_OP("FusedBatchNormGrad").Input("y_backprop: T").Input("x: T").Input("scale: T").Input("reserve_space_1: T").Input("reserve_space_2: T").Output("x_backprop: T").Output("scale_backprop: T").Output("offset_backprop: T").Output("reserve_space_3: T").Output("reserve_space_4: T").Attr("T: {float}").Attr("epsilon: float = 0.0001").Attr("data_format: string = 'NHWC'").Attr("is_training: bool = true");
 REGISTER_OP("BatchNormMi").Input("x: T").Input("scale: float").Input("offset: float").Output("y: T").Output("batch_mean: float").Output("batch_variance: float").Output("reserve_inv_std: float").Attr("T: {float, bfloat16}").Attr("epsilon: float = 0.0001").Attr("fuse_relu: bool = false");
 REGISTER_OP("BatchNormAddReluMi").Input("x: T").Input("scale: float").Input("offset: float").Input("side: T").Output("y: T").Output("batch_mean: float").Output("batch_variance: float").Output("reserve_inv_std: float").Attr("T: {float, bfloat16}").Attr("epsilon: float = 0.0001");
+REGISTER_OP("_Conv2DBnStats").Input("input: T").Input("filter: T").Output("output: T").Output("sums: float").Attr("T: {bfloat16}").Attr("strides: list(int)").Attr("use_cudnn_on_gpu: bool = true").Attr("padding: string").Attr("data_format: string = 'NHWC'");
+REGISTER_OP("_BatchNormMiStats").Input("x: T").Input("scale: float").Input("offset: float").Input("sums: float").Output("y: T").Output("batch_mean: float").Output("batch_variance: float").Output("reserve_inv_std: float").Attr("T: {bfloat16}").Attr("epsilon: float = 0.0001").Attr("fuse_relu: bool = false");
+REGISTER_OP("_BatchNormAddReluMiStats").Input("x: T").Input("scale: float").Input("offset: float").Input("side: T").Input("sums: float").Output("y: T").Output("batch_mean: float").Output("batch_variance: float").Output("reserve_inv_std: float").Attr("T: {bfloat16}").Attr("epsilon: float = 0.0001");
 REGISTER_OP("BatchNormAddReluMiGrad").Input("y_backprop: T").Input("x: T").Input("scale: float").Input("saved_mean: float").Input("saved_inv_std: float").Input("y_relu: T").Output("x_backprop: T").Output("scale_backprop: float").Output("offset_backprop: float").Output("side_backprop: T").Attr("T: {float, bfloat16}").Attr("epsilon: float = 0.0001");
 REGISTER_OP("BatchNormMiGrad").Input("y_backprop: T").Input("x: T").Input("scale: float").Input("saved_mean: float").Input("saved_inv_std: float").Input("y_relu: T").Output("x_backprop: T").Output("scale_backprop: float").Output("offset_backprop: float").Attr("T: {float, bfloat16}").Attr("epsilon: float = 0.0001").Attr("fuse_relu: bool = false");
 REGISTER_OP("_FusedElementwise").Input("inputs: N * T").Output("output: T").Attr("N: int >= 1").Attr("T: {float, bfloat16}").Attr("program: list(int)");
diff --git a/simple_tensorflow_amd/csrc/graph/graph.h b/simple_tensorflow_amd/csrc/graph/graph.h
--- a/simple_tensorflow_amd/csrc/graph/graph.h
+++ b/simple_tensorflow_amd/csrc/graph/graph.h
@@ -94,6 +94,7 @@
 
 class Device;
 
-int OptimizeGraph(Graph* g, Device* cpu, const std::set<std::string>& preserve);
+int OptimizeGraph(Graph* g, Device* cpu, const std::set<std::string>& preserve,
+                  bool have_gpu);
 
 }
diff --git a/simple_tensorflow_amd/csrc/graph/optimizer.cc b/simple_tensorflow_amd/csrc/graph/optimizer.cc
--- a/simple_tensorflow_amd/csrc/graph/optimizer.cc
+++ b/simple_tensorflow_amd/csrc/graph/optimizer.cc
@@ -3,6 +3,7 @@
 #include <string>
 #include <vector>
 
+#include "framework/device.h"
 #include "framework/op_kernel.h"
 #include "graph/graph.h"
 #include "kernels/fused_ew.h"
@@ -393,10 +394,70 @@
   return fused_total;
 }
 
+
+std::string GpuPlacementKey(const Node* n, bool have_gpu) {
+  if (!have_gpu) return "";
+  if (n->def.device.empty()) return "default";
+  std::string req = CanonicalDevice(n->def.device);
+  return StrStartsWith(req, "GPU") ? req : "";
+}
+
+bool RetypeNode(Node* n, const std::string& op) {
+  const OpDef* od = OpRegistry::Global()->LookUp(op);
+  if (!od) return false;
+  NodeDef def = n->def;
+  def.op = op;
+  std::vector<DataType> in, out;
+  std::vector<bool> refs;
+  if (!InOutTypesForNode(def, *od, &in, &out, &refs).ok()) return false;
+  n->def = std::move(def);
+  n->op_def = od;
+  n->in_types = std::move(in);
+  n->out_types = std::move(out);
+  n->out_is_ref = std::move(refs);
+  return true;
+}
+
+int FuseConvBnStats(Graph* g, const std::set<std::string>& preserve,
+                    bool have_gpu) {
+  int fused = 0;
+  std::vector<Node*> nodes = g->nodes();
+  for (Node* conv : nodes) {
+    if (conv->op() != "Conv2D" || preserve.count(conv->name()) ||
+        conv->out_types[0] != DT_BFLOAT16)
+      continue;
+    std::string where = GpuPlacementKey(conv, have_gpu);
+    if (where.empty()) continue;
+    Node* bn = nullptr;
+    int n_bn = 0;
+    for (const Edge* e : conv->out_edges) {
+      if (e->IsControl() || e->dst_input != 0) continue;
+      if (e->dst->op() == "BatchNormMi" ||
+          e->dst->op() == "BatchNormAddReluMi") {
+        bn = e->dst;
+        ++n_bn;
+      }
+    }
+    if (n_bn != 1 || preserve.count(bn->name()) ||
+        bn->in_types[0] != DT_BFLOAT16 ||
+        GpuPlacementKey(bn, have_gpu) != where)
+      continue;
+    int sums_slot = bn->num_inputs();
+    if (!RetypeNode(conv, "_Conv2DBnStats")) continue;
+    if (!RetypeNode(bn, "_" + bn->op() + "Stats")) {
+      RetypeNode(conv, "Conv2D");
+      continue;
+    }
+    g->AddEdge(conv, 1, bn, sums_slot);
+    ++fused;
+  }
+  return fused;
+}
+
 }
 
 int OptimizeGraph(Graph* g, Device* cpu,
-                  const std::set<std::string>& preserve) {
+                  const std::set<std::string>& preserve, bool have_gpu) {
   static const bool disabled = getenv("STF_NO_GRAPH_OPT") != nullptr;
   if (disabled) return 0;
   int total = 0;
@@ -408,6 +469,8 @@
   }
   static const bool no_fusion = getenv("STF_NO_FUSION") != nullptr;
   if (!no_fusion) total += FuseElementwise(g, preserve);
+  if (getenv("STF_NO_CONV_BN_STATS") == nullptr)
+    total += FuseConvBnStats(g, preserve, have_gpu);
   return total;
 }
 
diff --git a/simple_tensorflow_amd/csrc/kernels/gpu_conv.cc b/simple_tensorflow_amd/csrc/kernels/gpu_conv.cc
--- a/simple_tensorflow_amd/csrc/kernels/gpu_conv.cc
+++ b/simple_tensorflow_amd/csrc/kernels/gpu_conv.cc
@@ -80,7 +80,8 @@
 
 class GpuConv2DOp : public OpKernel {
  public:
-  explicit GpuConv2DOp(OpKernelConstruction* c) : OpKernel(c) {
+  explicit GpuConv2DOp(OpKernelConstruction* c, bool stats = false)
+      : OpKernel(c), stats_(stats) {
     c->GetAttr("strides", &strides_);
     c->GetAttr("padding", &padding_);
   }
@@ -92,6 +93,11 @@
     OP_REQUIRES_OK(ctx, GetConvGeom(x.shape(), w.shape(), strides_, padding_,
                                     &g));
     Tensor* y = ctx->allocate_output(0, TensorShape({g.N, g.P, g.Q, g.K}));
+    float* sums = nullptr;
+    if (stats_) {
+      sums = ctx->allocate_output(1, TensorShape({2 * g.K}))->flat<float>();
+      OP_HIP_OK(ctx, ZeroF32(sums, 2 * g.K, s));
+    }
     if (!g.is_1x1_s1() && (g.C % 8) != 0 && x.dtype() == DT_BFLOAT16) {
       int64_t c = g.C;
       Tensor xp, wp;
@@ -122,8 +128,21 @@
                                                    : kIm2ColGemm;
 
     Tensor wt;
+    Tensor partial;
+    float* pt = nullptr;
+    auto sum_partials = [&]() {
+      return stf_bn_partial_sums(pt, sums, g.M() / 256, (int)(2 * g.K), s);
+    };
     if (path == kImplicit8Ph) {
       OP_HIP_OK(ctx, TransposeBf16(ctx, w.raw_data(), rscp, g.K, &wt, s));
+      if (stats_) {
+        pt = TilePartials(ctx, g, &partial);
+        OP_HIP_OK(ctx, stf_conv2d_fwd_8ph_stats(x.raw_data(), wt.raw_data(),
+                                                y->raw_data(), pt, ZeroPage(),
+                                                &sg, rscp, s));
+        OP_HIP_OK(ctx, sum_partials());
+        return;
+      }
       OP_HIP_OK(ctx, stf_conv2d_fwd_8ph(x.raw_data(), wt.raw_data(),
                                         y->raw_data(), ZeroPage(), &sg, rscp,
                                         s));
@@ -133,25 +152,51 @@
       OP_HIP_OK(ctx, stf_conv2d_fwd_nt(x.raw_data(), w.raw_data(),
                                        y->raw_data(), ZeroPage(), &sg, rscp,
                                        s));
-      return;
-    }
-    Tensor col = x;
-    if (!g.is_1x1_s1()) OP_HIP_OK(ctx, Im2Col(ctx, x, g, rscp, &col, s));
-    if (!fits_8ph && (g.K & 7) == 0) {
-      OP_HIP_OK(ctx, stf_gemm_bf16(col.raw_data(), w.raw_data(), y->raw_data(),
-                                   g.M(), g.K, rscp, rscp, g.K, 0, 1, s));
     } else {
-      OP_HIP_OK(ctx, TransposeBf16(ctx, w.raw_data(), rscp, g.K, &wt, s));
-      OP_HIP_OK(ctx, stf_gemm_bf16_nt(col.raw_data(), wt.raw_data(),
-                                      y->raw_data(), g.M(), g.K, rscp, s));
-    }
-  }
-
- private:
+      Tensor col = x;
+      if (!g.is_1x1_s1()) OP_HIP_OK(ctx, Im2Col(ctx, x, g, rscp, &col, s));
+      if (!fits_8ph && (g.K & 7) == 0) {
+        OP_HIP_OK(ctx, stf_gemm_bf16(col.raw_data(), w.raw_data(),
+                                     y->raw_data(), g.M(), g.K, rscp, rscp,
+                                     g.K, 0, 1, s));
+      } else {
+        OP_HIP_OK(ctx, TransposeBf16(ctx, w.raw_data(), rscp, g.K, &wt, s));
+        if (stats_ && fits_8ph && getenv("STF_NO_8PH") == nullptr) {
+          pt = TilePartials(ctx, g, &partial);
+          OP_HIP_OK(ctx, stf_gemm_bf16_8ph_stats(col.raw_data(),
+                                                 wt.raw_data(), y->raw_data(),
+                                                 pt, g.M(), g.K, rscp, rscp,
+                                                 rscp, s));
+          OP_HIP_OK(ctx, sum_partials());
+          return;
+        }
+        OP_HIP_OK(ctx, stf_gemm_bf16_nt(col.raw_data(), wt.raw_data(),
+                                        y->raw_data(), g.M(), g.K, rscp, s));
+      }
+    }
+    if (stats_)
+      OP_HIP_OK(ctx, stf_bn_sums(1, y->raw_data(), sums, g.M(), (int)g.K, s));
+  }
+
+ private:
+  static float* TilePartials(OpKernelContext* ctx, const GpuConvGeom& g,
+                             Tensor* t) {
+    *t = ctx->allocate_temp(DT_FLOAT, TensorShape({g.M() / 256, 2 * g.K}));
+    return t->flat<float>();
+  }
+
+  bool stats_;
   std::vector<int64_t> strides_;
   std::string padding_;
 };
 REGISTER_KERNEL_BUILDER(Name("Conv2D").Device(DEVICE_GPU).TypeConstraint<bfloat16>("T"), GpuConv2DOp);
+
+class GpuConv2DBnStatsOp : public GpuConv2DOp {
+ public:
+  explicit GpuConv2DBnStatsOp(OpKernelConstruction* c)
+      : GpuConv2DOp(c, true) {}
+};
+REGISTER_KERNEL_BUILDER(Name("_Conv2DBnStats").Device(DEVICE_GPU).TypeConstraint<bfloat16>("T"), GpuConv2DBnStatsOp);
 
 class GpuConv2DBackpropInputOp : public OpKernel {
  public:
diff --git a/simple_tensorflow_amd/csrc/kernels/gpu_nn.cc b/simple_tensorflow_amd/csrc/kernels/gpu_nn.cc
--- a/simple_tensorflow_amd/csrc/kernels/gpu_nn.cc
+++ b/simple_tensorflow_amd/csrc/kernels/gpu_nn.cc
@@ -114,7 +114,8 @@
 
 class GpuBatchNormMiOp : public OpKernel {
  public:
-  explicit GpuBatchNormMiOp(OpKernelConstruction* c) : OpKernel(c) {
+  explicit GpuBatchNormMiOp(OpKernelConstruction* c, bool given_sums = false)
+      : OpKernel(c), given_sums_(given_sums) {
     c->GetAttr("epsilon", &eps_);
     c->GetAttr("fuse_relu", &fuse_relu_);
   }
@@ -129,6 +130,18 @@
     Tensor* var = ctx->allocate_output(2, TensorShape({c}));
     Tensor* inv_std = ctx->allocate_output(3, TensorShape({c}));
     hipStream_t s = GPU_STREAM(ctx);
+    if (given_sums_) {
+      const Tensor& sums = ctx->input(3);
+      OP_REQUIRES(ctx, sums.NumElements() == 2 * c,
+                  errors::InvalidArgument("_BatchNormMiStats: sums size"));
+      OP_HIP_OK(ctx, stf_bn_fwd_acc(DtypeCode(x.dtype()), x.raw_data(),
+                                    scale.raw_data(), offset.raw_data(),
+                                    sums.flat<float>(), mean->flat<float>(),
+                                    var->flat<float>(),
+                                    inv_std->flat<float>(), y->raw_data(),
+                                    rows, c, eps_, fuse_relu_ ? 1 : 0, s));
+      return;
+    }
     Tensor acc = ctx->allocate_temp(DT_FLOAT, TensorShape({2 * c}));
     OP_HIP_OK(ctx, ZeroF32(acc.raw_data(), 2 * c, s));
     OP_HIP_OK(ctx, stf_bn_fwd(DtypeCode(x.dtype()), x.raw_data(),
@@ -140,15 +153,24 @@
   }
 
  private:
+  bool given_sums_;
   float eps_ = 1e-4f;
   bool fuse_relu_ = false;
 };
+class GpuBatchNormMiStatsOp : public GpuBatchNormMiOp {
+ public:
+  explicit GpuBatchNormMiStatsOp(OpKernelConstruction* c)
+      : GpuBatchNormMiOp(c, true) {}
+};
+REGISTER_KERNEL_BUILDER(Name("_BatchNormMiStats").Device(DEVICE_GPU).TypeConstraint<bfloat16>("T"), GpuBatchNormMiStatsOp);
 REGISTER_KERNEL_BUILDER(Name("BatchNormMi").Device(DEVICE_GPU).TypeConstraint<float>("T"), GpuBatchNormMiOp);
 REGISTER_KERNEL_BUILDER(Name("BatchNormMi").Device(DEVICE_GPU).TypeConstraint<bfloat16>("T"), GpuBatchNormMiOp);
 
 class GpuBatchNormAddReluMiOp : public OpKernel {
  public:
-  explicit GpuBatchNormAddReluMiOp(OpKernelConstruction* c) : OpKernel(c) {
+  explicit GpuBatchNormAddReluMiOp(OpKernelConstruction* c,
+                                   bool given_sums = false)
+      : OpKernel(c), given_sums_(given_sums) {
     c->GetAttr("epsilon", &eps_);
   }
   void Compute(OpKernelContext* ctx) override {
@@ -163,6 +185,20 @@
     Tensor* var = ctx->allocate_output(2, TensorShape({c}));
     Tensor* inv_std = ctx->allocate_output(3, TensorShape({c}));
     hipStream_t s = GPU_STREAM(ctx);
+    if (given_sums_) {
+      const Tensor& sums = ctx->input(4);
+      OP_REQUIRES(ctx, sums.NumElements() == 2 * c,
+                  errors::InvalidArgument(
+                      "_BatchNormAddReluMiStats: sums size"));
+      OP_HIP_OK(ctx, stf_bn_add_relu_acc(x.raw_data(), side.raw_data(),
+                                         sums.flat<float>(),
+                                         mean->flat<float>(),
+                                         var->flat<float>(),
+                                         inv_std->flat<float>(),
+                                         scale.raw_data(), offset.raw_data(),
+                                         y->raw_data(), rows, c, eps_, s));
+      return;
+    }
     Tensor acc = ctx->allocate_temp(DT_FLOAT, TensorShape({2 * c}));
     OP_HIP_OK(ctx, ZeroF32(acc.raw_data(), 2 * c, s));
     OP_HIP_OK(ctx, stf_bn_stats_only(DtypeCode(x.dtype()), x.raw_data(),
@@ -178,9 +214,16 @@
   }
 
  private:
+  bool given_sums_;
   float eps_ = 1e-4f;
 };
 REGISTER_KERNEL_BUILDER(Name("BatchNormAddReluMi").Device(DEVICE_GPU).TypeConstraint<bfloat16>("T"), GpuBatchNormAddReluMiOp);
+class GpuBatchNormAddReluMiStatsOp : public GpuBatchNormAddReluMiOp {
+ public:
+  explicit GpuBatchNormAddReluMiStatsOp(OpKernelConstruction* c)
+      : GpuBatchNormAddReluMiOp(c, true) {}
+};
+REGISTER_KERNEL_BUILDER(Name("_BatchNormAddReluMiStats").Device(DEVICE_GPU).TypeConstraint<bfloat16>("T"), GpuBatchNormAddReluMiStatsOp);
 
 class GpuBatchNormMiGradOp : public OpKernel {
  public:
diff --git a/simple_tensorflow_amd/csrc/kernels/hip/bn.hip b/simple_tensorflow_amd/csrc/kernels/hip/bn.hip
--- a/simple_tensorflow_amd/csrc/kernels/hip/bn.hip
+++ b/simple_tensorflow_amd/csrc/kernels/hip/bn.hip
@@ -358,13 +358,30 @@
   }
 }
 
+__global__ void BnPartialSumsKernel(const float* __restrict__ partial,
+                                    float* __restrict__ acc, int64_t tiles,
+                                    int cols) {
+  __shared__ float red[4][64];
+  int lane_c = threadIdx.x & 63, lane_r = threadIdx.x >> 6;
+  int col = blockIdx.x * 64 + lane_c;
+  float sum = 0.f;
+  if (col < cols)
+    for (int64_t t = (int64_t)blockIdx.y * 4 + lane_r; t < tiles;
+         t += (int64_t)gridDim.y * 4)
+      sum += partial[t * cols + col];
+  red[lane_r][lane_c] = sum;
+  __syncthreads();
+  if (lane_r == 0 && col < cols)
+    atomicAdd(&acc[col], (red[0][lane_c] + red[1][lane_c]) +
+                             (red[2][lane_c] + red[3][lane_c]));
+}
+
 inline bool UseV9(int dtype, int c) { return dtype != 0 && c % 8 == 0; }
 
 inline size_t BnLdsBytes(int c) { return (size_t)c * 2 * sizeof(float); }
 
-void LaunchBnStats(int dtype, const void* x, float* acc, float* mean,
-                   float* var, float* inv_std, int64_t rows, int c, float eps,
-                   hipStream_t stream) {
+void LaunchBnSums(int dtype, const void* x, float* acc, int64_t rows, int c,
+                  hipStream_t stream) {
   if (UseV9(dtype, c)) {
     hipLaunchKernelGGL(BnStatsKernelV9, dim3(BnGridV9(c, rows)), dim3(256),
                        BnLdsBytes(c), stream, (const __bf16*)x, acc, rows, c);
@@ -375,26 +392,26 @@
                          BnLdsBytes(c), stream, (const T*)x, acc, rows, c);
     });
   }
+}
+
+void LaunchBnFinalize(const float* acc, float* mean, float* var,
+                      float* inv_std, int64_t rows, int c, float eps,
+                      hipStream_t stream) {
   hipLaunchKernelGGL(BnFinalizeKernel, dim3((c + 255) / 256), dim3(256), 0,
                      stream, acc, mean, var, inv_std, rows, c, eps);
 }
 
-}
-
-extern "C" {
-
-hipError_t stf_bn_stats_only(int dtype, const void* x, float* acc, float* mean,
-                             float* var, float* inv_std, int64_t rows, int c,
-                             float eps, hipStream_t stream) {
-  LaunchBnStats(dtype, x, acc, mean, var, inv_std, rows, c, eps, stream);
-  return hipGetLastError();
-}
-
-hipError_t stf_bn_fwd(int dtype, const void* x, const void* scale,
-                      const void* offset, float* acc, float* mean, float* var,
-                      float* inv_std, void* y, int64_t rows, int c, float eps,
-                      int fuse_relu, hipStream_t stream) {
-  LaunchBnStats(dtype, x, acc, mean, var, inv_std, rows, c, eps, stream);
+void LaunchBnStats(int dtype, const void* x, float* acc, float* mean,
+                   float* var, float* inv_std, int64_t rows, int c, float eps,
+                   hipStream_t stream) {
+  LaunchBnSums(dtype, x, acc, rows, c, stream);
+  LaunchBnFinalize(acc, mean, var, inv_std, rows, c, eps, stream);
+}
+
+void LaunchBnNorm(int dtype, const void* x, const void* scale,
+                  const void* offset, const float* mean, const float* inv_std,
+                  void* y, int64_t rows, int c, int fuse_relu,
+                  hipStream_t stream) {
   DispatchBool(fuse_relu, [&](auto relu) {
     constexpr bool RELU = decltype(relu)::value;
     if (UseV9(dtype, c)) {
@@ -413,6 +430,55 @@
                          c);
     });
   });
+}
+
+}
+
+extern "C" {
+
+hipError_t stf_bn_stats_only(int dtype, const void* x, float* acc, float* mean,
+                             float* var, float* inv_std, int64_t rows, int c,
+                             float eps, hipStream_t stream) {
+  LaunchBnStats(dtype, x, acc, mean, var, inv_std, rows, c, eps, stream);
+  return hipGetLastError();
+}
+
+hipError_t stf_bn_fwd(int dtype, const void* x, const void* scale,
+                      const void* offset, float* acc, float* mean, float* var,
+                      float* inv_std, void* y, int64_t rows, int c, float eps,
+                      int fuse_relu, hipStream_t stream) {
+  LaunchBnStats(dtype, x, acc, mean, var, inv_std, rows, c, eps, stream);
+  LaunchBnNorm(dtype, x, scale, offset, mean, inv_std, y, rows, c, fuse_relu,
+               stream);
+  return hipGetLastError();
+}
+
+hipError_t stf_bn_fwd_acc(int dtype, const void* x, const void* scale,
+                          const void* offset, const float* acc, float* mean,
+                          float* var, float* inv_std, void* y, int64_t rows,
+                          int c, float eps, int fuse_relu,
+                          hipStream_t stream) {
+  LaunchBnFinalize(acc, mean, var, inv_std, rows, c, eps, stream);
+  LaunchBnNorm(dtype, x, scale, offset, mean, inv_std, y, rows, c, fuse_relu,
+               stream);
+  return hipGetLastError();
+}
+
+hipError_t stf_bn_sums(int dtype, const void* x, float* acc, int64_t rows,
+                       int c, hipStream_t stream) {
+  LaunchBnSums(dtype, x, acc, rows, c, stream);
+  return hipGetLastError();
+}
+
+hipError_t stf_bn_partial_sums(const float* partial, float* acc,
+                               int64_t tiles, int cols, hipStream_t stream) {
+  if (tiles < 1 || cols < 1) return hipErrorInvalidValue;
+  int strips = (cols + 63) / 64;
+  int64_t splits = (tiles + 15) / 16;
+  int64_t cap = strips >= 1024 ? 1 : 1024 / strips;
+  if (splits > cap) splits = cap;
+  hipLaunchKernelGGL(BnPartialSumsKernel, dim3(strips, (uint32_t)splits),
+                     dim3(256), 0, stream, partial, acc, tiles, cols);
   return hipGetLastError();
 }
 
@@ -426,6 +492,17 @@
                      (const __bf16*)side, mean, inv_std, (const float*)scale,
                      (const float*)offset, (__bf16*)y, rows, c);
   return hipGetLastError();
+}
+
+hipError_t stf_bn_add_relu_acc(const void* x, const void* side,
+                               const float* acc, float* mean, float* var,
+                               float* inv_std, const void* scale,
+                               const void* offset, void* y, int64_t rows,
+                               int c, float eps, hipStream_t stream) {
+  if (c % 8 != 0) return hipErrorInvalidValue;
+  LaunchBnFinalize(acc, mean, var, inv_std, rows, c, eps, stream);
+  return stf_bn_add_relu(x, side, mean, inv_std, scale, offset, y, rows, c,
+                         stream);
 }
 
 hipError_t stf_bn_bwd(int dtype, const void* dy, const void* x,
diff --git a/simple_tensorflow_amd/csrc/kernels/hip/gemm_bf16_8ph.hip b/simple_tensorflow_amd/csrc/kernels/hip/gemm_bf16_8ph.hip
--- a/simple_tensorflow_amd/csrc/kernels/hip/gemm_bf16_8ph.hip
+++ b/simple_tensorflow_amd/csrc/kernels/hip/gemm_bf16_8ph.hip
@@ -30,11 +30,13 @@
   }
 }
 
-template <int NR, bool OUT_BF16, bool FUSE_RELU, class AG>
+template <int NR, bool OUT_BF16, bool FUSE_RELU, class AG, bool STATS = false>
 __launch_bounds__(512) __global__ void Gemm256x8Ph(
     AG ag, const uint16_t* __restrict__ B, void* __restrict__ C,
     const float* __restrict__ bias, const uint16_t* __restrict__ side,
-    int64_t M, int64_t N, int64_t K, int64_t ldb) {
+    int64_t M, int64_t N, int64_t K, int64_t ldb,
+    float* __restrict__ partial) {
+  static_assert(!STATS || OUT_BF16, "STATS reads the rounded bf16 tile");
   constexpr int kBN = 64 * NR;
   constexpr int kABytes = kBM * kBK * 2;
   constexpr int kBBytes = kBN * kBK * 2;
@@ -193,13 +195,25 @@
     }
     __builtin_amdgcn_s_barrier();
     asm volatile("s_waitcnt lgkmcnt(0)" ::: "memory");
+    float p1[8] = {0, 0, 0, 0, 0, 0, 0, 0};
+    float p2[8] = {0, 0, 0, 0, 0, 0, 0, 0};
 #pragma unroll
     for (int p = 0; p < kBM * kBN / 8 / kThreads; ++p) {
       int sidx = (p * kThreads + tid) * 8;
       int r = sidx / kBN;
       int c = sidx % kBN;
       int64_t off = (m0 + r) * N + n0 + c;
-      if (side) {
+      if constexpr (STATS) {
+        __bf16 v[8];
+        *(ulong2*)v = *(ulong2*)(cbuf + sidx);
+        *(ulong2*)((uint16_t*)C + off) = *(ulong2*)v;
+#pragma unroll
+        for (int e = 0; e < 8; ++e) {
+          float f = (float)v[e];
+          p1[e] += f;
+          p2[e] += f * f;
+        }
+      } else if (side) {
         __bf16 v[8], sv[8];
         *(ulong2*)v = *(ulong2*)(cbuf + sidx);
         *(ulong2*)sv = *(const ulong2*)(side + off);
@@ -208,6 +222,29 @@
         *(ulong2*)((uint16_t*)C + off) = *(ulong2*)v;
       } else {
         *(ulong2*)((uint16_t*)C + off) = *(ulong2*)(cbuf + sidx);
+      }
+    }
+    if constexpr (STATS) {
+      constexpr int kRedLd = kThreads + 8;
+      constexpr int kWin = kBN / 8;
+      float* red = (float*)lds;
+      asm volatile("s_waitcnt lgkmcnt(0)" ::: "memory");
+      __builtin_amdgcn_s_barrier();
+#pragma unroll
+      for (int e = 0; e < 8; ++e) {
+        red[e * kRedLd + tid] = p1[e];
+        red[(8 + e) * kRedLd + tid] = p2[e];
+      }
+      asm volatile("s_waitcnt lgkmcnt(0)" ::: "memory");
+      __builtin_amdgcn_s_barrier();
+      asm volatile("" ::: "memory");
+      if (tid < 2 * kBN) {
+        int stat = tid / kBN, col = tid % kBN;
+        const float* src = red + (stat * 8 + (col & 7)) * kRedLd + (col >> 3);
+        float sum = 0.f;
+#pragma unroll
+        for (int g = 0; g < kThreads / kWin; ++g) sum += src[g * kWin];
+        partial[((int64_t)(bid / nbn) * 2 + stat) * N + n0 + col] = sum;
       }
     }
     return;
@@ -230,18 +267,18 @@
   }
 }
 
-template <class AG>
+template <bool STATS = false, class AG>
 hipError_t Launch8Ph(const AG& ag, const void* B, void* C, const void* side,
                      int64_t M, int64_t N, int64_t K, int64_t ldb,
-                     hipStream_t stream) {
+                     hipStream_t stream, float* partial = nullptr) {
   auto launch = [&](auto nr_c) {
     constexpr int NR = decltype(nr_c)::value;
     int64_t blocks = (M / kBM) * (N / (64 * NR));
     size_t shmem = 64 * 1024 + 2 * (size_t)(64 * NR) * kBK * 2;
-    hipLaunchKernelGGL((Gemm256x8Ph<NR, true, false, AG>),
+    hipLaunchKernelGGL((Gemm256x8Ph<NR, true, false, AG, STATS>),
                        dim3((uint32_t)blocks), dim3(kThreads), shmem, stream,
                        ag, (const uint16_t*)B, C, (const float*)nullptr,
-                       (const uint16_t*)side, M, N, K, ldb);
+                       (const uint16_t*)side, M, N, K, ldb, partial);
   };
   if (N % 256 == 0) launch(std::integral_constant<int, 4>{});
   else if (N % 128 == 0) launch(std::integral_constant<int, 2>{});
@@ -274,6 +311,26 @@
     return hipErrorInvalidValue;
   return Launch8Ph(MakeConvAG(*g, x, zero16), wt, y, nullptr, M, g->cout,
                    rscp, rscp, stream);
+}
+
+hipError_t stf_gemm_bf16_8ph_stats(const void* A, const void* B, void* C,
+                                   float* partial, int64_t M, int64_t N,
+                                   int64_t K, int64_t lda, int64_t ldb,
+                                   hipStream_t stream) {
+  if (!stf_gemm_bf16_8ph_ok(M, N, K)) return hipErrorInvalidValue;
+  LinearAG ag{(const uint16_t*)A, lda};
+  return Launch8Ph<true>(ag, B, C, nullptr, M, N, K, ldb, stream, partial);
+}
+
+hipError_t stf_conv2d_fwd_8ph_stats(const void* x, const void* wt, void* y,
+                                    float* partial, const void* zero16,
+                                    const StfConvGeom* g, int64_t rscp,
+                                    hipStream_t stream) {
+  int64_t M = (int64_t)g->n * g->p * g->q;
+  if (!stf_gemm_bf16_8ph_ok(M, g->cout, rscp) || (g->c % 8) != 0)
+    return hipErrorInvalidValue;
+  return Launch8Ph<true>(MakeConvAG(*g, x, zero16), wt, y, nullptr, M,
+                         g->cout, rscp, rscp, stream, partial);
 }
 
 hipError_t stf_conv2d_dx_8ph(const void* dy, const void* wt, void* dx,
diff --git a/simple_tensorflow_amd/csrc/kernels/hip/stf_kernels.h b/simple_tensorflow_amd/csrc/kernels/hip/stf_kernels.h
--- a/simple_tensorflow_amd/csrc/kernels/hip/stf_kernels.h
+++ b/simple_tensorflow_amd/csrc/kernels/hip/stf_kernels.h
@@ -40,12 +40,20 @@
                                   const void* side_bf16, int64_t M, int64_t N,
                                   int64_t K, int64_t lda, int64_t ldb,
                                   hipStream_t stream);
+hipError_t stf_gemm_bf16_8ph_stats(const void* A, const void* B, void* C,
+                                   float* partial, int64_t M, int64_t N,
+                                   int64_t K, int64_t lda, int64_t ldb,
+                                   hipStream_t stream);
 hipError_t stf_gemm_f32_nt(const void* A, const void* B, void* C, int64_t M,
                            int64_t N, int64_t K, hipStream_t stream);
 
 hipError_t stf_conv2d_fwd_8ph(const void* x, const void* wt, void* y,
                               const void* zero16, const StfConvGeom* g,
                               int64_t rscp, hipStream_t stream);
+hipError_t stf_conv2d_fwd_8ph_stats(const void* x, const void* wt, void* y,
+                                    float* partial, const void* zero16,
+                                    const StfConvGeom* g, int64_t rscp,
+                                    hipStream_t stream);
 hipError_t stf_conv2d_fwd_nt(const void* x, const void* w, void* y,
                              const void* zero16, const StfConvGeom* g,
                              int64_t rscp, hipStream_t stream);
@@ -126,6 +134,20 @@
                            const float* inv_std, const void* scale,
                            const void* offset, void* y, int64_t rows, int c,
                            hipStream_t stream);
+hipError_t stf_bn_fwd_acc(int dtype, const void* x, const void* scale,
+                          const void* offset, const float* acc, float* mean,
+                          float* var, float* inv_std, void* y, int64_t rows,
+                          int c, float eps, int fuse_relu,
+                          hipStream_t stream);
+hipError_t stf_bn_add_relu_acc(const void* x, const void* side,
+                               const float* acc, float* mean, float* var,
+                               float* inv_std, const void* scale,
+                               const void* offset, void* y, int64_t rows,
+                               int c, float eps, hipStream_t stream);
+hipError_t stf_bn_sums(int dtype, const void* x, float* acc, int64_t rows,
+                       int c, hipStream_t stream);
+hipError_t stf_bn_partial_sums(const float* partial, float* acc,
+                               int64_t tiles, int cols, hipStream_t stream);
 hipError_t stf_bn_bwd(int dtype, const void* dy, const void* x,
                       const void* y_relu, const float* mean,
                       const float* inv_std, const void* scale, float* sum_dy,
diff --git a/simple_tensorflow_amd/csrc/runtime/session.cc b/simple_tensorflow_amd/csrc/runtime/session.cc
--- a/simple_tensorflow_amd/csrc/runtime/session.cc
+++ b/simple_tensorflow_amd/csrc/runtime/session.cc
@@ -111,7 +111,9 @@
     for (auto& f : feeds) preserve.insert(ParseTensorName(f).first);
     for (auto& f : fetches) preserve.insert(ParseTensorName(f).first);
     for (auto& t : targets) preserve.insert(ParseTensorName(t).first);
-    OptimizeGraph(graph.get(), devices_.LookUp("/cpu:0"), preserve);
+    bool have_gpu = false;
+    for (auto& d : devices_.devices()) have_gpu |= d->is_gpu();
+    OptimizeGraph(graph.get(), devices_.LookUp("/cpu:0"), preserve, have_gpu);
   }
 
   std::vector<Node*> order;
```

After: 7022 images/sec (median of 6 runs). 4.5% higher.
